# wzhe06/SparrowRecSys

Measured on AMD Instinct MI355X. Metric: ctr_samples_per_sec, higher is better.
Workload: dtype f32

## Files before the change

sparrowrecsys_amd/csrc/api_forward.h:

```cpp
static int launch_din_cols(sprk_handle h, const int32_t* ids, float* pooled, float* att, int32_t B, const DinColsMany* many, hipStream_t st) {
    DinColsRun c = h->din_cols_run;
    const long long ntasks = (long long)(many ? many->n : 1) * ((B + 15) / 16);
    const long long slots = (long long)h->num_cus * 16;
    c.ts = (c.T >= 16 && ntasks * 4 <= slots) ? 4 : ((c.T >= 8 && ntasks * 2 <= slots) ? 2 : 1);
    if (h->tune.din_cols_ts) c.ts = h->tune.din_cols_ts;
    if (many) c.ts = 1;
    c.ts_log2 = c.ts == 4 ? 2 : (c.ts == 2 ? 1 : 0);
    c.ql = (c.T + 3) / 4;
    const int EL = 4 * h->din_cols_kc;
    const size_t lds = ((size_t)2 * 64 * 36 + (size_t)DC_WAVES * 16 * c.idp + (size_t)DC_WAVES * 2 * 64 * EL) * sizeof(float);
    const long long grid = (ntasks * c.ts + DC_WAVES - 1) / DC_WAVES;
    if (many)
        hipLaunchKernelGGL(h->din_cols_kernels.many, dim3((unsigned)grid), dim3(DC_WAVES * 64), lds, st, c, nullptr, nullptr, nullptr, B, h->dev_err, *many);
    else
        hipLaunchKernelGGL(h->din_cols_kernels.one, dim3((unsigned)grid), dim3(DC_WAVES * 64), lds, st, c, ids, pooled, att, B, h->dev_err, DinColsOne{});
    HIP_TRY(hipGetLastError());
    return SPRK_OK;
}

static int launch_din_fused(sprk_handle h, const int32_t* ids, const float* dense, float* out, float* att, int32_t B, const DinFusedMany* many,
                            bool tail, hipStream_t st) {
    DinFusedRun c = h->din_fused_run;
    const long long ntasks = (long long)(many ? many->n : 1) * ((B + 15) / 16);
    const long long slots = (long long)h->num_cus * DF_WAVES;
// ... 136 lines not shown
        hipLaunchKernelGGL(h->mlp_rows_kernel, dim3(grid), dim3(MR_WAVES * 64), h->mlp_rows_lds, st, rr, ids, dense, out, B, h->dev_err, (const float*)h->mlp_rows_image);
        break;
    }
    case Route::DinTail: {
        const int tw = h->din_tail_waves;
        int grid = (ntasks + tw - 1) / tw;
        if (grid > h->num_cus) grid = h->num_cus;
        hipLaunchKernelGGL(h->din_tail_kernel, dim3(grid), dim3(tw * 64), kDinTailVariants[h->din_tail_variant].lds_bytes, st, h->din_tail_run, ids, dense, aux,
                           out, B, h->dev_err, h->din_tail_image, DinTailMany{});
        break;
    }
    default: {
        const int ntiles = (B + SPRK_TILE_M - 1) / SPRK_TILE_M;
        const int grid = ntiles < h->tile_grid_cap ? ntiles : h->tile_grid_cap;
        hipLaunchKernelGGL(k_tile_forward, dim3(grid), dim3(256), h->tile_lds_bytes, st, h->dev_plan, ids, dense, aux, out, B, h->dev_err);
    }
    }
    HIP_TRY(hipGetLastError());
    return SPRK_OK;
}

static int fork_helpers(sprk_handle h, int S, hipStream_t st) {
    HIP_TRY(hipEventRecord(h->many_fork, st));
    for (int s = 0; s < S; ++s) HIP_TRY(hipStreamWaitEvent(h->many_stream[s], h->many_fork, 0));
    return SPRK_OK;
}
static int join_helpers(sprk_handle h, int S, hipStream_t st) {
    for (int s = 0; s < S; ++s) {
        HIP_TRY(hipEventRecord(h->many_join[s], h->many_stream[s]));
        HIP_TRY(hipStreamWaitEvent(st, h->many_join[s], 0));
    }
    return SPRK_OK;
}

extern "C++" {
template <class Many, class Launch>
static int launch_groups(int32_t n_batches, int per, const int32_t* const* ids, const float* const* dense, float* const* out, Launch launch) {
    int g = 0;
    for (int32_t i0 = 0; i0 < n_batches; i0 += per, ++g) {
        Many m;
        memset(&m, 0, sizeof(m));
        m.n = n_batches - i0 < per ? n_batches - i0 : per;
        for (int j = 0; j < m.n; ++j) { m.ids[j] = ids[i0 + j]; m.dense[j] = dense ? dense[i0 + j] : nullptr; m.out[j] = out[i0 + j]; }
        SPRK_TRY(launch(m, g));
        HIP_TRY(hipGetLastError());
    }
    return SPRK_OK;
}
template <class Ok> static bool every_batch(int32_t n_batches, Ok ok) {
    for (int32_t i = 0; i < n_batches; ++i)
        if (!ok(i)) return false;
    return true;
}
}

static int launch_v2j_table(sprk_handle h, int32_t n_batches, const int32_t* const* ids, const float* const* dense, float* const* out, int32_t B,
                            hipStream_t st, bool* done) {
    *done = false;
    const int ntpb = (B + 15) / 16;
    long long grid = ((long long)n_batches * ntpb + V2_WAVES - 1) / V2_WAVES;
    if (grid > h->v2_grid_cap) grid = h->v2_grid_cap;
    if ((long long)n_batches * ntpb + 4 * grid * V2_WAVES >= (1LL << 31)) return SPRK_OK;
    hipStreamCaptureStatus cap = hipStreamCaptureStatusNone;
    if (hipStreamIsCapturing(st, &cap) != hipSuccess) { (void)hipGetLastError(); return SPRK_OK; }
    if (cap != hipStreamCaptureStatusNone) return SPRK_OK;
    const size_t n = (size_t)n_batches;
    int slot = h->v2j_table_last;
    bool same = slot >= 0 && h->v2j_table[slot].n == n && h->v2j_table[slot].stream == st;
    if (same) {
        const V2JBatch* last = h->v2j_table[slot].stage;
        for (size_t i = 0; i < n && same; ++i) same = last[i].ids == ids[i] && last[i].dense == dense[i] && last[i].out == out[i];
    }
    if (!same) {
        slot = h->v2j_table_last == 0 ? 1 : 0;
        sprk_engine::V2JTable& t = h->v2j_table[slot];
        if (!t.busy) HIP_TRY(hipEventCreateWithFlags(&t.busy, hipEventDisableTiming));
        if (t.used) HIP_TRY(hipEventSynchronize(t.busy));
        if (t.cap < n) {
            size_t want = t.cap ? 2 * t.cap : 4096;
            if (want < n) want = n;
            if (t.stage) (void)hipHostFree(t.stage);
            if (t.dev) (void)hipFree(t.dev);
            t.stage = nullptr; t.dev = nullptr; t.cap = 0; t.n = 0;
            HIP_TRY(hipHostMalloc((void**)&t.stage, want * sizeof(V2JBatch), hipHostMallocDefault));
            HIP_TRY(hipMalloc((void**)&t.dev, want * sizeof(V2JBatch)));
            t.cap = want;
        }
        t.n = 0;
        for (size_t i = 0; i < n; ++i) t.stage[i] = V2JBatch{ids[i], dense[i], out[i], nullptr};
        HIP_TRY(hipMemcpyAsync(t.dev, t.stage, n * sizeof(V2JBatch), hipMemcpyHostToDevice, st));
        t.n = n;
        t.stream = st;
        h->v2j_table_last = slot;
    }
    sprk_engine::V2JTable& t = h->v2j_table[slot];
    V2JRun jr = h->v2j_run;
    jr.flags = 0;
    const V2JManyTab m = {t.dev, n_batches, ntpb};
    hipLaunchKernelGGL(kV2JVariants[h->v2j_variant].fn_many_tab, dim3((int)grid), dim3(V2_WAVES * 64), h->v2j_lds_bytes, st, jr, m, B, h->dev_err, h->v2_image);
    HIP_TRY(hipGetLastError());
    HIP_TRY(hipEventRecord(t.busy, st));
    t.used = true;
    *done = true;
    return SPRK_OK;
}

static int forward_many_impl(sprk_handle h, int32_t n_batches, const int32_t* const* ids, const float* const* dense,
                             float* const* out, int32_t B, void* workspace, size_t workspace_bytes, void* stream,
                             int many_batches, int many_streams) {
    RoctxRange roctx_range_("sprk_forward_many");
    if (!h) return fail(SPRK_EINVAL, "handle is NULL");
    if (n_batches < 0) return fail(SPRK_EINVAL, "negative batch count");
    if (n_batches > 0 && !out) return fail(SPRK_EINVAL, "out is NULL");
    int S = (h->finalized && n_batches > 1) ? many_streams : 0;
    const size_t ws_need = (sprk_workspace_bytes(h, B) + 255) & ~(size_t)255;
    const bool ws_untouched = h->finalized && (h->route == Route::DinFused || h->route == Route::DienFused);
    if (S >= 2 && ws_need > 0 && !ws_untouched) {
        while (S >= 2 && (!workspace || workspace_bytes < (size_t)S * ws_need)) --S;
        if (S < 2) S = 0;
    }
    hipStream_t st = (hipStream_t)stream;
    const bool grouped = h->finalized && many_batches > 1 && n_batches > 1 && B > 0 && ids;
    const int ntpb = (B + 15) / 16;
    auto aligned = [&](int32_t i, const float* d) { return !(((uintptr_t)ids[i] | (uintptr_t)d) & 15); };
    auto present = [&](int32_t i) { return ids[i] && dense[i] && out[i]; };
    if (grouped && dense && h->route == Route::V2Joint && every_batch(n_batches, [&](int32_t i) { return present(i) && aligned(i, dense[i]); })) {
        const V2JVariant& jv = kV2JVariants[h->v2j_variant];
        V2JRun jr = h->v2j_run;
        jr.flags = 0;
        if (n_batches > many_batches) {
            bool done = false;
            SPRK_TRY(launch_v2j_table(h, n_batches, ids, dense, out, B, st, &done));
            if (done) return SPRK_OK;
        }
        return launch_groups<V2JMany>(n_batches, many_batches, ids, dense, out, [&](V2JMany& m, int) {
            m.ntpb = ntpb;
            long long grid = ((long long)m.n * ntpb + V2_WAVES - 1) / V2_WAVES;
            if (grid > h->v2_grid_cap) grid = h->v2_grid_cap;
            hipLaunchKernelGGL(jv.fn_many, dim3((int)grid), dim3(V2_WAVES * 64), h->v2j_lds_bytes, st, jr, m, B, h->dev_err, h->v2_image);
            return SPRK_OK;
        });
    }
    const float* const* rows_dense = h->plan.n_dense ? dense : nullptr;
    if (grouped && (dense || h->plan.n_dense == 0) && h->route == Route::Rows &&
        every_batch(n_batches, [&](int32_t i) { return ids[i] && out[i] && (!rows_dense || rows_dense[i]) && aligned(i, rows_dense ? rows_dense[i] : nullptr); })) {
        const RowsVariant& rv = kRowsVariants[h->rows_variant];
        RowsRun rr = h->rows_run;
        rr.flags = 0;
        return launch_groups<RowsMany>(n_batches, many_batches < RC_MB ? many_batches : RC_MB, ids, rows_dense, out, [&](RowsMany& m, int) {
            m.ntpb = ntpb;
            long long grid = ((long long)m.n * ntpb + RC_WAVES - 1) / RC_WAVES;
            if (grid > h->num_cus) grid = h->num_cus;
            hipLaunchKernelGGL(rv.fn_many, dim3((int)grid), dim3(RC_WAVES * 64), h->rows_lds_bytes, st, rr, m, B, h->dev_err, h->rows_image);
            return SPRK_OK;
        });
    }
    if (grouped && dense && h->route == Route::MlpRows && h->mlp_rows_many_kernel &&
        every_batch(n_batches, [&](int32_t i) { return present(i) && aligned(i, dense[i]); })) {
        MlpRowsRun rr = h->mlp_rows_run;
        rr.flags &= ~1;
        return launch_groups<MlpRowsMany>(n_batches, many_batches < MR_MB ? many_batches : MR_MB, ids, dense, out, [&](MlpRowsMany& m, int) {
            long long grid = ((long long)m.n * ntpb + MR_WAVES - 1) / MR_WAVES;
            if (grid > h->num_cus) grid = h->num_cus;
            hipLaunchKernelGGL(h->mlp_rows_many_kernel, dim3((int)grid), dim3(MR_WAVES * 64), h->mlp_rows_lds, st, rr, m, B, h->dev_err,
                               (const float*)h->mlp_rows_image);
            return SPRK_OK;
        });
    }
    if (grouped && dense && h->route == Route::Pairs && every_batch(n_batches, present)) {
        const size_t lds = kV1Variants[h->v1_variant].lds_bytes;
        return launch_groups<V1Many>(n_batches, many_batches < V1_MB ? many_batches : V1_MB, ids, dense, out, [&](V1Many& m, int) {
            m.ntpb = ntpb;
            long long grid = ((long long)m.n * ntpb + V1_WAVES - 1) / V1_WAVES;
            if (grid > h->num_cus) grid = h->num_cus;
            hipLaunchKernelGGL(h->v1_many_kernel, dim3((int)grid), dim3(V1_WAVES * 64), lds, st, h->v1_run, m, B, h->dev_err);
            return SPRK_OK;
        });
    }
    if (grouped && dense && h->route == Route::DinFused && h->tune.din_fused_mb && every_batch(n_batches, present)) {
        const int SG = S >= 2 ? S : 1;
        if (SG >= 2) SPRK_TRY(fork_helpers(h, SG, st));
        SPRK_TRY(launch_groups<DinFusedMany>(n_batches, many_batches < DF_MB ? many_batches : DF_MB, ids, dense, out, [&](DinFusedMany& m, int g) {
            return launch_din_fused(h, nullptr, nullptr, nullptr, nullptr, B, &m, true, SG >= 2 ? h->many_stream[g % SG] : st);
        }));
        if (SG >= 2) SPRK_TRY(join_helpers(h, SG, st));
        return SPRK_OK;
    }
    const bool cols = h->stage == Stage::DinCols || h->stage == Stage::DinFusedAttn;
    if (grouped && dense && workspace && ws_need > 0 && cols && (h->route == Route::DinTail || h->route == Route::DinFused)) {
        int per = many_batches < DIN_MB ? many_batches : DIN_MB;
        if ((size_t)per * ws_need > workspace_bytes) per = (int)(workspace_bytes / ws_need);
        if (per >= 2 && every_batch(n_batches, present)) {
            int SG = S >= 2 ? S : 1;
            while (SG > 1 && (size_t)SG * per * ws_need > workspace_bytes) --SG;
            if (SG >= 2) SPRK_TRY(fork_helpers(h, SG, st));
            const size_t tail_lds = kDinTailVariants[h->din_tail_variant].lds_bytes;
            const int tw = h->din_tail_waves;
            int g = 0;
            for (int32_t i0 = 0; i0 < n_batches; i0 += per, ++g) {
                const int n = n_batches - i0 < per ? n_batches - i0 : per;
                hipStream_t sg = SG >= 2 ? h->many_stream[g % SG] : st;
                char* wbase = (char*)workspace + (size_t)(g % SG) * per * ws_need;
                DinTailMany tm;
                memset(&tm, 0, sizeof(tm));
                tm.n = n; tm.ntpb = ntpb;
                for (int j = 0; j < n; ++j) {
                    float* pooled = (float*)(wbase + (size_t)j * ws_need);
                    tm.ids[j] = ids[i0 + j]; tm.dense[j] = dense[i0 + j]; tm.aux[j] = pooled; tm.out[j] = out[i0 + j];
                }
                if (n <= DC_MB) {
                    DinColsMany cm;
                    memset(&cm, 0, sizeof(cm));
                    cm.n = n;
                    for (int j = 0; j < n; ++j) { cm.ids[j] = tm.ids[j]; cm.pooled[j] = const_cast<float*>(tm.aux[j]); }
                    SPRK_TRY(launch_din_cols(h, nullptr, nullptr, nullptr, B, &cm, sg));
                } else {
                    for (int j = 0; j < n; ++j) SPRK_TRY(launch_din_cols(h, tm.ids[j], const_cast<float*>(tm.aux[j]), nullptr, B, nullptr, sg));
                }
                long long tg = ((long long)n * ntpb + tw - 1) / tw;
                if (tg > h->num_cus) tg = h->num_cus;
                hipLaunchKernelGGL(h->din_tail_many_kernel, dim3((int)tg), dim3(tw * 64), tail_lds, sg, h->din_tail_run, nullptr, nullptr, nullptr, nullptr, B,
                                   h->dev_err, h->din_tail_image, tm);
                HIP_TRY(hipGetLastError());
            }
// ... 93 lines not shown
    static const char* const kStageName[] = {"", "k_din_pool", "k_din_attn_cols", "k_din_fused", "k_dien_seq", "k_dien_seq_mfma"};
    const bool cols = h->stage == Stage::DinCols || h->stage == Stage::DinFusedAttn;
    size_t uploaded = 0;
    for (size_t b : h->slot_bytes) uploaded += b;
#ifndef SPRK_BUILD_DEFINES_STR
#define SPRK_BUILD_DEFINES_STR ""
#endif
    char split[96] = "";
    auto site = [&](bool on, const char* name) {
        if (!on) return;
        if (split[0]) strncat(split, ",", sizeof(split) - strlen(split) - 1);
        strncat(split, name, sizeof(split) - strlen(split) - 1);
    };
    switch (h->route) {
    case Route::V2Joint: site(kV2JVariants[h->v2j_variant].half, "v2"); break;
    case Route::Pairs:
        site(h->v1_run.w1frag != nullptr, "dyn_w1"); site(h->v1_run.w0frag != nullptr, "dyn_w0"); site(h->v1_run.e_scale != 0.f, "pairs_e");
        break;
    case Route::Rows: site(kRowsVariants[h->rows_variant].unf, "rows_unf"); break;
    case Route::MlpRows: site(h->mlp_rows_run.inv_w1_scale != 0.f, "dyn_w1"); break;
    case Route::DinTail: case Route::DinFused: case Route::DienFused:
        site(h->din_tail_run.inv_w1_scale != 0.f, "dyn_w1"); site(h->din_tail_run.inv_w0p_scale != 0.f, "dyn_w0p");
        site(h->din_tail_run.e_unscale != 0.f, "tail_unf");
        break;
    case Route::Tile: break;
    }
    site(cols, "din_attn");
    site(h->stage == Stage::DienSeqMfma, "dien_seq");
    const int n = snprintf(buf, buf_bytes, "kernel=%s;stage=%s;stage_waves_per_workgroup=%d;fused=%d;uploaded_bytes=%zu;derived_bytes=%zu;first_dense_fold=%d;split_f16=%s;build_defines=%s", kern,
                           kStageName[(int)h->stage], cols ? DC_WAVES : 0, h->route != Route::Tile ? 1 : 0, uploaded, h->derived_bytes, h->n_acc_folded, split, SPRK_BUILD_DEFINES_STR);
    if (n < 0 || (size_t)n >= buf_bytes) return fail(SPRK_EINVAL, "describe: buffer of %zu bytes is too small", buf_bytes);
    return SPRK_OK;
}

int sprk_check_ids(sprk_handle h, void* stream) {
    if (!h) return fail(SPRK_EINVAL, "handle is NULL");
    if (!h->finalized) return fail(SPRK_ESTATE, "check_ids before finalize");
    int flag = 0;
    HIP_TRY(hipMemcpyAsync(&flag, h->dev_err, sizeof(int), hipMemcpyDeviceToHost, (hipStream_t)stream));
    HIP_TRY(hipStreamSynchronize((hipStream_t)stream));
    if (flag) {
        HIP_TRY(hipMemsetAsync(h->dev_err, 0, sizeof(int), (hipStream_t)stream));
        HIP_TRY(hipStreamSynchronize((hipStream_t)stream));
        return fail(SPRK_ERANGE, "an id was outside its table (TF would raise InvalidArgumentError: assert_less_than_num_buckets) [flag 0x%x]", flag);
    }
    return SPRK_OK;
}

void sprk_destroy(sprk_handle h) {
    if (!h) return;
    for (size_t i = 0; i < h->slot_ptr.size(); ++i) free_slot(h, i);
    for (const sprk_engine::DevAlloc& a : h->allocs) release(a);
    if (h->v2j_tab) (void)hipFree(h->v2j_tab);
    for (sprk_engine::V2JTable& t : h->v2j_table) {
        if (t.used) (void)hipEventSynchronize(t.busy);
        if (t.stage) (void)hipHostFree(t.stage);
        if (t.dev) (void)hipFree(t.dev);
        if (t.busy) (void)hipEventDestroy(t.busy);
    }
    for (int i = 0; i < 4; ++i) { if (h->many_stream[i]) (void)hipStreamDestroy(h->many_stream[i]); if (h->many_join[i]) (void)hipEventDestroy(h->many_join[i]); }
    if (h->many_fork) (void)hipEventDestroy(h->many_fork);
    delete h;
}

int sprk_embedding_gather(const float* table, int32_t V, int32_t D, int32_t row_stride, const int32_t* ids,
                          int32_t B, float* out, void* stream) {
    if (!table || !ids || !out) return fail(SPRK_EINVAL, "NULL argument");
    if (V <= 0 || D <= 0 || (D & 3) || row_stride < D || (row_stride & 3)) return fail(SPRK_EINVAL, "bad gather geometry V=%d D=%d row_stride=%d", V, D, row_stride);
    if (B < 0) return fail(SPRK_EINVAL, "negative batch");
    if (B == 0) return SPRK_OK;
    const long long total = (long long)B * (D / 4);
    long long blocks = (total + 255) / 256;
    if (blocks > 8192) blocks = 8192;
    hipLaunchKernelGGL(k_embedding_gather, dim3((unsigned)blocks), dim3(256), 0, (hipStream_t)stream, table, V, D / 4, row_stride, ids, B, out);
    HIP_TRY(hipGetLastError());
    return SPRK_OK;
}
```

sparrowrecsys_amd/csrc/host_engine.h:

```cpp
enum class Route { Tile, V2Joint, Rows, Pairs, MlpRows, DinTail, DinFused, DienFused };
enum class Stage { None, DinPool, DinCols, DinFusedAttn, DienSeq, DienSeqMfma };

typedef void (*V2JKernel)(const V2JRun, const int*, const float*, float*, int, int*, const float*);
typedef void (*V2JManyKernel)(const V2JRun, const V2JMany, int, int*, const float*);
typedef void (*V2JManyTabKernel)(const V2JRun, const V2JManyTab, int, int*, const float*);
typedef void (*RowsKernel)(const RowsRun, const int*, const float*, float*, int, int*, const float*);
typedef void (*RowsManyKernel)(const RowsRun, const RowsMany, int, int*, const float*);
typedef void (*V1Kernel)(const V1Run, const int*, const float*, float*, int, int*);
typedef void (*V1ManyKernel)(const V1Run, const V1Many, int, int*);
typedef void (*MlpRowsKernel)(const MlpRowsRun, const int*, const float*, float*, int, int*, const float*);
typedef void (*MlpRowsManyKernel)(const MlpRowsRun, const MlpRowsMany, int, int*, const float*);
typedef void (*DinTailKernel)(const DinTailRun, const int*, const float*, const float*, float*, int, int*, const float*, const DinTailMany);
typedef void (*DinColsKernel)(const DinColsRun, const int*, float*, float*, int, int*, const DinColsOne);
typedef void (*DinColsManyKernel)(const DinColsRun, const int*, float*, float*, int, int*, const DinColsMany);
typedef void (*DinFusedKernel)(const DinFusedRun, const int*, const float*, float*, float*, int, int*, const DinFusedOne);
typedef void (*DinFusedManyKernel)(const DinFusedRun, const int*, const float*, float*, float*, int, int*, const DinFusedMany);
typedef void (*DienSeqKernel)(const DienRun, const int*, float*, int, int*);
typedef void (*DienFusedKernel)(const DienRun, const DinTailRun, const int*, const float*, float*, int, int*, const float*, float*);
struct DinColsKernels { DinColsKernel one; DinColsManyKernel many; };
struct DinFusedKernels { DinFusedKernel one; DinFusedManyKernel many; };
template <class Kernel> static int set_max_lds(Kernel k, size_t bytes) {
    HIP_TRY(hipFuncSetAttribute(reinterpret_cast<const void*>(k), hipFuncAttributeMaxDynamicSharedMemorySize, (int)bytes));
    return SPRK_OK;
}

struct sprk_engine {
    sprk_plan plan;
    std::vector<void*> slot_ptr;
    std::vector<size_t> slot_bytes;
    std::vector<char> slot_external;
    DevPlan* dev_plan = nullptr;
    int* dev_err = nullptr;
    bool finalized = false;
    Route route = Route::Tile;
    Stage stage = Stage::None;
    int device = 0;
    int num_cus = 256;
    int buf_stride[SPRK_MAX_BUFS] = {0, 0, 0};
    int buf_base[SPRK_MAX_BUFS] = {0, 0, 0};
    size_t tile_lds_bytes = 0;
    int ids_base = 0;
    std::vector<int> idc;
    int tile_grid_cap = 0;
    int many_streams = 0;
    hipStream_t many_stream[4] = {nullptr, nullptr, nullptr, nullptr};
    hipEvent_t many_fork = nullptr, many_join[4] = {nullptr, nullptr, nullptr, nullptr};
    int v1_variant = -1;
    V1Kernel v1_kernel = nullptr;
    V1Kernel v1_one_kernel = nullptr;
    V1ManyKernel v1_many_kernel = nullptr;
    V1Run v1_run;
    int mlp_rows_nbig = -1;
    MlpRowsRun mlp_rows_run;
    MlpRowsKernel mlp_rows_kernel = nullptr;
    MlpRowsManyKernel mlp_rows_many_kernel = nullptr;
    float* mlp_rows_image = nullptr;
    float* mlp_rows_small = nullptr;
    size_t mlp_rows_lds = 0;
    int din_tail_variant = -1;
    DinTailRun din_tail_run;
    DinTailKernel din_tail_kernel = nullptr, din_tail_many_kernel = nullptr;
    int din_tail_waves = 0;
    float* din_tail_image = nullptr;
    int din_ms = 0;
    size_t din_lds_bytes = 0;
    int din_grid_cap = 0;
    DienRun dien_run{};
    float* dien_frag = nullptr;
    size_t dien_frag_floats = 0;
    DienSeqKernel dien_seq_kernel = nullptr;
    SprkTuning tune;
    int din_cols_kc = 0;
    DinColsRun din_cols_run;
    DinColsKernels din_cols_kernels{};
    bool din_fused = false;
    bool din_fused_attn = false;
    DinFusedRun din_fused_run;
    DinFusedKernels din_fused_kernels[2]{};
    DinFusedKernel din_fused_att_kernel = nullptr;
    float* din_fused_image = nullptr;
    bool dien_fused = false;
    DienFusedKernel dien_fused_kernel = nullptr;
    size_t dien_fused_lds = 0;
    int v2_variant = -1;
    bool v2_rows_ok = false;
    V2Args v2;
    const float* v2_w1_grp[V2_MAX_FIELDS] = {};
    V2Run v2run;
    int v2_grid_cap = 0;
    float* v2_image = nullptr;
    float* v2_fo_all = nullptr;
    float* v2_folded = nullptr;
    size_t v2_fo_floats = 0;
    int v2j_variant = -1;
    V2JKernel v2j1_kernel = nullptr;
    float* v2j1_image = nullptr;
    size_t v2j1_lds_bytes = 0;
    int v2j1_waves = 8;
    int many_batches = 1;
    int rows_variant = -1;
    bool rows_from_v2 = false;
    int rows_g_emb = 0;
    RowsRun rows_run;
    float* rows_tab = nullptr;
    float* rows_scal = nullptr;
    float* rows_small = nullptr;
    float* rows_image = nullptr;
    size_t rows_lds_bytes = 0;
    int n_acc_folded = 0;
    size_t derived_bytes = 0;
    V2JRun v2j_run;
    float* v2j_tab = nullptr;
    size_t v2j_lds_bytes = 0;
    float* v2j_big = nullptr;
    struct V2JTable {
        V2JBatch* stage = nullptr;
        V2JBatch* dev = nullptr;
        size_t cap = 0;
        size_t n = 0;
        hipStream_t stream = nullptr;
        hipEvent_t busy = nullptr;
        bool used = false;
    };
    V2JTable v2j_table[2];
    int v2j_table_last = -1;
    struct DevAlloc { void* p; size_t vmm_size; hipMemGenericAllocationHandle_t handle; };
    std::vector<DevAlloc> allocs;
};

static void release(const sprk_engine::DevAlloc& a) {
    if (!a.vmm_size) { (void)hipFree(a.p); return; }
    (void)hipMemUnmap(a.p, a.vmm_size);
    (void)hipMemRelease(a.handle);
    (void)hipMemAddressFree(a.p, a.vmm_size);
}
template <class T> static int dev_alloc(sprk_engine* h, T** out, size_t bytes) {
    void* p = nullptr;
    HIP_TRY(hipMalloc(&p, bytes));
    h->allocs.push_back(sprk_engine::DevAlloc{p, 0, nullptr});
    *out = static_cast<T*>(p);
    return SPRK_OK;
}
static void dev_free(sprk_engine* h, void* p) {
    if (!p) return;
    for (size_t i = 0; i < h->allocs.size(); ++i)
        if (h->allocs[i].p == p) {
            release(h->allocs[i]);
            h->allocs.erase(h->allocs.begin() + (long)i);
            return;
        }
}
static void free_slot(sprk_engine* h, size_t slot) {
    if (h->slot_ptr[slot] && !h->slot_external[slot]) (void)hipFree(h->slot_ptr[slot]);
}

template <class T> static int table_alloc(sprk_engine* h, T** out, size_t bytes) {
    *out = nullptr;
    if (h->tune.vmm_tables && bytes >= ((size_t)256 << 20)) {
        hipMemAllocationProp prop = {};
        prop.type = hipMemAllocationTypePinned;
        prop.location.type = hipMemLocationTypeDevice;
        prop.location.id = h->device;
        size_t gran = 0;
        if (hipMemGetAllocationGranularity(&gran, &prop, hipMemAllocationGranularityRecommended) == hipSuccess) {
            if (gran < ((size_t)2 << 20)) gran = (size_t)2 << 20;
            const size_t total = (bytes + gran - 1) / gran * gran;
            void* va = nullptr;
            hipMemGenericAllocationHandle_t hnd;
            if (hipMemAddressReserve(&va, total, (size_t)1 << 30, nullptr, 0) == hipSuccess) {
                if (hipMemCreate(&hnd, total, &prop, 0) == hipSuccess) {
                    hipMemAccessDesc acc = {};
                    acc.location = prop.location;
                    acc.flags = hipMemAccessFlagsProtReadWrite;
                    if (hipMemMap(va, total, 0, hnd, 0) == hipSuccess) {
                        if (hipMemSetAccess(va, total, &acc, 1) == hipSuccess) {
                            h->allocs.push_back(sprk_engine::DevAlloc{va, total, hnd});
                            *out = static_cast<T*>(va);
                            return SPRK_OK;
// ... 14 lines not shown
```

sparrowrecsys_amd/csrc/host_setup_pairs.h:

```cpp
constexpr int V1_WAVES = 8;
constexpr int V1_ONE_MAX_TASKS = 16384;
struct V1Variant {
    int nf, nv;
    bool sep;
    V1Kernel fn_dyn, fn_f32, fn_one;
    V1ManyKernel fn_many_dyn, fn_many_f32;
    void (*pack)(const V1Run, float*);
    size_t lds_bytes;
};
#define V1_VARIANT(NF, NV, SEP, ONE)                                                                                                    \
    {NF, NV, SEP, &k_deepfm_pairs<NF, NV, 4, 4, V1_WAVES, true, SEP>, &k_deepfm_pairs<NF, NV, 4, 4, V1_WAVES, false, SEP>, ONE,         \
     &k_deepfm_pairs_many<NF, NV, 4, 4, V1_WAVES, true, SEP>, &k_deepfm_pairs_many<NF, NV, 4, 4, V1_WAVES, false, SEP>,                 \
     &k_v1_pack_image<4, 4, (NV + 3) / 4>, V1Lds<4, 4, (NV + 3) / 4>::bytes}
#define V1_ONE(NF, NV, SEP) &k_deepfm_pairs1<NF, NV, 4, 4, V1_WAVES, SEP>
#define V1_BOTH(NF, NV) V1_VARIANT(NF, NV, true, V1_ONE(NF, NV, true)), V1_VARIANT(NF, NV, false, V1_ONE(NF, NV, false))
const V1Variant kV1Variants[] = {
    V1_BOTH(6, 4),
    V1_BOTH(4, 3),
    V1_BOTH(4, 4),
    V1_VARIANT(4, 16, true, nullptr), V1_VARIANT(4, 16, false, nullptr),
};

int setup_deepfm_pairs(sprk_engine* h) {
    if (!h->tune.v1_chain) return SPRK_OK;
    const sprk_plan& p = h->plan;
    if (p.model_kind != SPRK_MODEL_DEEPFM || p.din.enabled || p.n_ops != 3 || p.n_taps != 3 || p.n_pairs < 1) return SPRK_OK;
    const sprk_op &od = p.ops[0], &o0 = p.ops[1], &o1 = p.ops[2];
    if (od.kind != SPRK_OP_PAIR_DOT || od.src_buf != 0 || od.dst_buf != 0) return SPRK_OK;
    if (o0.kind != SPRK_OP_DENSE || o0.act != SPRK_ACT_RELU || o0.src_buf != 0 || o0.dst_buf != 1 || o0.dst_off != 0 || o0.N != 64) return SPRK_OK;
    if (o1.kind != SPRK_OP_DENSE || o1.act != SPRK_ACT_RELU || o1.src_buf != 1 || o1.src_off != 0 || o1.K != o0.N || o1.dst_off != 0 || o1.N != 64) return SPRK_OK;
    V1Run r;
    memset(&r, 0, sizeof(r));
    int row_dst[V1_MAX_FIELDS], nf = 0, Dp = 0, num_dst = -1, scal_dst[V1_MAX_FIELDS], ns = 0, scal_col[V1_MAX_FIELDS], scal_vocab[V1_MAX_FIELDS];
    const float* scal_tab[V1_MAX_FIELDS];
    const int ds0 = o0.src_off, ds1 = o0.src_off + o0.K;
    int dsep_col[V1_MAX_DEEP], dsep_vocab[V1_MAX_DEEP], dsep_dst[V1_MAX_DEEP], n_dsep = 0;
    const float* dsep_tab[V1_MAX_DEEP];
    for (int i = 0; i < p.n_segs; ++i) {
        const sprk_seg& sg = p.segs[i];
        if (sg.kind == SPRK_SEG_ROWS) {
            if (nf == 0 && n_dsep == 0) Dp = sg.row_stride;
            if (sg.row_stride != Dp || sg.count * 4 != Dp || Dp > 64) return SPRK_OK;
            if (h->slot_bytes[sg.slot] < ((size_t)sg.vocab + 1) * Dp * sizeof(float)) return SPRK_OK;
            bool twin_outside = false;
            for (int j = 0; j < p.n_segs; ++j)
                if (j != i && p.segs[j].kind == SPRK_SEG_ROWS && p.segs[j].field == sg.field &&
                    !(p.segs[j].dst >= ds0 && p.segs[j].dst + p.segs[j].row_stride <= ds1)) twin_outside = true;
            if (twin_outside && sg.dst >= ds0 && sg.dst + Dp <= ds1) {
                if (n_dsep == V1_MAX_DEEP) return SPRK_OK;
                dsep_col[n_dsep] = sg.field; dsep_vocab[n_dsep] = sg.vocab; dsep_tab[n_dsep] = (const float*)h->slot_ptr[sg.slot];
                dsep_dst[n_dsep++] = sg.dst;
                continue;
            }
            if (nf == V1_MAX_FIELDS) return SPRK_OK;
            r.col[nf] = sg.field; r.vocab[nf] = sg.vocab; r.table[nf] = (const float*)h->slot_ptr[sg.slot];
            row_dst[nf++] = sg.dst;
        } else if (sg.kind == SPRK_SEG_SCALAR) {
            if (ns == V1_MAX_FIELDS) return SPRK_OK;
            if (h->slot_bytes[sg.slot] < ((size_t)sg.vocab + 1) * sizeof(float)) return SPRK_OK;
            scal_col[ns] = sg.field; scal_vocab[ns] = sg.vocab; scal_tab[ns] = (const float*)h->slot_ptr[sg.slot]; scal_dst[ns++] = sg.dst;
        } else if (sg.kind == SPRK_SEG_DENSE) {
            if (num_dst >= 0 || sg.field != 0 || sg.count > 8) return SPRK_OK;
            num_dst = sg.dst; r.n_num = sg.count;
        } else if (sg.kind != SPRK_SEG_ZERO) {
            return SPRK_OK;
// ... 124 lines not shown
                const long long rows = (long long)r.vocab[f] + 1;
                jobs.push_back({deep_tables[f], rows, Dp, Dp, absmax_grid(rows * Dp, 8192), 0});
            }
            float mx = 0.f, e_scale = 0.f;
            SPRK_TRY(static_scale(jobs, &e_scale, &mx));
            if (e_scale != 0.f && mx > 0.f) {
                r.e_scale = e_scale;
                r.e_inv = r.inv_w0_scale / r.e_scale;
            }
        }
    }
    r.tab = nullptr;
    if (PC == 1) {
        const int pack = !sep ? 0 : (Dp <= 12 ? 80 : (Dp == 16 ? 64 : 0));
        size_t rows = 0;
        for (int f = 0; f < nf; ++f) rows += (size_t)r.vocab[f] + 1;
        if (sep && !pack) for (int d = 0; d < r.n_deep; ++d) rows += (size_t)r.vocab[d] + 1;
        if (rows * 128 < ((size_t)1 << 32)) {
            float* tab = nullptr;
            SPRK_TRY(table_alloc(h, &tab, rows * 128));
            h->derived_bytes += rows * 128;
            float* w1c = nullptr;
            if (pack == 64) {
                size_t nw = 0;
                for (int d = 0; d < r.n_deep; ++d) { r.w1cbase[d] = (unsigned)nw; nw += (size_t)r.vocab[d] + 1; }
                SPRK_TRY(dev_alloc(h, &w1c, nw * sizeof(float) + 16));
                for (int d = 0; d < r.n_deep; ++d)
                    HIP_TRY(hipMemcpy(w1c + r.w1cbase[d], r.w1[d], ((size_t)r.vocab[d] + 1) * sizeof(float), hipMemcpyDeviceToDevice));
            }
            size_t base = 0;
            for (int f = 0; f < nf + ((sep && !pack) ? r.n_deep : 0); ++f) {
                const bool deep_row = f >= nf;
                const bool packed_here = pack && f < r.n_deep;
                const long long n = (long long)r.vocab[deep_row ? f - nf : f] + 1;
                long long nb = (n * 32 + 255) / 256;
                if (nb > 65536) nb = 65536;
                hipLaunchKernelGGL(k_v1_build_rows, dim3((unsigned)nb), dim3(256), 0, 0, r.table[f], Dp,
                                   (deep_row || (packed_here && pack == 64)) ? (const float*)nullptr : r.w1[f], n, tab + base * 32,
                                   packed_here ? r.table[nf + f] : (const float*)nullptr, pack / 4);
                r.rowbase[f] = (unsigned)base;
                base += (size_t)n;
            }
            HIP_TRY(hipGetLastError());
            HIP_TRY(hipDeviceSynchronize());
            r.tab = tab;
            r.pack = pack;
            r.w1c = w1c;
        }
    }
    const V1Variant& vv = kV1Variants[variant];
    const bool dyn = r.inv_w1_scale != 0.f;
    h->v1_kernel = dyn ? vv.fn_dyn : vv.fn_f32;
    h->v1_many_kernel = dyn ? vv.fn_many_dyn : vv.fn_many_f32;
    h->v1_one_kernel = (r.tab && r.w1frag && PC == 1 && h->tune.v1_one) ? vv.fn_one : nullptr;
    SPRK_TRY(set_max_lds(h->v1_kernel, vv.lds_bytes));
    SPRK_TRY(set_max_lds(h->v1_many_kernel, vv.lds_bytes));
    if (h->v1_one_kernel) SPRK_TRY(set_max_lds(h->v1_one_kernel, vv.lds_bytes));
    h->v1_run = r;
    h->v1_variant = variant;
    return SPRK_OK;
}
```

sparrowrecsys_amd/csrc/host_setup_rows.h:

```cpp
constexpr int RC_WAVES = 8;
struct RowsLayout { int image_floats, ss, rb, sn, s1, off_wn, off_bn, off_m, off_c0, off_w1, off_b1, off_hfm, off_hd, off_fn, off_cp, off_af; };
template <class LD> constexpr RowsLayout rows_layout() {
    return {LD::total_pad, LD::SS, LD::RB, LD::SN, LD::S1, LD::off_wn, LD::off_bn, LD::off_m, LD::off_c0, LD::off_w1, LD::off_b1, LD::off_hfm,
            LD::off_hd, LD::off_fn, LD::off_cp, LD::off_af};
}
struct RowsVariant {
    int kpc, h0c, h1c, g_big, njf;
    bool hasnum;
    bool unf;
    RowsKernel fn;
    RowsManyKernel fn_many;
    RowsKernel fn_one;
    RowsLayout ld;
};
#define ROWS_VARIANT_X(KPC, H0C, H1C, G_BIG, NJF, HASNUM, UNF)                                                                   \
    {KPC, H0C, H1C, G_BIG, NJF, HASNUM, UNF, &k_rows_chain<KPC, H0C, H1C, G_BIG, NJF, HASNUM, RC_WAVES, UNF>,                    \
     &k_rows_chain_many<KPC, H0C, H1C, G_BIG, NJF, HASNUM, RC_WAVES, UNF>, &k_rows_chain1<KPC, H0C, H1C, G_BIG, NJF, HASNUM, RC_WAVES, UNF>, \
     rows_layout<RowsLds<KPC, H0C, H1C, HASNUM, UNF>>()}
#define ROWS_VARIANT(KPC, H0C, H1C, G_BIG, NJF, HASNUM) ROWS_VARIANT_X(KPC, H0C, H1C, G_BIG, NJF, HASNUM, false)
const RowsVariant kRowsVariants[] = {
    ROWS_VARIANT_X(4, 2, 1, 2, 2, true, true),
    ROWS_VARIANT_X(4, 2, 1, 2, 1, true, true), ROWS_VARIANT_X(4, 2, 1, 1, 1, true, true), ROWS_VARIANT_X(2, 2, 1, 2, 2, true, true),
    ROWS_VARIANT(4, 2, 1, 2, 2, true),
    ROWS_VARIANT(4, 2, 1, 2, 1, true), ROWS_VARIANT(4, 2, 1, 1, 1, true), ROWS_VARIANT(4, 2, 1, 3, 3, true), ROWS_VARIANT(4, 2, 1, 3, 1, true),
    ROWS_VARIANT(2, 2, 1, 2, 2, true),
    ROWS_VARIANT(2, 2, 1, 3, 3, true),
    ROWS_VARIANT(1, 2, 1, 3, 3, true),
    ROWS_VARIANT(0, 1, 1, 2, 0, false),
};
int find_rows_variant(int kpc, int h0c, int h1c, int g_big, int njf, bool hasnum, bool unf = false) {
    for (size_t v = 0; v < sizeof(kRowsVariants) / sizeof(kRowsVariants[0]); ++v) {
        const RowsVariant& r = kRowsVariants[v];
        if (r.kpc == kpc && r.h0c == h0c && r.h1c == h1c && r.g_big == g_big && r.njf == njf && r.hasnum == hasnum && r.unf == unf) return (int)v;
    }
    return -1;
}
int pull(std::vector<float>& dst, const float* src, size_t n) {
    dst.resize(n);
    HIP_TRY(hipMemcpy(dst.data(), src, n * sizeof(float), hipMemcpyDeviceToHost));
    return SPRK_OK;
}
int rows_finish(sprk_engine* h, const RowsVariant& rv, const std::vector<float>& image, size_t small_floats) {
    SPRK_TRY(dev_alloc(h, &h->rows_image, (size_t)rv.ld.image_floats * sizeof(float)));
    HIP_TRY(hipMemcpy(h->rows_image, image.data(), (size_t)rv.ld.image_floats * sizeof(float), hipMemcpyHostToDevice));
    h->rows_lds_bytes = ((size_t)rv.ld.image_floats + RC_WAVES * 256 + small_floats) * sizeof(float);
    if (h->rows_lds_bytes > 160 * 1024) return fail(SPRK_EINVAL, "rows chain needs %zu bytes of LDS", h->rows_lds_bytes);
    SPRK_TRY(set_max_lds(rv.fn, h->rows_lds_bytes));
    SPRK_TRY(set_max_lds(rv.fn_many, h->rows_lds_bytes));
    SPRK_TRY(set_max_lds(rv.fn_one, h->rows_lds_bytes));
    HIP_TRY(hipDeviceSynchronize());
    return SPRK_OK;
}

int setup_rows_v2(sprk_engine* h, bool allow_unf = true) {
    const V2Args& a = h->v2;
    const sprk_plan& p = h->plan;
    const int G = h->rows_g_emb;
    const sprk_op &d0 = p.ops[G + 2], &d1 = p.ops[G + 3];
    const int KP = p.ops[0].N, H0 = d0.N, H1 = d1.N, Dp = a.ldp_emb;
    int big[V2_MAX_FIELDS], nbig = 0, sm[V2_MAX_FIELDS], nsm = 0;
    for (int g = 0; g < G; ++g) {
        if ((long long)a.emb_vocab[g] + 1 <= 32 && nsm < RC_MAX_SMALL) sm[nsm++] = g;
        else big[nbig++] = g;
    }
    if (nbig < 1 || nbig > RC_MAX_BIG) return SPRK_OK;
    int variant = -1;
    float p_scale = 1.f;
    if (allow_unf && h->tune.rows_unf && h->tune.dyn_f16 && nbig <= 2 && Dp <= 16 && KP + H0 > 16) {
        const int vu = find_rows_variant(KP / 16, H0 / 16, H1 / 16, nbig, nsm, true, true);
        if (vu >= 0) {
            std::vector<AbsmaxJob> jobs;
            for (int b = 0; b < nbig; ++b) jobs.push_back({a.table[big[b]], (long long)a.emb_vocab[big[b]] + 1, Dp, Dp, 1024, 0});
            float e_scale = 0.f;
            SPRK_TRY(static_scale(jobs, &e_scale));
            if (e_scale != 0.f) {
                p_scale = e_scale;
                variant = vu;
            }
        }
    }
    if (variant < 0) variant = find_rows_variant(KP / 16, H0 / 16, H1 / 16, nbig, nsm, true);
    if (variant < 0) return SPRK_OK;
    const RowsVariant& rv = kRowsVariants[variant];
    const bool unf = rv.unf;
    const float* w1g[V2_MAX_FIELDS];
    for (int g = 0; g < G; ++g) {
        w1g[g] = nullptr;
        for (int i = 0; i < a.n_fo; ++i)
            if (a.fo_col[i] == a.emb_col[g] && a.fo_vocab[i] == a.emb_vocab[g]) w1g[g] = a.w1[i];
        if (!w1g[g]) return SPRK_OK;
    }
    RowsRun& r = h->rows_run;
    memset(&r, 0, sizeof(r));
    r.F = a.F; r.ND = a.ND; r.n_num = a.n_num;
    size_t big_rows = 0;
    for (int b = 0; b < nbig; ++b) {
        r.big_col[b] = a.emb_col[big[b]]; r.big_vocab[b] = a.emb_vocab[big[b]];
        r.big_rowbase[b] = (unsigned)big_rows; r.big_scal[b] = (unsigned)big_rows;
        big_rows += (size_t)a.emb_vocab[big[b]] + 1;
    }
    if (big_rows >= ((size_t)1 << 31)) return SPRK_OK;
// ... 181 lines not shown
```

sparrowrecsys_amd/csrc/k_chain_v1.h:

```cpp

#define V1_MAX_FIELDS 8
#define V1_MAX_DEEP 2
#define V1_MAX_ROWS (V1_MAX_FIELDS + V1_MAX_DEEP)

struct V1Run {
    int F, ND, n_num;
    int nf;
    int col[V1_MAX_FIELDS];
    int vocab[V1_MAX_FIELDS];
    int row_floats;
    const float* table[V1_MAX_ROWS];
    const float* w1[V1_MAX_FIELDS];
    int n_deep;
    int sep;
    int pack;
    const float* w1c;
    unsigned w1cbase[V1_MAX_DEEP];
    float pw[V1_MAX_FIELDS * V1_MAX_FIELDS];
    const float* w0;
    const float* b0;
    const float* W1;
    int ld1;
    const float* b1;
    const float* hdeep;
    float head_bias;
    const float* w1frag;
    float inv_w1_scale;
    const float* w0frag;
    float inv_w0_scale;
    const float* image;
    float e_scale, e_inv;
    const float* tab;
    unsigned rowbase[V1_MAX_ROWS];
};

static __global__ __launch_bounds__(256) void k_v1_build_rows(const float* __restrict__ table, int Dp, const float* __restrict__ w1,
                                                       long long rows, float* __restrict__ out, const float* __restrict__ deep, int deep_off) {
    const long long total = rows * 32;
    for (long long i = (long long)blockIdx.x * 256 + threadIdx.x; i < total; i += (long long)gridDim.x * 256) {
        const long long v = i >> 5;
        const int c = (int)(i & 31);
        float x = c < Dp ? table[v * Dp + c] : ((c == 16 && w1) ? w1[v] : 0.f);
        if (deep && c >= deep_off && c - deep_off < Dp) x = deep[v * Dp + (c - deep_off)];
        out[i] = x;
    }
}

static __global__ __launch_bounds__(256) void k_v1_pack_w0(const float* __restrict__ W0, int ldw0, int n_deep, int off0, int off1,
                                                    int Dp, int n_off, int n_num, int H0, int PC, float* __restrict__ w0) {
    const int KW = 16 * (V1_MAX_DEEP * PC + 1);
    for (int i = threadIdx.x; i < H0 * KW; i += 256) {
        const int n = i / KW, k = i - n * KW, c = k >> 4, j = k & 15;
        float v = 0.f;
        if (c < V1_MAX_DEEP * PC) {
            const int f = c / PC, col = 16 * (c - f * PC) + j;
            if (f < n_deep && col < Dp) v = W0[(size_t)n * ldw0 + (f == 0 ? off0 : off1) + col];
        } else if (j < n_num) {
            v = W0[(size_t)n * ldw0 + n_off + j];
        }
        w0[i] = v;
    }
}

#define V1_MB 16
struct V1Many {
    const int* ids[V1_MB];
    const float* dense[V1_MB];
    float* out[V1_MB];
    int n, ntpb;
};

template <int H0C, int H1C, int PC = 1>
struct V1Lds {
    static constexpr int H0 = H0C * 16, H1 = H1C * 16;
    static constexpr int S1 = H0 + 4;
    static constexpr int KE = 32 * PC;
    static constexpr int SE = KE + 4;
    static constexpr int off_w1 = 0;
    static constexpr int off_w0e = off_w1 + H1 * S1;
    static constexpr int off_w0n = off_w0e + H0 * SE;
    static constexpr int off_b0 = off_w0n + H0 * 8;
    static constexpr int off_b1 = off_b0 + H0;
    static constexpr int off_hd = off_b1 + H1;
    static constexpr int total = off_hd + H1;
    static constexpr int total_pad = (total + 255) & ~255;
    static constexpr size_t bytes = sizeof(float) * total_pad;
    static_assert(H1C * (H0C / 2) * 512 <= H1 * S1 && H0C * PC * 512 <= H0 * SE && H0C % 2 == 0, "fragments fit their regions");
};

template <int H0C, int H1C, int PC>
__global__ __launch_bounds__(256) void k_v1_pack_image(const V1Run A, float* __restrict__ img) {
    using LD = V1Lds<H0C, H1C, PC>;
    const int tid = threadIdx.x, KW = 16 * (V1_MAX_DEEP * PC + 1);
    for (int i = tid; i < LD::total_pad; i += 256) img[i] = 0.f;
    __syncthreads();
    if (A.w1frag) {
        for (int i = tid; i < H1C * (H0C / 2) * 512; i += 256) img[LD::off_w1 + i] = A.w1frag[i];
    } else {
        for (int i = tid; i < LD::H1 * LD::S1; i += 256) {
            const int n = i / LD::S1, k = i - n * LD::S1;
            img[LD::off_w1 + i] = k < LD::H0 ? A.W1[(size_t)n * A.ld1 + k] : 0.f;
        }
    }
    if (A.w0frag) {
        for (int i = tid; i < H0C * PC * 512; i += 256) img[LD::off_w0e + i] = A.w0frag[i];
    } else {
        for (int i = tid; i < LD::H0 * LD::SE; i += 256) {
            const int n = i / LD::SE, k = i - n * LD::SE;
            img[LD::off_w0e + i] = k < LD::KE ? A.w0[(size_t)n * KW + k] : 0.f;
        }
    }
    for (int i = tid; i < LD::H0 * 8; i += 256) img[LD::off_w0n + i] = A.w0[(size_t)(i >> 3) * KW + 16 * V1_MAX_DEEP * PC + (i & 7)];
    for (int i = tid; i < LD::H0; i += 256) img[LD::off_b0 + i] = A.b0[i];
    for (int i = tid; i < LD::H1; i += 256) { img[LD::off_b1 + i] = A.b1[i]; img[LD::off_hd + i] = A.hdeep[i]; }
}

template <int NR, int PC>
struct V1Set {
    f32x4 x[NR][PC];
    float xa, xb;
    float w1a, w1b;
};

template <int NF, int NV, int H0C, int H1C, int WAVES, bool DYN, bool MB, bool SEP, bool ONE = false>
__device__ __forceinline__ void v1_body(const V1Run& A, const int* __restrict__ ids0, const float* __restrict__ dense0,
                                        float* __restrict__ out0, int B, int* __restrict__ err, const V1Many* __restrict__ Mp) {
    constexpr int PC = (NV + 3) / 4;
    constexpr int NR = NF + (SEP ? V1_MAX_DEEP : 0);
    constexpr int DB = SEP ? NF : 0;
    using LD = V1Lds<H0C, H1C, PC>;
    using Set = V1Set<NR, PC>;
    static_assert(!(ONE && MB) && !(ONE && PC > 1), "one-task shape: one batch, narrow rows");
    static_assert(NF >= 2 && NF <= V1_MAX_FIELDS && NV >= 1 && (NV <= 4 || NV % 4 == 0) && NV <= 16, "shape");
    const int tid = threadIdx.x;
    const int lane = tid & 63;
    const int wave = __builtin_amdgcn_readfirstlane(tid >> 6);
    const int r = lane & 15, q = lane >> 4;
    const f32x4 zero = f32x4{0.f, 0.f, 0.f, 0.f};
    const int m_ntpb = MB ? Mp->ntpb : 0;
    const int ntasks = MB ? Mp->n * m_ntpb : (B + 15) >> 4;
    const int task_stride = gridDim.x * WAVES;
    bool bad = false;
    auto batch_of = [&](int t, int& tl) {
        if constexpr (MB) {
            const int b = __builtin_amdgcn_readfirstlane(t / m_ntpb);
            tl = t - b * m_ntpb;
            return b;
        } else {
            tl = t;
            return 0;
        }
    };
    auto ld_ids = [&](int tg, int (&idv)[NF]) {
        int t;
        const int bi = batch_of(tg, t);
        const int* ids = MB ? Mp->ids[bi] : ids0;
        const int m = min(t * 16 + r, B - 1);
        const int* row = ids + (size_t)m * A.F;
#pragma unroll
        for (int f = 0; f < NF; ++f) idv[f] = row[A.col[f]];
    };
    auto issue_gather = [&](int tg, const int (&idv)[NF], Set& S) {
        int t;
        const int bi = batch_of(tg, t);
        const float* dense = MB ? Mp->dense[bi] : dense0;
        const int m = min(t * 16 + r, B - 1);
        {
            const float* nrow = dense + (size_t)m * A.ND;
            const int last = A.n_num - 1;
            S.xa = nrow[min(q, last)];
            S.xb = nrow[min(q + 4, last)];
        }
        unsigned sid[NF];
#pragma unroll
        for (int f = 0; f < NF; ++f) {
            bad |= (unsigned)(idv[f] + 1) > (unsigned)A.vocab[f];
            sid[f] = min((unsigned)idv[f], (unsigned)A.vocab[f]);
        }
        if ((ONE && NV == 4) || (PC == 1 && A.tab)) {
            const char* tb = reinterpret_cast<const char*>(A.tab);
            unsigned ro[NF];
#pragma unroll
            for (int f = 0; f < NF; ++f) ro[f] = (sid[f] + A.rowbase[f]) * 128u;
#pragma unroll
            for (int f = 0; f < NF; ++f) S.x[f][0] = q < NV ? *reinterpret_cast<const f32x4*>(tb + (ro[f] + 16u * q)) : zero;
            if constexpr (SEP) {
#pragma unroll
                for (int d = 0; d < V1_MAX_DEEP; ++d) {
                    S.x[NF + d][0] = zero;
                    if (d < A.n_deep) {
                        const unsigned rd = A.pack ? ro[d] + (unsigned)A.pack : (sid[d] + A.rowbase[NF + d]) * 128u;
                        if (q < NV) S.x[NF + d][0] = *reinterpret_cast<const f32x4*>(tb + (rd + 16u * q));
                    }
                }
            }
            unsigned oa = ro[0], ob = ro[NF > 4 ? 4 : 0];
            if (NF > 1) oa = q == 1 ? ro[NF > 1 ? 1 : 0] : oa;
            if (NF > 2) oa = q == 2 ? ro[NF > 2 ? 2 : 0] : oa;
            if (NF > 3) oa = q == 3 ? ro[NF > 3 ? 3 : 0] : oa;
            if (NF > 5) ob = q == 1 ? ro[NF > 5 ? 5 : 0] : ob;
            if (NF > 6) ob = q == 2 ? ro[NF > 6 ? 6 : 0] : ob;
            if (NF > 7) ob = q == 3 ? ro[NF > 7 ? 7 : 0] : ob;
            const float* pa = reinterpret_cast<const float*>(tb + (oa + 64u));
            if (A.w1c) {
                const unsigned ci = (q == 1 ? sid[1] + A.w1cbase[1] : sid[0] + A.w1cbase[0]);
                pa = q < A.n_deep ? A.w1c + ci : pa;
            }
            S.w1a = (q < NF) ? *pa : 0.f;
            S.w1b = (NF > 4 && q + 4 < NF) ? *reinterpret_cast<const float*>(tb + (ob + 64u)) : 0.f;
            return;
        }
#pragma unroll
        for (int f = 0; f < NF; ++f)
#pragma unroll
            for (int pc = 0; pc < PC; ++pc)
                S.x[f][pc] = 4 * pc + q < NV ? ld4(A.table[f] + (size_t)sid[f] * A.row_floats + 16 * pc + 4 * q) : zero;
        if constexpr (SEP) {
#pragma unroll
// ... 107 lines not shown
#pragma unroll
            for (int nb = 0; nb < H0C; ++nb)
#pragma unroll
                for (int j = 0; j < 4; ++j) mx = fmaxf(mx, h0[nb][j]);
            mx = rows4_max(mx);
            float scale, inv;
            dyn_scale(mx, A.inv_w1_scale, scale, inv);
            f32x4 acc[H1C];
#pragma unroll
            for (int n1 = 0; n1 < H1C; ++n1) acc[n1] = zero;
            int wfo = LD::off_w1 + lane * 4;
            asm volatile("" : "+v"(wfo));
#pragma unroll
            for (int b = 0; b < H0C / 2; ++b) {
                f16x8 bh, bl;
                dyn_split8(h0[2 * b], h0[2 * b + 1], scale, bh, bl);
#pragma unroll
                for (int n1 = 0; n1 < H1C; ++n1) {
                    const f16x8 ah = __builtin_bit_cast(f16x8, ld4(smem + wfo + ((n1 * (H0C / 2) + b) * 2 + 0) * 256));
                    const f16x8 al = __builtin_bit_cast(f16x8, ld4(smem + wfo + ((n1 * (H0C / 2) + b) * 2 + 1) * 256));
                    acc[n1] = mfma_f16(ah, bh, acc[n1]);
                    acc[n1] = mfma_f16(ah, bl, acc[n1]);
                    acc[n1] = mfma_f16(al, bh, acc[n1]);
                }
            }
#pragma unroll
            for (int n1 = 0; n1 < H1C; ++n1) h1[n1] = acc[n1] * inv + ld4(smem + LD::off_b1 + n1 * 16 + 4 * q);
        } else {
#pragma unroll
            for (int n1 = 0; n1 < H1C; ++n1) h1[n1] = ld4(smem + LD::off_b1 + n1 * 16 + 4 * q);
            int w1o = LD::off_w1 + r * LD::S1 + 4 * q;
            asm volatile("" : "+v"(w1o));
#pragma unroll
            for (int c = 0; c < H0C; ++c) {
                f32x4 a[H1C];
#pragma unroll
                for (int n1 = 0; n1 < H1C; ++n1) a[n1] = ld4(smem + w1o + n1 * 16 * LD::S1 + 16 * c);
#pragma unroll
                for (int st = 0; st < 4; ++st)
#pragma unroll
                    for (int n1 = 0; n1 < H1C; ++n1)
                        h1[n1] = __builtin_amdgcn_mfma_f32_16x16x4f32(a[n1][st], h0[c][st], h1[n1], 0, 0, 0);
            }
        }
#pragma unroll
        for (int n1 = 0; n1 < H1C; ++n1) {
            const f32x4 hd = ld4(smem + LD::off_hd + n1 * 16 + 4 * q), hr = relu4_fast(h1[n1]);
#pragma unroll
            for (int j = 0; j < 4; ++j) z = fmaf(hd[j], hr[j], z);
        }
        z = rows4_sum(z);
        return sigmoidf_acc(z + A.head_bias);
    };
    auto store = [&](int tg, float score) {
        int tl;
        const int bo = batch_of(tg, tl);
        float* out = MB ? Mp->out[bo] : out0;
        const int mm = tl * 16 + r;
        if (q == 0 && mm < B) out[mm] = score;
    };

    int tA = blockIdx.x * WAVES + wave, tB = tA + task_stride;
    int idA[NF], idB[NF];
#pragma unroll
    for (int f = 0; f < NF; ++f) { idA[f] = -1; idB[f] = -1; }
    if (tA < ntasks) ld_ids(tA, idA);
    if (!ONE && tB < ntasks) ld_ids(tB, idB);
#pragma unroll 1
    for (int c = wave; c < LD::total_pad / 256; c += WAVES) lds_dma16(A.image + c * 256 + lane * 4, smem + c * 256);
    Set SA, SB;
    if constexpr (ONE) {
        __builtin_amdgcn_s_waitcnt(0x0F70);
        __builtin_amdgcn_s_barrier();
        if (tA < ntasks) issue_gather(tA, idA, SA);
#pragma unroll
        for (int nb = 0; nb < H0C; ++nb) {
            rna[nb] = smem[LD::off_w0n + (nb * 16 + r) * 8 + q];
            rnb[nb] = smem[LD::off_w0n + (nb * 16 + r) * 8 + q + 4];
        }
        if (tA < ntasks) store(tA, compute(SA));
    } else {
    __builtin_amdgcn_s_waitcnt(0x0F70);
    __builtin_amdgcn_s_barrier();
#pragma unroll
    for (int nb = 0; nb < H0C; ++nb) {
        rna[nb] = smem[LD::off_w0n + (nb * 16 + r) * 8 + q];
        rnb[nb] = smem[LD::off_w0n + (nb * 16 + r) * 8 + q + 4];
    }
    if (tA >= ntasks) {
    } else if (PC == 1 && ntasks <= 2 * task_stride) {
        issue_gather(tA, idA, SA);
        if (tB < ntasks) issue_gather(tB, idB, SB);
        store(tA, compute(SA));
        if (tB < ntasks) store(tB, compute(SB));
    } else {
        issue_gather(tA, idA, SA);
        for (int tk = tA; tk < ntasks; tk += task_stride) {
            const Set cur = SA;
            if (tk + task_stride < ntasks) {
                issue_gather(tk + task_stride, idB, SA);
                if (tk + 2 * task_stride < ntasks) ld_ids(tk + 2 * task_stride, idB);
            }
            store(tk, compute(cur));
        }
    }
    }
    if (__ballot(bad) != 0 && lane == 0) atomicOr(err, 1);
}

template <int NF, int NV, int H0C, int H1C, int WAVES, bool DYN, bool SEP>
__global__ __launch_bounds__(WAVES * 64, 2) void k_deepfm_pairs(const V1Run A, const int* __restrict__ ids, const float* __restrict__ dense,
                                                                float* __restrict__ out, int B, int* __restrict__ err) {
    v1_body<NF, NV, H0C, H1C, WAVES, DYN, false, SEP>(A, ids, dense, out, B, err, nullptr);
}
template <int NF, int NV, int H0C, int H1C, int WAVES, bool DYN, bool SEP>
__global__ __launch_bounds__(WAVES * 64, 2) void k_deepfm_pairs_many(const V1Run A, const V1Many M, int B, int* __restrict__ err) {
    v1_body<NF, NV, H0C, H1C, WAVES, DYN, true, SEP>(A, nullptr, nullptr, nullptr, B, err, &M);
}
template <int NF, int NV, int H0C, int H1C, int WAVES, bool SEP>
__global__ __launch_bounds__(WAVES * 64, 4) void k_deepfm_pairs1(const V1Run A, const int* __restrict__ ids, const float* __restrict__ dense,
                                                                 float* __restrict__ out, int B, int* __restrict__ err) {
    v1_body<NF, NV, H0C, H1C, WAVES, true, false, SEP, true>(A, ids, dense, out, B, err, nullptr);
}
```

sparrowrecsys_amd/csrc/k_chain_v2j.h:

```cpp

#define V2J_MAX_BIG 4
#define V2J_MAX_JF 3
#define V2J_SS 52

struct V2JRun {
    int F, ND, n_num;
    int big_col[V2J_MAX_BIG];
    int big_vocab[V2J_MAX_BIG];
    unsigned big_rowbase[V2J_MAX_BIG];
    int big_grp[V2J_MAX_BIG];
    int j_col[V2J_MAX_JF];
    int j_vocab[V2J_MAX_JF];
    int s_off[V2J_MAX_JF];
    int small_floats;
    int wf_off;
    const float* tab0;
    const float* small;
    float h0w, fo_bias, head_bias;
    int flags;
    float w_scale, unscale_h, unscale_s;
};

#define V2J_MB 64
struct V2JMany {
    const int* ids[V2J_MB];
    const float* dense[V2J_MB];
    float* out[V2J_MB];
    int n;
    int ntpb;
};
struct V2JBatch {
    const int* ids;
    const float* dense;
    float* out;
    void* pad_;
};
struct V2JManyTab {
    const V2JBatch* batch;
    int n;
    int ntpb;
};
struct V2JOne {};
__device__ __forceinline__ const int* v2j_ids(const V2JMany& m, int b) { return m.ids[b]; }
__device__ __forceinline__ const float* v2j_dense(const V2JMany& m, int b) { return m.dense[b]; }
__device__ __forceinline__ float* v2j_out(const V2JMany& m, int b) { return m.out[b]; }
typedef const __attribute__((address_space(4))) V2JBatch* V2JBatchCP;
__device__ __forceinline__ const int* v2j_ids(const V2JManyTab& m, int b) { return ((V2JBatchCP)(uintptr_t)m.batch + b)->ids; }
__device__ __forceinline__ const float* v2j_dense(const V2JManyTab& m, int b) { return ((V2JBatchCP)(uintptr_t)m.batch + b)->dense; }
__device__ __forceinline__ float* v2j_out(const V2JManyTab& m, int b) { return ((V2JBatchCP)(uintptr_t)m.batch + b)->out; }

__device__ __forceinline__ void split_half4(f32x4 w, float scale, f16x4& hi, f16x4& lo) {
#pragma unroll
    for (int j = 0; j < 4; ++j) {
        const float x = w[j] * scale;
        const _Float16 h = (_Float16)x;
        hi[j] = h;
        lo[j] = (_Float16)(x - (float)h);
    }
}

static __global__ __launch_bounds__(256) void k_v2_absmax(const float* __restrict__ rows, long long nrows, int row_floats,
                                                   int ncols, unsigned* __restrict__ out) {
    float m = 0.f;
    const long long total = nrows * ncols;
    for (long long i = (long long)blockIdx.x * 256 + threadIdx.x; i < total; i += (long long)gridDim.x * 256) {
        const long long v = i / ncols;
        const int c = (int)(i - v * ncols);
        const float a = fabsf(rows[v * row_floats + c]);
        m = (a > m || a != a) ? a : m;
    }
    for (int d = 32; d >= 1; d >>= 1) { const float o = __shfl_xor(m, d); m = (o > m || o != o) ? o : m; }
    if ((threadIdx.x & 63) == 0) atomicMax(out, __float_as_uint(m));
}
static __global__ __launch_bounds__(256) void k_v2_count_small(const float* __restrict__ rows, long long nrows, int row_floats, int ncols,
                                                        float thresh, unsigned long long* __restrict__ out) {
    unsigned small = 0, nz = 0;
    const long long total = nrows * ncols;
    for (long long i = (long long)blockIdx.x * 256 + threadIdx.x; i < total; i += (long long)gridDim.x * 256) {
        const long long v = i / ncols;
        const int c = (int)(i - v * ncols);
        const float a = fabsf(rows[v * row_floats + c]);
        nz += a > 0.f;
        small += (a > 0.f && a < thresh);
    }
    for (int d = 32; d >= 1; d >>= 1) { small += __shfl_xor(small, d); nz += __shfl_xor(nz, d); }
    if ((threadIdx.x & 63) == 0) { atomicAdd(out, (unsigned long long)small); atomicAdd(out + 1, (unsigned long long)nz); }
}
static __global__ __launch_bounds__(256) void k_v2_split_rows(const float* __restrict__ src, float* __restrict__ dst,
                                                       long long nrows, float scale) {
    const long long total = nrows * 8;
    for (long long i = (long long)blockIdx.x * 256 + threadIdx.x; i < total; i += (long long)gridDim.x * 256) {
        const long long v = i >> 3;
        const int pc = (int)(i & 7);
        const f32x4 in = ld4(src + v * 32 + 4 * pc);
        if (pc < 4) {
            f16x4 hi, lo;
            split_half4(in, scale, hi, lo);
            f16x8 o = {hi[0], hi[1], hi[2], hi[3], lo[0], lo[1], lo[2], lo[3]};
            *reinterpret_cast<f16x8*>(dst + v * 32 + 4 * pc) = o;
        } else {
            st4(dst + v * 32 + 4 * pc, in);
        }
// ... 52 lines not shown
    return f32x4{__builtin_fmaf(s.x, s.x, -(p.x * p.x)), __builtin_fmaf(s.y, s.y, -(p.y * p.y)), __builtin_fmaf(s.z, s.z, -(p.z * p.z)),
                 __builtin_fmaf(s.w, s.w, -(p.w * p.w))};
}

template <int G_BIG, int NJF>
struct V2JSet {
    f32x4 x[G_BIG];
    int so[NJF];
    f32x4 xn;
    float w1a;
    float* dst;
};

template <int G_BIG, int NJF, int KPC, int H0C, int H1C, int WAVES, bool HALF, class Many>
__device__ __forceinline__ void v2j_body(const V2JRun& A, const int* __restrict__ ids, const float* __restrict__ dense,
                                         float* __restrict__ out, int B, int* __restrict__ err,
                                         const float* __restrict__ image, const Many* __restrict__ Mp) {
    constexpr bool MB = !std::is_same<Many, V2JOne>::value;
    constexpr int G_EMB = G_BIG + NJF;
    using LD = V2Lds<G_EMB, 4, KPC, H0C, H1C, true>;
    using Set = V2JSet<G_BIG, NJF>;
    constexpr int KP = LD::KP, H0 = H0C * 16;
    constexpr unsigned RB = (KP + 16) * 4;
    static_assert(KP + H0 + 1 <= V2J_SS, "small-field row layout");
    constexpr int NKR = HALF ? 1 : (G_BIG + 1) * KPC;
    static_assert(KPC == 1, "row layout: one 16-float chunk of projections per field");
    static_assert(G_BIG >= 1 && G_BIG <= 3 && NJF >= 1 && NJF <= V2J_MAX_JF, "field split");
    const int tid = threadIdx.x;
    const int lane = tid & 63;
    const int wave = __builtin_amdgcn_readfirstlane(tid >> 6);
    const int r = lane & 15, q = lane >> 4;
    const f32x4 zero = f32x4{0.f, 0.f, 0.f, 0.f};
    int m_ntpb = 0, ntasks = (B + 15) >> 4;
    if constexpr (MB) { m_ntpb = Mp->ntpb; ntasks = Mp->n * m_ntpb; }
    const int task_stride = gridDim.x * WAVES;
    const int wave_global = blockIdx.x * WAVES + wave;
    auto batch_of = [&](int tk) -> int {
        if constexpr (MB) return __builtin_amdgcn_readfirstlane(tk / m_ntpb);
        else return 0;
    };
    auto in_batch = [&](int tk, int b) -> int { return MB ? tk - b * m_ntpb : tk; };
    float* stage = smem + LD::total_pad + wave * LD::stage_floats;
    const float* small_s = smem + LD::total_pad + WAVES * LD::stage_floats;
    const float* wq = smem + 4 * q;
    bool bad = false;
    const bool aligned = !(A.flags & 1);
    auto clampt = [&](int tk) { return tk < ntasks ? tk : ntasks - 1; };

    auto ld_raw = [&](int tkg, f32x4& raw) -> int {
        const int b = batch_of(tkg);
        const int tk = in_batch(tkg, b);
        const int* ids_b = ids;
        const float* dense_b = dense;
        if constexpr (MB) { ids_b = v2j_ids(*Mp, b); dense_b = v2j_dense(*Mp, b); }
        if (aligned && tk * 16 + 16 <= B) {
            const bool isid = lane < 32;
            const int j = isid ? lane : lane - 32;
            const int n4 = 4 * (isid ? A.F : A.ND);
            const float* src = isid ? reinterpret_cast<const float*>(ids_b) + (size_t)tk * 16 * A.F
                                    : dense_b + (size_t)tk * 16 * A.ND;
            raw = ld4(src + 4 * (j < n4 ? j : 0));
        }
        return b;
    };
    auto gather = [&](int tkg, int b, const f32x4& raw, Set& S) {
        const int tk = in_batch(tkg, b);
        if (aligned && tk * 16 + 16 <= B) {
            const bool isid = lane < 32;
            const int j = isid ? lane : lane - 32;
            const int n4 = 4 * (isid ? A.F : A.ND);
            if (j < n4) st4(stage + (isid ? 0 : 128) + 4 * j, raw);
        } else {
            const int* ids_b = ids;
            const float* dense_b = dense;
            if constexpr (MB) { ids_b = v2j_ids(*Mp, b); dense_b = v2j_dense(*Mp, b); }
            stage_task_slow(stage, ids_b, dense_b, A.F, A.ND, tk, B, lane);
        }
        const int* sid_row = reinterpret_cast<const int*>(stage) + r * A.F;
        unsigned sid[G_BIG];
#pragma unroll
        for (int b = 0; b < G_BIG; ++b) {
            const int id = sid_row[A.big_col[b]];
            bad |= (unsigned)(id + 1) > (unsigned)A.big_vocab[b];
            sid[b] = min((unsigned)id, (unsigned)A.big_vocab[b]) + A.big_rowbase[b];
        }
#pragma unroll
        for (int f = 0; f < NJF; ++f) {
            const int id = sid_row[A.j_col[f]];
            bad |= (unsigned)(id + 1) > (unsigned)A.j_vocab[f];
            S.so[f] = A.s_off[f] + (int)min((unsigned)id, (unsigned)A.j_vocab[f]) * V2J_SS;
        }
        {
            const float* nrow = stage + 128 + r * A.ND;
            const int c0 = 4 * q, last = A.n_num - 1;
            if constexpr (HALF) {
                S.xn.x = nrow[min(q, last)];
                S.xn.y = nrow[min(q + 4, last)];
            } else {
                S.xn.x = nrow[min(c0 + 0, last)];
                S.xn.y = nrow[min(c0 + 1, last)];
                S.xn.z = nrow[min(c0 + 2, last)];
                S.xn.w = nrow[min(c0 + 3, last)];
            }
        }
        const char* tb = reinterpret_cast<const char*>(A.tab0);
#pragma unroll
        for (int b = 0; b < G_BIG; ++b) S.x[b] = *reinterpret_cast<const f32x4*>(tb + (sid[b] * RB + 16u * q));
        {
            unsigned s0 = sid[0] * RB, s1 = sid[G_BIG > 1 ? 1 : 0] * RB, s2 = sid[G_BIG > 2 ? 2 : 0] * RB;
            asm("" : "+v"(s0), "+v"(s1), "+v"(s2));
            unsigned so = s0;
            if (G_BIG > 1) so = q == 1 ? s1 : so;
            if (G_BIG > 2) so = q == 2 ? s2 : so;
            S.w1a = *reinterpret_cast<const float*>(tb + (so + 4u * KP));
        }
        {
            float* out_b;
            if constexpr (MB) {
                out_b = v2j_out(*Mp, b);
                asm("" : "+s"(out_b));
            } else {
                out_b = out;
            }
            const int m = tk * 16 + r;
            S.dst = (q == 0 && m < B) ? out_b + m : nullptr;
        }
    };

    f32x4 rW0[H0C][NKR], rW1[H1C][H0C];
    f32x4 rwn[KPC], rbpn[KPC], rb1[H1C], rhfm[KPC], rhd[H1C];
    f32x4 rfn = zero;
    float rwn8[2] = {0.f, 0.f}, rfn8[2] = {0.f, 0.f}, rwf[H0C][2];
    f16x8 hWa[HALF ? G_BIG : 1][H0C], hWb[HALF ? G_BIG : 1][H0C];
    f16x8 hSel = {0, 0, 0, 0, 0, 0, 0, 0};
    auto load_weights = [&]() {
        const float* w0r = wq + LD::off_w0 + r * LD::S0;
#pragma unroll
        for (int n0 = 0; n0 < H0C; ++n0) {
            if constexpr (HALF) {
                rwf[n0][0] = small_s[A.wf_off + (n0 * 16 + r) * 8 + q];
                rwf[n0][1] = small_s[A.wf_off + (n0 * 16 + r) * 8 + q + 4];
            } else {
                rW0[n0][0] = ld4(w0r + n0 * 16 * LD::S0 + 16 * G_EMB);
            }
#pragma unroll
            for (int b = 0; b < G_BIG; ++b) {
                const f32x4 w = ld4(w0r + n0 * 16 * LD::S0 + 16 * A.big_grp[b]);
                if constexpr (HALF) {
                    f16x4 hi, lo;
                    split_half4(w, A.w_scale, hi, lo);
                    hWa[b][n0] = f16x8{hi[0], hi[1], hi[2], hi[3], hi[0], hi[1], hi[2], hi[3]};
                    hWb[b][n0] = f16x8{lo[0], lo[1], lo[2], lo[3], lo[0], lo[1], lo[2], lo[3]};
                } else {
                    rW0[n0][(HALF ? 0 : 1 + b)] = w;
                }
            }
        }
        if constexpr (HALF) {
#pragma unroll
            for (int e = 0; e < 8; ++e) hSel[e] = (4 * q + (e & 3) == r) ? (_Float16)1.0f : (_Float16)0.0f;
        }
#pragma unroll
        for (int n1 = 0; n1 < H1C; ++n1) {
#pragma unroll
            for (int j = 0; j < H0C; ++j) rW1[n1][j] = ld4(wq + LD::off_w1 + (n1 * 16 + r) * LD::S1 + 16 * j);
            rb1[n1] = ld4(wq + LD::off_b1 + n1 * 16);
            rhd[n1] = ld4(wq + LD::off_hd + n1 * 16);
        }
#pragma unroll
        for (int nb = 0; nb < KPC; ++nb) {
            rwn[nb] = ld4(wq + LD::off_wn + (nb * 16 + r) * LD::SN);
            rbpn[nb] = ld4(wq + LD::off_bp + G_EMB * KP + nb * 16);
// ... 124 lines not shown
#pragma unroll 1
    for (int c = wave; c < A.small_floats / 256; c += WAVES) lds_dma16(A.small + c * 256 + lane * 4, smem + LD::total_pad + WAVES * LD::stage_floats + c * 256);
    const bool two = tA < ntasks && ntasks <= 2 * task_stride;
    constexpr int NG = G_BIG + 1;
    static_assert(NG < 16, "s_waitcnt immediate below encodes vmcnt < 16");
    if (two) {
        gather(tA, nA, rawA, SA);
        __builtin_amdgcn_s_waitcnt(0x0F70 | NG);
    } else {
        __builtin_amdgcn_s_waitcnt(0x0F70);
        if (tA < ntasks) {
            gather(tA, nA, rawA, SA);
            nA = ld_raw(clampt(tA + 2 * task_stride), rawA);
            gather(clampt(tB), nB, rawB, SB);
            nB = ld_raw(clampt(tB + 2 * task_stride), rawB);
        }
    }
    __builtin_amdgcn_s_barrier();
    load_weights();
    if (tA >= ntasks) {
    } else if (two) {
        gather(clampt(tB), nB, rawB, SB);
        store(SA, compute(SA));
        if (tB < ntasks) store(SB, compute(SB));
    } else {
        for (;;) {
            store(SA, compute(SA));
            tA += 2 * task_stride;
            gather(clampt(tA), nA, rawA, SA);
            nA = ld_raw(clampt(tA + 2 * task_stride), rawA);
            if (tB >= ntasks) break;
            store(SB, compute(SB));
            tB += 2 * task_stride;
            gather(clampt(tB), nB, rawB, SB);
            nB = ld_raw(clampt(tB + 2 * task_stride), rawB);
            if (tA >= ntasks) break;
        }
    }
    if (__ballot(bad) != 0 && lane == 0) atomicOr(err, 1);
}

template <int G_BIG, int NJF, int KPC, int H0C, int H1C, int WAVES, bool HALF>
__global__ __launch_bounds__(WAVES * 64, 2) void k_deepfm_v2_joint(const V2JRun A, const int* __restrict__ ids,
                                                                   const float* __restrict__ dense, float* __restrict__ out, int B,
                                                                   int* __restrict__ err, const float* __restrict__ image) {
    v2j_body<G_BIG, NJF, KPC, H0C, H1C, WAVES, HALF, V2JOne>(A, ids, dense, out, B, err, image, nullptr);
}
template <int G_BIG, int NJF, int KPC, int H0C, int H1C, int WAVES, bool HALF>
__global__ __launch_bounds__(WAVES * 64, 2) void k_deepfm_v2_joint_many(const V2JRun A, const V2JMany M, int B, int* __restrict__ err,
                                                                        const float* __restrict__ image) {
    v2j_body<G_BIG, NJF, KPC, H0C, H1C, WAVES, HALF, V2JMany>(A, nullptr, nullptr, nullptr, B, err, image, &M);
}
template <int G_BIG, int NJF, int KPC, int H0C, int H1C, int WAVES, bool HALF>
__global__ __launch_bounds__(WAVES * 64, 2) void k_deepfm_v2_joint_many_tab(const V2JRun A, const V2JManyTab M, int B, int* __restrict__ err,
                                                                            const float* __restrict__ image) {
    v2j_body<G_BIG, NJF, KPC, H0C, H1C, WAVES, HALF, V2JManyTab>(A, nullptr, nullptr, nullptr, B, err, image, &M);
}
```

sparrowrecsys_amd/csrc/k_rows_chain.h:

```cpp

#define RC_MAX_BIG 3
#define RC_MAX_SMALL 3
#define RC_MB 64

struct RowsRun {
    int F, ND, n_num;
    int big_col[RC_MAX_BIG];
    int big_vocab[RC_MAX_BIG];
    unsigned big_rowbase[RC_MAX_BIG];
    unsigned big_scal[RC_MAX_BIG];
    int s_col[RC_MAX_SMALL];
    int s_vocab[RC_MAX_SMALL];
    int s_off[RC_MAX_SMALL];
    int small_floats;
    const float* rows;
    const float* scal;
    const float* small;
    float bias;
    int flags;
    float unscale;
};
struct RowsMany {
    const int* ids[RC_MB];
    const float* dense[RC_MB];
    float* out[RC_MB];
    int n, ntpb;
};

template <int KPC, int H0C, int H1C, bool HASNUM, bool UNF = false>
struct RowsLds {
    static constexpr int KP = KPC * 16, H0 = H0C * 16, H1 = H1C * 16;
    static constexpr int SS = KP + H0 + 4;
    static constexpr int RB = UNF ? 64 : (((KP + H0) * 4 + 63) & ~63);
    static constexpr int SN = 12;
    static constexpr int S1 = H0 + 4;
    static constexpr int off_wn = 0;
    static constexpr int off_bn = off_wn + (HASNUM ? KP * SN : 0);
    static constexpr int off_m = off_bn + (HASNUM ? KP : 0);
    static constexpr int off_c0 = off_m + (HASNUM ? H0 * SN : 0);
    static constexpr int off_w1 = off_c0 + H0;
    static constexpr int off_b1 = off_w1 + H1 * S1;
    static constexpr int off_hfm = off_b1 + H1;
    static constexpr int off_hd = off_hfm + KP;
    static constexpr int off_fn = off_hd + H1;
    static constexpr int off_cp = off_fn + 8;
    static constexpr int off_af = (off_cp + (UNF ? KP : 0) + 3) & ~3;
    static constexpr int total = off_af + (UNF ? (KPC + H0C) * 2 * 256 : 0);
    static constexpr int total_pad = (total + 255) & ~255;
    static constexpr int stage_floats = 256;
    static_assert((SS / 4) % 2 == 1, "small-row stride must be an odd number of 16-byte slots");
};

static __global__ __launch_bounds__(256) void k_rows_build(const float* __restrict__ table, int row_floats, long long rows,
                                                    const float* __restrict__ Wp, int ldp, const float* __restrict__ bp, int KP,
                                                    const float* __restrict__ W0t, int ld0, int col0, int H0, int nsrc,
                                                    const float* __restrict__ qbias,
                                                    const float* __restrict__ w1, const float* __restrict__ hfm, int n_hfm, float h0w,
                                                    float* __restrict__ out, int out_stride, float* __restrict__ scal_out,
                                                    int scal_in_row) {
    __shared__ float sP[4][64];
    const int wv = threadIdx.x >> 6, n = threadIdx.x & 63;
    for (long long v = (long long)blockIdx.x * 4 + wv; v < rows; v += (long long)gridDim.x * 4) {
        const float* x = table + v * row_floats;
        float p = 0.f;
        if (KP > 0) {
            if (n < KP) {
                const float* w = Wp + (size_t)n * ldp;
                p = bp ? bp[n] : 0.f;
                for (int c = 0; c < row_floats; c += 16)
                    for (int s = 0; s < 4; ++s)
                        for (int q = 0; q < 4; ++q) {
                            const int k = c + 4 * q + s;
                            if (k < row_floats) p = fmaf(w[k], x[k], p);
                        }
            }
        } else if (n < nsrc) {
            p = x[n];
        }
        sP[wv][n] = p;
        float sqw = (KP > 0 && n < n_hfm && n < KP) ? hfm[n] * p * p : 0.f;
        for (int d = 32; d >= 1; d >>= 1) sqw += __shfl_xor(sqw, d);
        float* o = out ? out + v * out_stride : nullptr;
        if (o && n < KP) o[n] = p;
        for (int m = n; o && m < H0; m += 64) {
            const float* w = W0t + (size_t)m * ld0 + col0;
            float acc = qbias ? qbias[m] : 0.f;
            for (int k = 0; k < nsrc; ++k) acc = fmaf(w[k], sP[wv][k], acc);
            o[KP + m] = acc;
        }
        const float s = w1 ? h0w * w1[v] - sqw : 0.f;
        if (n == 0) {
            if (scal_out) scal_out[v] = s;
            if (o && scal_in_row) o[KP + H0] = s;
        }
    }
}

static __global__ __launch_bounds__(256) void k_rows_unf_split(const float* __restrict__ table, int row_floats, long long rows, float scale,
                                                        _Float16* __restrict__ out, int W = 16) {
    for (long long i = (long long)blockIdx.x * 256 + threadIdx.x; i < rows * W; i += (long long)gridDim.x * 256) {
        const long long v = i / W;
        const int k = (int)(i - v * W);
        const float x = k < row_floats ? table[v * row_floats + k] * scale : 0.f;
        const _Float16 hi = (_Float16)x;
        out[v * 2 * W + k] = hi;
        out[v * 2 * W + W + k] = (_Float16)(x - (float)hi);
    }
}
template <int G_BIG, int KPC, int H0C>
struct RowsSetUnf {
    f16x8 ehi, elo;
    int so[RC_MAX_SMALL];
    float xa, xb;
    float sc;
};

template <int G_BIG, int KPC, int H0C>
struct RowsSet {
    f32x4 xp[G_BIG > 0 ? G_BIG : 1][KPC > 0 ? KPC : 1];
    f32x4 xq[G_BIG > 0 ? G_BIG : 1][H0C];
    int so[RC_MAX_SMALL];
    float xa, xb;
    float sc;
};

__device__ __forceinline__ float dot4_fma(f32x4 a, f32x4 b, float acc) {
    acc = fmaf(a.x, b.x, acc);
    acc = fmaf(a.y, b.y, acc);
    acc = fmaf(a.z, b.z, acc);
    return fmaf(a.w, b.w, acc);
}

template <int KPC, int H0C, int H1C, int G_BIG, int NJF, bool HASNUM, int WAVES, bool MB, bool ONE = false, bool UNF = false>
__device__ __forceinline__ void rows_chain_body(const RowsRun& A, const int* __restrict__ ids, const float* __restrict__ dense,
                                                float* __restrict__ out, int B, int* __restrict__ err,
                                                const float* __restrict__ image, const RowsMany* __restrict__ Mp) {
    using LD = RowsLds<KPC, H0C, H1C, HASNUM, UNF>;
    using Set = typename std::conditional<UNF, RowsSetUnf<G_BIG, KPC, H0C>, RowsSet<G_BIG, KPC, H0C>>::type;
    static_assert(!UNF || (G_BIG <= 2 && KPC > 0), "UNF: two big fields are one K = 32 block");
    constexpr int KP = LD::KP, H0 = LD::H0;
    constexpr unsigned RB = LD::RB;
    constexpr bool HASFM = KPC > 0;
    static_assert(G_BIG >= 1 && G_BIG <= RC_MAX_BIG && NJF >= 0 && NJF <= RC_MAX_SMALL, "field split");
    const int tid = threadIdx.x;
    const int lane = tid & 63;
    const int wave = __builtin_amdgcn_readfirstlane(tid >> 6);
    const int r = lane & 15, q = lane >> 4;
    const f32x4 zero = f32x4{0.f, 0.f, 0.f, 0.f};
    const int m_n = MB ? Mp->n : 1, m_ntpb = MB ? Mp->ntpb : 0;
    const int ntasks = MB ? m_n * m_ntpb : (B + 15) >> 4;
    const int task_stride = gridDim.x * WAVES;
    const int wave_global = blockIdx.x * WAVES + wave;
    auto batch_of = [&](int tk, int& tl) {
        if constexpr (MB) {
            const int b = __builtin_amdgcn_readfirstlane(tk / m_ntpb);
            tl = tk - b * m_ntpb;
            return b;
        } else {
            tl = tk;
            return 0;
        }
    };
    float* stage = smem + LD::total_pad + wave * LD::stage_floats;
    const float* small_s = smem + LD::total_pad + WAVES * LD::stage_floats;
    const float* wq = smem + 4 * q;
    bool bad = false;
    const bool aligned = !(A.flags & 1);
    auto clampt = [&](int tk) { return tk < ntasks ? tk : ntasks - 1; };

    auto ld_raw = [&](int tkg, f32x4& raw) {
        int tk;
        const int bi = batch_of(tkg, tk);
        const int* ids_b = MB ? Mp->ids[bi] : ids;
        const float* dense_b = MB ? Mp->dense[bi] : dense;
        if (aligned && tk * 16 + 16 <= B) {
            const bool isid = lane < 32 || !HASNUM;
            const int j = lane < 32 ? lane : lane - 32;
            const int n4 = 4 * (isid ? A.F : A.ND);
            const float* src = isid ? reinterpret_cast<const float*>(ids_b) + (size_t)tk * 16 * A.F
                                    : dense_b + (size_t)tk * 16 * A.ND;
            raw = ld4(src + 4 * (j < n4 ? j : 0));
        }
    };
    auto gather = [&](int tkg, const f32x4& raw, Set& S) {
        int tk;
        const int bi = batch_of(tkg, tk);
        const int* ids_b = MB ? Mp->ids[bi] : ids;
        const float* dense_b = MB ? Mp->dense[bi] : dense;
        if (aligned && tk * 16 + 16 <= B) {
            const bool isid = lane < 32;
            const int j = isid ? lane : lane - 32;
            const int n4 = 4 * (isid ? A.F : (HASNUM ? A.ND : 0));
            if (j < n4) st4(stage + (isid ? 0 : 128) + 4 * j, raw);
        } else {
            stage_task_slow(stage, ids_b, dense_b, A.F, HASNUM ? A.ND : 0, tk, B, lane);
        }
        const int* sid_row = reinterpret_cast<const int*>(stage) + r * A.F;
        unsigned sid[G_BIG], rid[G_BIG];
#pragma unroll
        for (int b = 0; b < G_BIG; ++b) {
            const int id = sid_row[A.big_col[b]];
            bad |= (unsigned)(id + 1) > (unsigned)A.big_vocab[b];
            rid[b] = min((unsigned)id, (unsigned)A.big_vocab[b]);
            sid[b] = rid[b] + A.big_rowbase[b];
        }
#pragma unroll
        for (int f = 0; f < NJF; ++f) {
            const int id = sid_row[A.s_col[f]];
            bad |= (unsigned)(id + 1) > (unsigned)A.s_vocab[f];
            S.so[f] = A.s_off[f] + (int)min((unsigned)id, (unsigned)A.s_vocab[f]) * LD::SS;
        }
        if constexpr (HASNUM) {
            const float* nrow = stage + 128 + r * A.ND;
            const int last = A.n_num - 1;
            S.xa = nrow[min(q, last)];
            S.xb = nrow[min(q + 4, last)];
        }
        const char* tb = reinterpret_cast<const char*>(A.rows);
        if constexpr (UNF) {
            unsigned sq = sid[0];
            if (G_BIG > 1) sq = (q >> 1) ? sid[G_BIG > 1 ? 1 : 0] : sq;
            else sq = (q >> 1) ? (unsigned)A.big_vocab[0] + A.big_rowbase[0] : sq;
            const size_t ro = (size_t)sq * RB + 16u * (q & 1);
            S.ehi = *reinterpret_cast<const f16x8*>(tb + ro);
            S.elo = *reinterpret_cast<const f16x8*>(tb + ro + 32u);
        } else {
#pragma unroll
        for (int b = 0; b < G_BIG; ++b) {
            const size_t ro = (size_t)sid[b] * RB + 16u * q;
#pragma unroll
            for (int nb = 0; nb < KPC; ++nb) S.xp[b][nb] = *reinterpret_cast<const f32x4*>(tb + ro + 64u * nb);
#pragma unroll
            for (int n0 = 0; n0 < H0C; ++n0) S.xq[b][n0] = *reinterpret_cast<const f32x4*>(tb + ro + 4u * KP + 64u * n0);
        }
        }
        if constexpr (HASFM) {
            unsigned s0 = rid[0] + A.big_scal[0], s1 = rid[G_BIG > 1 ? 1 : 0] + A.big_scal[G_BIG > 1 ? 1 : 0],
                     s2 = rid[G_BIG > 2 ? 2 : 0] + A.big_scal[G_BIG > 2 ? 2 : 0];
            asm("" : "+v"(s0), "+v"(s1), "+v"(s2));
            unsigned so = s0;
            if (G_BIG > 1) so = q == 1 ? s1 : so;
            if (G_BIG > 2) so = q == 2 ? s2 : so;
            S.sc = A.scal[so];
        }
    };

    float rwna[HASFM && HASNUM ? KPC : 1], rwnb[HASFM && HASNUM ? KPC : 1];
    float rma[H0C], rmb[H0C];
    f32x4 rW1[H1C][H0C];
    float rfa = 0.f, rfb = 0.f;
    auto load_weights = [&]() {
        if constexpr (HASNUM) {
#pragma unroll
            for (int nb = 0; nb < KPC; ++nb) {
                rwna[nb] = smem[LD::off_wn + (nb * 16 + r) * LD::SN + q];
                rwnb[nb] = smem[LD::off_wn + (nb * 16 + r) * LD::SN + q + 4];
            }
#pragma unroll
            for (int n0 = 0; n0 < H0C; ++n0) {
                rma[n0] = smem[LD::off_m + (n0 * 16 + r) * LD::SN + q];
                rmb[n0] = smem[LD::off_m + (n0 * 16 + r) * LD::SN + q + 4];
            }
            rfa = smem[LD::off_fn + q];
            rfb = smem[LD::off_fn + q + 4];
        }
#pragma unroll
        for (int n1 = 0; n1 < H1C; ++n1)
#pragma unroll
            for (int j = 0; j < H0C; ++j) rW1[n1][j] = ld4(wq + LD::off_w1 + (n1 * 16 + r) * LD::S1 + 16 * j);
    };

    auto compute = [&](const Set& S) -> float {
#pragma clang fp contract(off)
        float zz = 0.f;
        f32x4 pn[HASFM ? KPC : 1], hp[H0C];
#pragma unroll
        for (int n0 = 0; n0 < H0C; ++n0) hp[n0] = ld4(wq + LD::off_c0 + n0 * 16);
        if constexpr (HASNUM) {
#pragma unroll
            for (int nb = 0; nb < KPC; ++nb) {
                pn[nb] = __builtin_amdgcn_mfma_f32_16x16x4f32(rwna[nb], S.xa, ld4(wq + LD::off_bn + nb * 16), 0, 0, 0);
            }
#pragma unroll
            for (int n0 = 0; n0 < H0C; ++n0) hp[n0] = __builtin_amdgcn_mfma_f32_16x16x4f32(rma[n0], S.xa, hp[n0], 0, 0, 0);
#pragma unroll
            for (int nb = 0; nb < KPC; ++nb) pn[nb] = __builtin_amdgcn_mfma_f32_16x16x4f32(rwnb[nb], S.xb, pn[nb], 0, 0, 0);
#pragma unroll
            for (int n0 = 0; n0 < H0C; ++n0) hp[n0] = __builtin_amdgcn_mfma_f32_16x16x4f32(rmb[n0], S.xb, hp[n0], 0, 0, 0);
            zz = fmaf(rfb, S.xb, rfa * S.xa);
        } else if constexpr (HASFM) {
#pragma unroll
            for (int nb = 0; nb < KPC; ++nb) pn[nb] = zero;
        }
        if constexpr (HASFM) zz += (q < G_BIG) ? S.sc : 0.f;
        f32x4 s[HASFM ? KPC : 1];
        f32x4 hq[H0C];
// ... 12 lines not shown
            }
        } else {
#pragma unroll
        for (int nb = 0; nb < KPC; ++nb) {
            s[nb] = S.xp[0][nb];
#pragma unroll
            for (int b = 1; b < G_BIG; ++b) s[nb] += S.xp[b][nb];
        }
#pragma unroll
        for (int n0 = 0; n0 < H0C; ++n0) {
            hq[n0] = S.xq[0][n0];
#pragma unroll
            for (int b = 1; b < G_BIG; ++b) hq[n0] += S.xq[b][n0];
        }
        }
        float ssc = 0.f;
#pragma unroll
        for (int f = 0; f < NJF; ++f) {
#pragma unroll
            for (int nb = 0; nb < KPC; ++nb) s[nb] += ld4(small_s + S.so[f] + 16 * nb + 4 * q);
#pragma unroll
            for (int n0 = 0; n0 < H0C; ++n0) hq[n0] += ld4(small_s + S.so[f] + KP + 16 * n0 + 4 * q);
            ssc += small_s[S.so[f] + KP + H0];
        }
        if (NJF > 0) zz += (q == 3) ? ssc : 0.f;
        float z = zz;
        if constexpr (HASFM) {
#pragma unroll
            for (int nb = 0; nb < KPC; ++nb) {
                const f32x4 t = s[nb] + pn[nb], u = pn[nb] * pn[nb];
                const f32x4 d = f32x4{fmaf(t.x, t.x, -u.x), fmaf(t.y, t.y, -u.y), fmaf(t.z, t.z, -u.z), fmaf(t.w, t.w, -u.w)};
                z = dot4_fma(ld4(wq + LD::off_hfm + nb * 16), d, z);
            }
        }
        f32x4 h0[H0C];
#pragma unroll
        for (int n0 = 0; n0 < H0C; ++n0) h0[n0] = relu4_fast(hp[n0] + hq[n0]);
#pragma unroll
        for (int n1 = 0; n1 < H1C; ++n1) {
            f32x4 e = ld4(wq + LD::off_b1 + n1 * 16), o = zero;
#pragma unroll
            for (int j = 0; j < H0C; ++j) {
                e = __builtin_amdgcn_mfma_f32_16x16x4f32(rW1[n1][j].x, h0[j].x, e, 0, 0, 0);
                o = __builtin_amdgcn_mfma_f32_16x16x4f32(rW1[n1][j].y, h0[j].y, o, 0, 0, 0);
                e = __builtin_amdgcn_mfma_f32_16x16x4f32(rW1[n1][j].z, h0[j].z, e, 0, 0, 0);
                o = __builtin_amdgcn_mfma_f32_16x16x4f32(rW1[n1][j].w, h0[j].w, o, 0, 0, 0);
            }
            z = dot4_fma(ld4(wq + LD::off_hd + n1 * 16), relu4_fast(e + o), z);
        }
        z += __shfl_xor(z, 16);
        z += __shfl_xor(z, 32);
        return sigmoidf_fast(z + A.bias);
    };
    auto store = [&](int tkg, float score) {
        int tk;
        const int bi = batch_of(tkg, tk);
        float* out_b = MB ? Mp->out[bi] : out;
        const int m = tk * 16 + r;
        if (q == 0 && m < B) out_b[m] = score;
    };

    Set SA, SB;
    f32x4 rawA = zero, rawB = zero;
    int tA = wave_global, tB = wave_global + task_stride;
    if (ntasks > 0) {
        if (!ONE || tA < ntasks) ld_raw(clampt(tA), rawA);
        if (!ONE) ld_raw(clampt(tB), rawB);
    }
#pragma unroll 1
    for (int c = wave; c < LD::total_pad / 256; c += WAVES) lds_dma16(image + c * 256 + lane * 4, smem + c * 256);
    if constexpr (NJF > 0) {
#pragma unroll 1
        for (int c = wave; c < A.small_floats / 256; c += WAVES) lds_dma16(A.small + c * 256 + lane * 4, smem + LD::total_pad + WAVES * LD::stage_floats + c * 256);
    }
    constexpr int NG = (UNF ? 2 : G_BIG * (KPC + H0C)) + (HASFM ? 1 : 0);
    constexpr int WAIT_NG = 0x0F70 | (NG & 15) | ((NG >> 4) << 14);
    static_assert(NG < 64, "vmcnt field");
    if constexpr (ONE) {
        if (tA < ntasks) {
            gather(tA, rawA, SA);
            __builtin_amdgcn_s_waitcnt(WAIT_NG);
        } else {
            __builtin_amdgcn_s_waitcnt(0x0F70);
        }
        __builtin_amdgcn_s_barrier();
        load_weights();
        if (tA < ntasks) store(tA, compute(SA));
    } else {
    constexpr bool FAST2 = NG < 16;
    const bool two = FAST2 && tA < ntasks && ntasks <= 2 * task_stride;
    if (two) {
        gather(tA, rawA, SA);
        __builtin_amdgcn_s_waitcnt(0x0F70 | (FAST2 ? NG : 0));
    } else {
        __builtin_amdgcn_s_waitcnt(0x0F70);
    }
    __builtin_amdgcn_s_barrier();
    load_weights();
    if (tA >= ntasks) {
    } else if (two) {
        gather(clampt(tB), rawB, SB);
        store(tA, compute(SA));
        if (tB < ntasks) store(tB, compute(SB));
    } else {
        gather(tA, rawA, SA);
        ld_raw(clampt(tA + 2 * task_stride), rawA);
        gather(clampt(tB), rawB, SB);
        ld_raw(clampt(tB + 2 * task_stride), rawB);
        for (;;) {
            store(tA, compute(SA));
            tA += 2 * task_stride;
            gather(clampt(tA), rawA, SA);
            ld_raw(clampt(tA + 2 * task_stride), rawA);
            if (tB >= ntasks) break;
            store(tB, compute(SB));
            tB += 2 * task_stride;
            gather(clampt(tB), rawB, SB);
            ld_raw(clampt(tB + 2 * task_stride), rawB);
            if (tA >= ntasks) break;
        }
    }
    }
    if (__ballot(bad) != 0 && lane == 0) atomicOr(err, 1);
}

template <int KPC, int H0C, int H1C, int G_BIG, int NJF, bool HASNUM, int WAVES, bool UNF = false>
__global__ __launch_bounds__(WAVES * 64, 2) void k_rows_chain(const RowsRun A, const int* __restrict__ ids,
                                                              const float* __restrict__ dense, float* __restrict__ out, int B,
                                                              int* __restrict__ err, const float* __restrict__ image) {
    rows_chain_body<KPC, H0C, H1C, G_BIG, NJF, HASNUM, WAVES, false, false, UNF>(A, ids, dense, out, B, err, image, nullptr);
}
template <int KPC, int H0C, int H1C, int G_BIG, int NJF, bool HASNUM, int WAVES, bool UNF = false>
__global__ __launch_bounds__(WAVES * 64, UNF ? 4 : 3) void k_rows_chain1(const RowsRun A, const int* __restrict__ ids,
                                                               const float* __restrict__ dense, float* __restrict__ out, int B,
                                                               int* __restrict__ err, const float* __restrict__ image) {
    rows_chain_body<KPC, H0C, H1C, G_BIG, NJF, HASNUM, WAVES, false, true, UNF>(A, ids, dense, out, B, err, image, nullptr);
}
template <int KPC, int H0C, int H1C, int G_BIG, int NJF, bool HASNUM, int WAVES, bool UNF = false>
__global__ __launch_bounds__(WAVES * 64, 2) void k_rows_chain_many(const RowsRun A, const RowsMany M, int B,
                                                                   int* __restrict__ err, const float* __restrict__ image) {
    rows_chain_body<KPC, H0C, H1C, G_BIG, NJF, HASNUM, WAVES, true, false, UNF>(A, nullptr, nullptr, nullptr, B, err, image, &M);
}
```

sparrowrecsys_amd/csrc/tu_instances.h:

```cpp
#ifndef SPRK_SINGLE_TU
#ifndef SPRK_TU_FAMILY
#define SPRK_TU_FAMILY 0
#endif
#if SPRK_TU_FAMILY == 1
#define SPRK_INST_1 template
#else
#define SPRK_INST_1 extern template
#endif
#if SPRK_TU_FAMILY == 2
#define SPRK_INST_2 template
#else
#define SPRK_INST_2 extern template
#endif
#if SPRK_TU_FAMILY == 3
#define SPRK_INST_3 template
#else
#define SPRK_INST_3 extern template
#endif
#if SPRK_TU_FAMILY == 4
#define SPRK_INST_4 template
#else
#define SPRK_INST_4 extern template
#endif
#if SPRK_TU_FAMILY == 5
#define SPRK_INST_5 template
#else
#define SPRK_INST_5 extern template
#endif
#if SPRK_TU_FAMILY == 6
#define SPRK_INST_6 template
#else
#define SPRK_INST_6 extern template
#endif
SPRK_INST_1 __global__ void sprk_dev::k_deepfm_v2_joint<1, 1, 1, 2, 1, 8, false>(sprk_dev::V2JRun, int const*, float const*, float*, int, int*, float const*);
SPRK_INST_1 __global__ void sprk_dev::k_deepfm_v2_joint<1, 1, 1, 2, 1, 8, true>(sprk_dev::V2JRun, int const*, float const*, float*, int, int*, float const*);
SPRK_INST_1 __global__ void sprk_dev::k_deepfm_v2_joint<1, 2, 1, 2, 1, 8, false>(sprk_dev::V2JRun, int const*, float const*, float*, int, int*, float const*);
SPRK_INST_1 __global__ void sprk_dev::k_deepfm_v2_joint<1, 2, 1, 2, 1, 8, true>(sprk_dev::V2JRun, int const*, float const*, float*, int, int*, float const*);
SPRK_INST_1 __global__ void sprk_dev::k_deepfm_v2_joint<1, 3, 1, 2, 1, 8, false>(sprk_dev::V2JRun, int const*, float const*, float*, int, int*, float const*);
SPRK_INST_1 __global__ void sprk_dev::k_deepfm_v2_joint<1, 3, 1, 2, 1, 8, true>(sprk_dev::V2JRun, int const*, float const*, float*, int, int*, float const*);
SPRK_INST_1 __global__ void sprk_dev::k_deepfm_v2_joint<2, 1, 1, 2, 1, 8, false>(sprk_dev::V2JRun, int const*, float const*, float*, int, int*, float const*);
SPRK_INST_1 __global__ void sprk_dev::k_deepfm_v2_joint<2, 1, 1, 2, 1, 8, true>(sprk_dev::V2JRun, int const*, float const*, float*, int, int*, float const*);
SPRK_INST_1 __global__ void sprk_dev::k_deepfm_v2_joint<2, 2, 1, 2, 1, 8, false>(sprk_dev::V2JRun, int const*, float const*, float*, int, int*, float const*);
SPRK_INST_1 __global__ void sprk_dev::k_deepfm_v2_joint<2, 2, 1, 2, 1, 8, true>(sprk_dev::V2JRun, int const*, float const*, float*, int, int*, float const*);
SPRK_INST_1 __global__ void sprk_dev::k_deepfm_v2_joint<2, 3, 1, 2, 1, 8, false>(sprk_dev::V2JRun, int const*, float const*, float*, int, int*, float const*);
SPRK_INST_1 __global__ void sprk_dev::k_deepfm_v2_joint<2, 3, 1, 2, 1, 8, true>(sprk_dev::V2JRun, int const*, float const*, float*, int, int*, float const*);
SPRK_INST_1 __global__ void sprk_dev::k_deepfm_v2_joint<3, 1, 1, 2, 1, 8, false>(sprk_dev::V2JRun, int const*, float const*, float*, int, int*, float const*);
SPRK_INST_1 __global__ void sprk_dev::k_deepfm_v2_joint<3, 1, 1, 2, 1, 8, true>(sprk_dev::V2JRun, int const*, float const*, float*, int, int*, float const*);
SPRK_INST_1 __global__ void sprk_dev::k_deepfm_v2_joint<3, 2, 1, 2, 1, 8, false>(sprk_dev::V2JRun, int const*, float const*, float*, int, int*, float const*);
SPRK_INST_1 __global__ void sprk_dev::k_deepfm_v2_joint<3, 2, 1, 2, 1, 8, true>(sprk_dev::V2JRun, int const*, float const*, float*, int, int*, float const*);
SPRK_INST_1 __global__ void sprk_dev::k_deepfm_v2_joint<3, 3, 1, 2, 1, 8, false>(sprk_dev::V2JRun, int const*, float const*, float*, int, int*, float const*);
SPRK_INST_1 __global__ void sprk_dev::k_deepfm_v2_joint<3, 3, 1, 2, 1, 8, true>(sprk_dev::V2JRun, int const*, float const*, float*, int, int*, float const*);
SPRK_INST_1 __global__ void sprk_dev::k_deepfm_v2_joint_many<1, 1, 1, 2, 1, 8, false>(sprk_dev::V2JRun, sprk_dev::V2JMany, int, int*, float const*);
SPRK_INST_1 __global__ void sprk_dev::k_deepfm_v2_joint_many<1, 1, 1, 2, 1, 8, true>(sprk_dev::V2JRun, sprk_dev::V2JMany, int, int*, float const*);
SPRK_INST_1 __global__ void sprk_dev::k_deepfm_v2_joint_many<1, 2, 1, 2, 1, 8, false>(sprk_dev::V2JRun, sprk_dev::V2JMany, int, int*, float const*);
SPRK_INST_1 __global__ void sprk_dev::k_deepfm_v2_joint_many<1, 2, 1, 2, 1, 8, true>(sprk_dev::V2JRun, sprk_dev::V2JMany, int, int*, float const*);
SPRK_INST_1 __global__ void sprk_dev::k_deepfm_v2_joint_many<1, 3, 1, 2, 1, 8, false>(sprk_dev::V2JRun, sprk_dev::V2JMany, int, int*, float const*);
SPRK_INST_1 __global__ void sprk_dev::k_deepfm_v2_joint_many<1, 3, 1, 2, 1, 8, true>(sprk_dev::V2JRun, sprk_dev::V2JMany, int, int*, float const*);
SPRK_INST_1 __global__ void sprk_dev::k_deepfm_v2_joint_many<2, 1, 1, 2, 1, 8, false>(sprk_dev::V2JRun, sprk_dev::V2JMany, int, int*, float const*);
SPRK_INST_1 __global__ void sprk_dev::k_deepfm_v2_joint_many<2, 1, 1, 2, 1, 8, true>(sprk_dev::V2JRun, sprk_dev::V2JMany, int, int*, float const*);
SPRK_INST_1 __global__ void sprk_dev::k_deepfm_v2_joint_many<2, 2, 1, 2, 1, 8, false>(sprk_dev::V2JRun, sprk_dev::V2JMany, int, int*, float const*);
SPRK_INST_1 __global__ void sprk_dev::k_deepfm_v2_joint_many<2, 2, 1, 2, 1, 8, true>(sprk_dev::V2JRun, sprk_dev::V2JMany, int, int*, float const*);
SPRK_INST_1 __global__ void sprk_dev::k_deepfm_v2_joint_many<2, 3, 1, 2, 1, 8, false>(sprk_dev::V2JRun, sprk_dev::V2JMany, int, int*, float const*);
SPRK_INST_1 __global__ void sprk_dev::k_deepfm_v2_joint_many<2, 3, 1, 2, 1, 8, true>(sprk_dev::V2JRun, sprk_dev::V2JMany, int, int*, float const*);
SPRK_INST_1 __global__ void sprk_dev::k_deepfm_v2_joint_many<3, 1, 1, 2, 1, 8, false>(sprk_dev::V2JRun, sprk_dev::V2JMany, int, int*, float const*);
SPRK_INST_1 __global__ void sprk_dev::k_deepfm_v2_joint_many<3, 1, 1, 2, 1, 8, true>(sprk_dev::V2JRun, sprk_dev::V2JMany, int, int*, float const*);
SPRK_INST_1 __global__ void sprk_dev::k_deepfm_v2_joint_many<3, 2, 1, 2, 1, 8, false>(sprk_dev::V2JRun, sprk_dev::V2JMany, int, int*, float const*);
SPRK_INST_1 __global__ void sprk_dev::k_deepfm_v2_joint_many<3, 2, 1, 2, 1, 8, true>(sprk_dev::V2JRun, sprk_dev::V2JMany, int, int*, float const*);
SPRK_INST_1 __global__ void sprk_dev::k_deepfm_v2_joint_many<3, 3, 1, 2, 1, 8, false>(sprk_dev::V2JRun, sprk_dev::V2JMany, int, int*, float const*);
SPRK_INST_1 __global__ void sprk_dev::k_deepfm_v2_joint_many<3, 3, 1, 2, 1, 8, true>(sprk_dev::V2JRun, sprk_dev::V2JMany, int, int*, float const*);
SPRK_INST_1 __global__ void sprk_dev::k_deepfm_v2_joint_many_tab<1, 1, 1, 2, 1, 8, false>(sprk_dev::V2JRun, sprk_dev::V2JManyTab, int, int*, float const*);
SPRK_INST_1 __global__ void sprk_dev::k_deepfm_v2_joint_many_tab<1, 1, 1, 2, 1, 8, true>(sprk_dev::V2JRun, sprk_dev::V2JManyTab, int, int*, float const*);
SPRK_INST_1 __global__ void sprk_dev::k_deepfm_v2_joint_many_tab<1, 2, 1, 2, 1, 8, false>(sprk_dev::V2JRun, sprk_dev::V2JManyTab, int, int*, float const*);
SPRK_INST_1 __global__ void sprk_dev::k_deepfm_v2_joint_many_tab<1, 2, 1, 2, 1, 8, true>(sprk_dev::V2JRun, sprk_dev::V2JManyTab, int, int*, float const*);
SPRK_INST_1 __global__ void sprk_dev::k_deepfm_v2_joint_many_tab<1, 3, 1, 2, 1, 8, false>(sprk_dev::V2JRun, sprk_dev::V2JManyTab, int, int*, float const*);
SPRK_INST_1 __global__ void sprk_dev::k_deepfm_v2_joint_many_tab<1, 3, 1, 2, 1, 8, true>(sprk_dev::V2JRun, sprk_dev::V2JManyTab, int, int*, float const*);
SPRK_INST_1 __global__ void sprk_dev::k_deepfm_v2_joint_many_tab<2, 1, 1, 2, 1, 8, false>(sprk_dev::V2JRun, sprk_dev::V2JManyTab, int, int*, float const*);
SPRK_INST_1 __global__ void sprk_dev::k_deepfm_v2_joint_many_tab<2, 1, 1, 2, 1, 8, true>(sprk_dev::V2JRun, sprk_dev::V2JManyTab, int, int*, float const*);
SPRK_INST_1 __global__ void sprk_dev::k_deepfm_v2_joint_many_tab<2, 2, 1, 2, 1, 8, false>(sprk_dev::V2JRun, sprk_dev::V2JManyTab, int, int*, float const*);
SPRK_INST_1 __global__ void sprk_dev::k_deepfm_v2_joint_many_tab<2, 2, 1, 2, 1, 8, true>(sprk_dev::V2JRun, sprk_dev::V2JManyTab, int, int*, float const*);
SPRK_INST_1 __global__ void sprk_dev::k_deepfm_v2_joint_many_tab<2, 3, 1, 2, 1, 8, false>(sprk_dev::V2JRun, sprk_dev::V2JManyTab, int, int*, float const*);
SPRK_INST_1 __global__ void sprk_dev::k_deepfm_v2_joint_many_tab<2, 3, 1, 2, 1, 8, true>(sprk_dev::V2JRun, sprk_dev::V2JManyTab, int, int*, float const*);
SPRK_INST_1 __global__ void sprk_dev::k_deepfm_v2_joint_many_tab<3, 1, 1, 2, 1, 8, false>(sprk_dev::V2JRun, sprk_dev::V2JManyTab, int, int*, float const*);
SPRK_INST_1 __global__ void sprk_dev::k_deepfm_v2_joint_many_tab<3, 1, 1, 2, 1, 8, true>(sprk_dev::V2JRun, sprk_dev::V2JManyTab, int, int*, float const*);
SPRK_INST_1 __global__ void sprk_dev::k_deepfm_v2_joint_many_tab<3, 2, 1, 2, 1, 8, false>(sprk_dev::V2JRun, sprk_dev::V2JManyTab, int, int*, float const*);
SPRK_INST_1 __global__ void sprk_dev::k_deepfm_v2_joint_many_tab<3, 2, 1, 2, 1, 8, true>(sprk_dev::V2JRun, sprk_dev::V2JManyTab, int, int*, float const*);
SPRK_INST_1 __global__ void sprk_dev::k_deepfm_v2_joint_many_tab<3, 3, 1, 2, 1, 8, false>(sprk_dev::V2JRun, sprk_dev::V2JManyTab, int, int*, float const*);
SPRK_INST_1 __global__ void sprk_dev::k_deepfm_v2_joint_many_tab<3, 3, 1, 2, 1, 8, true>(sprk_dev::V2JRun, sprk_dev::V2JManyTab, int, int*, float const*);
SPRK_INST_2 __global__ void sprk_dev::k_deepfm_v2_joint1<1, 1, false>(sprk_dev::V2JRun, int const*, float const*, float*, int, int*, float const*);
SPRK_INST_2 __global__ void sprk_dev::k_deepfm_v2_joint1<1, 1, true>(sprk_dev::V2JRun, int const*, float const*, float*, int, int*, float const*);
SPRK_INST_2 __global__ void sprk_dev::k_deepfm_v2_joint1<1, 2, false>(sprk_dev::V2JRun, int const*, float const*, float*, int, int*, float const*);
SPRK_INST_2 __global__ void sprk_dev::k_deepfm_v2_joint1<1, 2, true>(sprk_dev::V2JRun, int const*, float const*, float*, int, int*, float const*);
SPRK_INST_2 __global__ void sprk_dev::k_deepfm_v2_joint1<1, 3, false>(sprk_dev::V2JRun, int const*, float const*, float*, int, int*, float const*);
SPRK_INST_2 __global__ void sprk_dev::k_deepfm_v2_joint1<1, 3, true>(sprk_dev::V2JRun, int const*, float const*, float*, int, int*, float const*);
SPRK_INST_2 __global__ void sprk_dev::k_deepfm_v2_joint1<2, 1, false>(sprk_dev::V2JRun, int const*, float const*, float*, int, int*, float const*);
SPRK_INST_2 __global__ void sprk_dev::k_deepfm_v2_joint1<2, 1, true>(sprk_dev::V2JRun, int const*, float const*, float*, int, int*, float const*);
SPRK_INST_2 __global__ void sprk_dev::k_deepfm_v2_joint1<2, 2, false>(sprk_dev::V2JRun, int const*, float const*, float*, int, int*, float const*);
SPRK_INST_2 __global__ void sprk_dev::k_deepfm_v2_joint1<2, 2, true>(sprk_dev::V2JRun, int const*, float const*, float*, int, int*, float const*);
SPRK_INST_2 __global__ void sprk_dev::k_deepfm_v2_joint1<2, 3, false>(sprk_dev::V2JRun, int const*, float const*, float*, int, int*, float const*);
SPRK_INST_2 __global__ void sprk_dev::k_deepfm_v2_joint1<2, 3, true>(sprk_dev::V2JRun, int const*, float const*, float*, int, int*, float const*);
SPRK_INST_2 __global__ void sprk_dev::k_deepfm_v2_joint1<3, 1, false>(sprk_dev::V2JRun, int const*, float const*, float*, int, int*, float const*);
SPRK_INST_2 __global__ void sprk_dev::k_deepfm_v2_joint1<3, 1, true>(sprk_dev::V2JRun, int const*, float const*, float*, int, int*, float const*);
SPRK_INST_2 __global__ void sprk_dev::k_deepfm_v2_joint1<3, 2, false>(sprk_dev::V2JRun, int const*, float const*, float*, int, int*, float const*);
SPRK_INST_2 __global__ void sprk_dev::k_deepfm_v2_joint1<3, 2, true>(sprk_dev::V2JRun, int const*, float const*, float*, int, int*, float const*);
SPRK_INST_2 __global__ void sprk_dev::k_deepfm_v2_joint1<3, 3, false>(sprk_dev::V2JRun, int const*, float const*, float*, int, int*, float const*);
SPRK_INST_2 __global__ void sprk_dev::k_deepfm_v2_joint1<3, 3, true>(sprk_dev::V2JRun, int const*, float const*, float*, int, int*, float const*);
SPRK_INST_2 __global__ void sprk_dev::k_rows_chain<0, 1, 1, 2, 0, false, 8, false>(sprk_dev::RowsRun, int const*, float const*, float*, int, int*, float const*);
SPRK_INST_2 __global__ void sprk_dev::k_rows_chain<1, 2, 1, 3, 3, true, 8, false>(sprk_dev::RowsRun, int const*, float const*, float*, int, int*, float const*);
SPRK_INST_2 __global__ void sprk_dev::k_rows_chain<2, 2, 1, 2, 2, true, 8, false>(sprk_dev::RowsRun, int const*, float const*, float*, int, int*, float const*);
SPRK_INST_2 __global__ void sprk_dev::k_rows_chain<2, 2, 1, 2, 2, true, 8, true>(sprk_dev::RowsRun, int const*, float const*, float*, int, int*, float const*);
SPRK_INST_2 __global__ void sprk_dev::k_rows_chain<2, 2, 1, 3, 3, true, 8, false>(sprk_dev::RowsRun, int const*, float const*, float*, int, int*, float const*);
SPRK_INST_2 __global__ void sprk_dev::k_rows_chain<4, 2, 1, 1, 1, true, 8, false>(sprk_dev::RowsRun, int const*, float const*, float*, int, int*, float const*);
SPRK_INST_2 __global__ void sprk_dev::k_rows_chain<4, 2, 1, 1, 1, true, 8, true>(sprk_dev::RowsRun, int const*, float const*, float*, int, int*, float const*);
SPRK_INST_2 __global__ void sprk_dev::k_rows_chain<4, 2, 1, 2, 1, true, 8, false>(sprk_dev::RowsRun, int const*, float const*, float*, int, int*, float const*);
SPRK_INST_2 __global__ void sprk_dev::k_rows_chain<4, 2, 1, 2, 1, true, 8, true>(sprk_dev::RowsRun, int const*, float const*, float*, int, int*, float const*);
SPRK_INST_2 __global__ void sprk_dev::k_rows_chain<4, 2, 1, 2, 2, true, 8, false>(sprk_dev::RowsRun, int const*, float const*, float*, int, int*, float const*);
SPRK_INST_2 __global__ void sprk_dev::k_rows_chain<4, 2, 1, 2, 2, true, 8, true>(sprk_dev::RowsRun, int const*, float const*, float*, int, int*, float const*);
SPRK_INST_2 __global__ void sprk_dev::k_rows_chain<4, 2, 1, 3, 1, true, 8, false>(sprk_dev::RowsRun, int const*, float const*, float*, int, int*, float const*);
SPRK_INST_2 __global__ void sprk_dev::k_rows_chain<4, 2, 1, 3, 3, true, 8, false>(sprk_dev::RowsRun, int const*, float const*, float*, int, int*, float const*);
SPRK_INST_2 __global__ void sprk_dev::k_rows_chain1<0, 1, 1, 2, 0, false, 8, false>(sprk_dev::RowsRun, int const*, float const*, float*, int, int*, float const*);
SPRK_INST_2 __global__ void sprk_dev::k_rows_chain1<1, 2, 1, 3, 3, true, 8, false>(sprk_dev::RowsRun, int const*, float const*, float*, int, int*, float const*);
SPRK_INST_2 __global__ void sprk_dev::k_rows_chain1<2, 2, 1, 2, 2, true, 8, false>(sprk_dev::RowsRun, int const*, float const*, float*, int, int*, float const*);
SPRK_INST_2 __global__ void sprk_dev::k_rows_chain1<2, 2, 1, 2, 2, true, 8, true>(sprk_dev::RowsRun, int const*, float const*, float*, int, int*, float const*);
SPRK_INST_2 __global__ void sprk_dev::k_rows_chain1<2, 2, 1, 3, 3, true, 8, false>(sprk_dev::RowsRun, int const*, float const*, float*, int, int*, float const*);
SPRK_INST_2 __global__ void sprk_dev::k_rows_chain1<4, 2, 1, 1, 1, true, 8, false>(sprk_dev::RowsRun, int const*, float const*, float*, int, int*, float const*);
SPRK_INST_2 __global__ void sprk_dev::k_rows_chain1<4, 2, 1, 1, 1, true, 8, true>(sprk_dev::RowsRun, int const*, float const*, float*, int, int*, float const*);
SPRK_INST_2 __global__ void sprk_dev::k_rows_chain1<4, 2, 1, 2, 1, true, 8, false>(sprk_dev::RowsRun, int const*, float const*, float*, int, int*, float const*);
SPRK_INST_2 __global__ void sprk_dev::k_rows_chain1<4, 2, 1, 2, 1, true, 8, true>(sprk_dev::RowsRun, int const*, float const*, float*, int, int*, float const*);
SPRK_INST_2 __global__ void sprk_dev::k_rows_chain1<4, 2, 1, 2, 2, true, 8, false>(sprk_dev::RowsRun, int const*, float const*, float*, int, int*, float const*);
SPRK_INST_2 __global__ void sprk_dev::k_rows_chain1<4, 2, 1, 2, 2, true, 8, true>(sprk_dev::RowsRun, int const*, float const*, float*, int, int*, float const*);
SPRK_INST_2 __global__ void sprk_dev::k_rows_chain1<4, 2, 1, 3, 1, true, 8, false>(sprk_dev::RowsRun, int const*, float const*, float*, int, int*, float const*);
SPRK_INST_2 __global__ void sprk_dev::k_rows_chain1<4, 2, 1, 3, 3, true, 8, false>(sprk_dev::RowsRun, int const*, float const*, float*, int, int*, float const*);
SPRK_INST_2 __global__ void sprk_dev::k_rows_chain_many<0, 1, 1, 2, 0, false, 8, false>(sprk_dev::RowsRun, sprk_dev::RowsMany, int, int*, float const*);
SPRK_INST_2 __global__ void sprk_dev::k_rows_chain_many<1, 2, 1, 3, 3, true, 8, false>(sprk_dev::RowsRun, sprk_dev::RowsMany, int, int*, float const*);
SPRK_INST_2 __global__ void sprk_dev::k_rows_chain_many<2, 2, 1, 2, 2, true, 8, false>(sprk_dev::RowsRun, sprk_dev::RowsMany, int, int*, float const*);
SPRK_INST_2 __global__ void sprk_dev::k_rows_chain_many<2, 2, 1, 2, 2, true, 8, true>(sprk_dev::RowsRun, sprk_dev::RowsMany, int, int*, float const*);
SPRK_INST_2 __global__ void sprk_dev::k_rows_chain_many<2, 2, 1, 3, 3, true, 8, false>(sprk_dev::RowsRun, sprk_dev::RowsMany, int, int*, float const*);
SPRK_INST_2 __global__ void sprk_dev::k_rows_chain_many<4, 2, 1, 1, 1, true, 8, false>(sprk_dev::RowsRun, sprk_dev::RowsMany, int, int*, float const*);
SPRK_INST_2 __global__ void sprk_dev::k_rows_chain_many<4, 2, 1, 1, 1, true, 8, true>(sprk_dev::RowsRun, sprk_dev::RowsMany, int, int*, float const*);
SPRK_INST_2 __global__ void sprk_dev::k_rows_chain_many<4, 2, 1, 2, 1, true, 8, false>(sprk_dev::RowsRun, sprk_dev::RowsMany, int, int*, float const*);
SPRK_INST_2 __global__ void sprk_dev::k_rows_chain_many<4, 2, 1, 2, 1, true, 8, true>(sprk_dev::RowsRun, sprk_dev::RowsMany, int, int*, float const*);
SPRK_INST_2 __global__ void sprk_dev::k_rows_chain_many<4, 2, 1, 2, 2, true, 8, false>(sprk_dev::RowsRun, sprk_dev::RowsMany, int, int*, float const*);
SPRK_INST_2 __global__ void sprk_dev::k_rows_chain_many<4, 2, 1, 2, 2, true, 8, true>(sprk_dev::RowsRun, sprk_dev::RowsMany, int, int*, float const*);
SPRK_INST_2 __global__ void sprk_dev::k_rows_chain_many<4, 2, 1, 3, 1, true, 8, false>(sprk_dev::RowsRun, sprk_dev::RowsMany, int, int*, float const*);
SPRK_INST_2 __global__ void sprk_dev::k_rows_chain_many<4, 2, 1, 3, 3, true, 8, false>(sprk_dev::RowsRun, sprk_dev::RowsMany, int, int*, float const*);
SPRK_INST_2 __global__ void sprk_dev::k_v2_pack_image<2, 4, 1, 2, 1, true>(sprk_dev::V2Args, float*);
SPRK_INST_2 __global__ void sprk_dev::k_v2_pack_image<3, 4, 1, 2, 1, true>(sprk_dev::V2Args, float*);
SPRK_INST_2 __global__ void sprk_dev::k_v2_pack_image<4, 4, 1, 2, 1, true>(sprk_dev::V2Args, float*);
SPRK_INST_2 __global__ void sprk_dev::k_v2_pack_image<5, 4, 1, 2, 1, true>(sprk_dev::V2Args, float*);
SPRK_INST_2 __global__ void sprk_dev::k_v2_pack_image<6, 4, 1, 2, 1, true>(sprk_dev::V2Args, float*);
SPRK_INST_3 __global__ void sprk_dev::k_deepfm_pairs<4, 16, 4, 4, 8, false, false>(sprk_dev::V1Run, int const*, float const*, float*, int, int*);
SPRK_INST_3 __global__ void sprk_dev::k_deepfm_pairs<4, 16, 4, 4, 8, false, true>(sprk_dev::V1Run, int const*, float const*, float*, int, int*);
SPRK_INST_3 __global__ void sprk_dev::k_deepfm_pairs<4, 16, 4, 4, 8, true, false>(sprk_dev::V1Run, int const*, float const*, float*, int, int*);
SPRK_INST_3 __global__ void sprk_dev::k_deepfm_pairs<4, 16, 4, 4, 8, true, true>(sprk_dev::V1Run, int const*, float const*, float*, int, int*);
SPRK_INST_3 __global__ void sprk_dev::k_deepfm_pairs<4, 3, 4, 4, 8, false, false>(sprk_dev::V1Run, int const*, float const*, float*, int, int*);
SPRK_INST_3 __global__ void sprk_dev::k_deepfm_pairs<4, 3, 4, 4, 8, false, true>(sprk_dev::V1Run, int const*, float const*, float*, int, int*);
SPRK_INST_3 __global__ void sprk_dev::k_deepfm_pairs<4, 3, 4, 4, 8, true, false>(sprk_dev::V1Run, int const*, float const*, float*, int, int*);
SPRK_INST_3 __global__ void sprk_dev::k_deepfm_pairs<4, 3, 4, 4, 8, true, true>(sprk_dev::V1Run, int const*, float const*, float*, int, int*);
SPRK_INST_3 __global__ void sprk_dev::k_deepfm_pairs<4, 4, 4, 4, 8, false, false>(sprk_dev::V1Run, int const*, float const*, float*, int, int*);
SPRK_INST_3 __global__ void sprk_dev::k_deepfm_pairs<4, 4, 4, 4, 8, false, true>(sprk_dev::V1Run, int const*, float const*, float*, int, int*);
SPRK_INST_3 __global__ void sprk_dev::k_deepfm_pairs<4, 4, 4, 4, 8, true, false>(sprk_dev::V1Run, int const*, float const*, float*, int, int*);
SPRK_INST_3 __global__ void sprk_dev::k_deepfm_pairs<4, 4, 4, 4, 8, true, true>(sprk_dev::V1Run, int const*, float const*, float*, int, int*);
SPRK_INST_3 __global__ void sprk_dev::k_deepfm_pairs<6, 4, 4, 4, 8, false, false>(sprk_dev::V1Run, int const*, float const*, float*, int, int*);
SPRK_INST_3 __global__ void sprk_dev::k_deepfm_pairs<6, 4, 4, 4, 8, false, true>(sprk_dev::V1Run, int const*, float const*, float*, int, int*);
SPRK_INST_3 __global__ void sprk_dev::k_deepfm_pairs<6, 4, 4, 4, 8, true, false>(sprk_dev::V1Run, int const*, float const*, float*, int, int*);
SPRK_INST_3 __global__ void sprk_dev::k_deepfm_pairs<6, 4, 4, 4, 8, true, true>(sprk_dev::V1Run, int const*, float const*, float*, int, int*);
SPRK_INST_3 __global__ void sprk_dev::k_deepfm_pairs1<4, 3, 4, 4, 8, false>(sprk_dev::V1Run, int const*, float const*, float*, int, int*);
SPRK_INST_3 __global__ void sprk_dev::k_deepfm_pairs1<4, 3, 4, 4, 8, true>(sprk_dev::V1Run, int const*, float const*, float*, int, int*);
SPRK_INST_3 __global__ void sprk_dev::k_deepfm_pairs1<4, 4, 4, 4, 8, false>(sprk_dev::V1Run, int const*, float const*, float*, int, int*);
SPRK_INST_3 __global__ void sprk_dev::k_deepfm_pairs1<4, 4, 4, 4, 8, true>(sprk_dev::V1Run, int const*, float const*, float*, int, int*);
SPRK_INST_3 __global__ void sprk_dev::k_deepfm_pairs1<6, 4, 4, 4, 8, false>(sprk_dev::V1Run, int const*, float const*, float*, int, int*);
SPRK_INST_3 __global__ void sprk_dev::k_deepfm_pairs1<6, 4, 4, 4, 8, true>(sprk_dev::V1Run, int const*, float const*, float*, int, int*);
SPRK_INST_3 __global__ void sprk_dev::k_deepfm_pairs_many<4, 16, 4, 4, 8, false, false>(sprk_dev::V1Run, sprk_dev::V1Many, int, int*);
SPRK_INST_3 __global__ void sprk_dev::k_deepfm_pairs_many<4, 16, 4, 4, 8, false, true>(sprk_dev::V1Run, sprk_dev::V1Many, int, int*);
SPRK_INST_3 __global__ void sprk_dev::k_deepfm_pairs_many<4, 16, 4, 4, 8, true, false>(sprk_dev::V1Run, sprk_dev::V1Many, int, int*);
SPRK_INST_3 __global__ void sprk_dev::k_deepfm_pairs_many<4, 16, 4, 4, 8, true, true>(sprk_dev::V1Run, sprk_dev::V1Many, int, int*);
SPRK_INST_3 __global__ void sprk_dev::k_deepfm_pairs_many<4, 3, 4, 4, 8, false, false>(sprk_dev::V1Run, sprk_dev::V1Many, int, int*);
SPRK_INST_3 __global__ void sprk_dev::k_deepfm_pairs_many<4, 3, 4, 4, 8, false, true>(sprk_dev::V1Run, sprk_dev::V1Many, int, int*);
SPRK_INST_3 __global__ void sprk_dev::k_deepfm_pairs_many<4, 3, 4, 4, 8, true, false>(sprk_dev::V1Run, sprk_dev::V1Many, int, int*);
SPRK_INST_3 __global__ void sprk_dev::k_deepfm_pairs_many<4, 3, 4, 4, 8, true, true>(sprk_dev::V1Run, sprk_dev::V1Many, int, int*);
SPRK_INST_3 __global__ void sprk_dev::k_deepfm_pairs_many<4, 4, 4, 4, 8, false, false>(sprk_dev::V1Run, sprk_dev::V1Many, int, int*);
SPRK_INST_3 __global__ void sprk_dev::k_deepfm_pairs_many<4, 4, 4, 4, 8, false, true>(sprk_dev::V1Run, sprk_dev::V1Many, int, int*);
SPRK_INST_3 __global__ void sprk_dev::k_deepfm_pairs_many<4, 4, 4, 4, 8, true, false>(sprk_dev::V1Run, sprk_dev::V1Many, int, int*);
SPRK_INST_3 __global__ void sprk_dev::k_deepfm_pairs_many<4, 4, 4, 4, 8, true, true>(sprk_dev::V1Run, sprk_dev::V1Many, int, int*);
SPRK_INST_3 __global__ void sprk_dev::k_deepfm_pairs_many<6, 4, 4, 4, 8, false, false>(sprk_dev::V1Run, sprk_dev::V1Many, int, int*);
SPRK_INST_3 __global__ void sprk_dev::k_deepfm_pairs_many<6, 4, 4, 4, 8, false, true>(sprk_dev::V1Run, sprk_dev::V1Many, int, int*);
SPRK_INST_3 __global__ void sprk_dev::k_deepfm_pairs_many<6, 4, 4, 4, 8, true, false>(sprk_dev::V1Run, sprk_dev::V1Many, int, int*);
SPRK_INST_3 __global__ void sprk_dev::k_deepfm_pairs_many<6, 4, 4, 4, 8, true, true>(sprk_dev::V1Run, sprk_dev::V1Many, int, int*);
SPRK_INST_3 __global__ void sprk_dev::k_v1_pack_image<4, 4, 1>(sprk_dev::V1Run, float*);
SPRK_INST_3 __global__ void sprk_dev::k_v1_pack_image<4, 4, 4>(sprk_dev::V1Run, float*);
SPRK_INST_4 __global__ void sprk_dev::k_dien_fused<10, 32, 8, 4>(sprk_dev::DienRun, sprk_dev::DinTailRun, int const*, float const*, float*, int, int*, float const*, float*);
SPRK_INST_4 __global__ void sprk_dev::k_dien_fused<16, 32, 8, 4>(sprk_dev::DienRun, sprk_dev::DinTailRun, int const*, float const*, float*, int, int*, float const*, float*);
SPRK_INST_4 __global__ void sprk_dev::k_dien_mfma_pack<10, 32>(float const*, unsigned int const*, float*, int);
SPRK_INST_4 __global__ void sprk_dev::k_dien_mfma_pack<16, 32>(float const*, unsigned int const*, float*, int);
SPRK_INST_4 __global__ void sprk_dev::k_dien_seq<10, 32>(sprk_dev::DienRun, int const*, float*, int, int*);
SPRK_INST_4 __global__ void sprk_dev::k_dien_seq<16, 32>(sprk_dev::DienRun, int const*, float*, int, int*);
SPRK_INST_4 __global__ void sprk_dev::k_dien_seq_mfma<10, 32>(sprk_dev::DienRun, int const*, float*, int, int*);
SPRK_INST_4 __global__ void sprk_dev::k_dien_seq_mfma<16, 32>(sprk_dev::DienRun, int const*, float*, int, int*);
SPRK_INST_4 __global__ void sprk_dev::k_din_attn_cols<1, false>(sprk_dev::DinColsRun, int const*, float*, float*, int, int*, sprk_dev::DinColsArg<false>::type);
SPRK_INST_4 __global__ void sprk_dev::k_din_attn_cols<1, true>(sprk_dev::DinColsRun, int const*, float*, float*, int, int*, sprk_dev::DinColsArg<true>::type);
SPRK_INST_4 __global__ void sprk_dev::k_din_attn_cols<2, false>(sprk_dev::DinColsRun, int const*, float*, float*, int, int*, sprk_dev::DinColsArg<false>::type);
SPRK_INST_4 __global__ void sprk_dev::k_din_attn_cols<2, true>(sprk_dev::DinColsRun, int const*, float*, float*, int, int*, sprk_dev::DinColsArg<true>::type);
SPRK_INST_4 __global__ void sprk_dev::k_din_tail<4, 2, 1, 16, true, false, true>(sprk_dev::DinTailRun, int const*, float const*, float const*, float*, int, int*, float const*, sprk_dev::DinTailMany);
SPRK_INST_4 __global__ void sprk_dev::k_din_tail<4, 2, 1, 16, true, true, true>(sprk_dev::DinTailRun, int const*, float const*, float const*, float*, int, int*, float const*, sprk_dev::DinTailMany);
SPRK_INST_4 __global__ void sprk_dev::k_din_tail<4, 2, 1, 8, false, false, false>(sprk_dev::DinTailRun, int const*, float const*, float const*, float*, int, int*, float const*, sprk_dev::DinTailMany);
SPRK_INST_4 __global__ void sprk_dev::k_din_tail<4, 2, 1, 8, false, true, false>(sprk_dev::DinTailRun, int const*, float const*, float const*, float*, int, int*, float const*, sprk_dev::DinTailMany);
SPRK_INST_4 __global__ void sprk_dev::k_din_tail<4, 2, 1, 8, true, false, false>(sprk_dev::DinTailRun, int const*, float const*, float const*, float*, int, int*, float const*, sprk_dev::DinTailMany);
SPRK_INST_4 __global__ void sprk_dev::k_din_tail<4, 2, 1, 8, true, true, false>(sprk_dev::DinTailRun, int const*, float const*, float const*, float*, int, int*, float const*, sprk_dev::DinTailMany);
SPRK_INST_4 __global__ void sprk_dev::k_din_tail<4, 2, 2, 8, false, false, false>(sprk_dev::DinTailRun, int const*, float const*, float const*, float*, int, int*, float const*, sprk_dev::DinTailMany);
SPRK_INST_4 __global__ void sprk_dev::k_din_tail<4, 2, 2, 8, false, true, false>(sprk_dev::DinTailRun, int const*, float const*, float const*, float*, int, int*, float const*, sprk_dev::DinTailMany);
SPRK_INST_4 __global__ void sprk_dev::k_din_tail<4, 2, 2, 8, true, false, false>(sprk_dev::DinTailRun, int const*, float const*, float const*, float*, int, int*, float const*, sprk_dev::DinTailMany);
SPRK_INST_4 __global__ void sprk_dev::k_din_tail<4, 2, 2, 8, true, false, true>(sprk_dev::DinTailRun, int const*, float const*, float const*, float*, int, int*, float const*, sprk_dev::DinTailMany);
SPRK_INST_4 __global__ void sprk_dev::k_din_tail<4, 2, 2, 8, true, true, false>(sprk_dev::DinTailRun, int const*, float const*, float const*, float*, int, int*, float const*, sprk_dev::DinTailMany);
SPRK_INST_4 __global__ void sprk_dev::k_din_tail<4, 2, 2, 8, true, true, true>(sprk_dev::DinTailRun, int const*, float const*, float const*, float*, int, int*, float const*, sprk_dev::DinTailMany);
SPRK_INST_4 __global__ void sprk_dev::k_din_tail<8, 4, 1, 16, true, false, true>(sprk_dev::DinTailRun, int const*, float const*, float const*, float*, int, int*, float const*, sprk_dev::DinTailMany);
SPRK_INST_4 __global__ void sprk_dev::k_din_tail<8, 4, 1, 16, true, true, true>(sprk_dev::DinTailRun, int const*, float const*, float const*, float*, int, int*, float const*, sprk_dev::DinTailMany);
SPRK_INST_4 __global__ void sprk_dev::k_din_tail<8, 4, 1, 8, false, false, false>(sprk_dev::DinTailRun, int const*, float const*, float const*, float*, int, int*, float const*, sprk_dev::DinTailMany);
SPRK_INST_4 __global__ void sprk_dev::k_din_tail<8, 4, 1, 8, false, true, false>(sprk_dev::DinTailRun, int const*, float const*, float const*, float*, int, int*, float const*, sprk_dev::DinTailMany);
SPRK_INST_4 __global__ void sprk_dev::k_din_tail<8, 4, 1, 8, true, false, false>(sprk_dev::DinTailRun, int const*, float const*, float const*, float*, int, int*, float const*, sprk_dev::DinTailMany);
SPRK_INST_4 __global__ void sprk_dev::k_din_tail<8, 4, 1, 8, true, true, false>(sprk_dev::DinTailRun, int const*, float const*, float const*, float*, int, int*, float const*, sprk_dev::DinTailMany);
SPRK_INST_4 __global__ void sprk_dev::k_din_tail<8, 4, 2, 8, false, false, false>(sprk_dev::DinTailRun, int const*, float const*, float const*, float*, int, int*, float const*, sprk_dev::DinTailMany);
SPRK_INST_4 __global__ void sprk_dev::k_din_tail<8, 4, 2, 8, false, true, false>(sprk_dev::DinTailRun, int const*, float const*, float const*, float*, int, int*, float const*, sprk_dev::DinTailMany);
SPRK_INST_4 __global__ void sprk_dev::k_din_tail<8, 4, 2, 8, true, false, false>(sprk_dev::DinTailRun, int const*, float const*, float const*, float*, int, int*, float const*, sprk_dev::DinTailMany);
SPRK_INST_4 __global__ void sprk_dev::k_din_tail<8, 4, 2, 8, true, false, true>(sprk_dev::DinTailRun, int const*, float const*, float const*, float*, int, int*, float const*, sprk_dev::DinTailMany);
SPRK_INST_4 __global__ void sprk_dev::k_din_tail<8, 4, 2, 8, true, true, false>(sprk_dev::DinTailRun, int const*, float const*, float const*, float*, int, int*, float const*, sprk_dev::DinTailMany);
SPRK_INST_4 __global__ void sprk_dev::k_din_tail<8, 4, 2, 8, true, true, true>(sprk_dev::DinTailRun, int const*, float const*, float const*, float*, int, int*, float const*, sprk_dev::DinTailMany);
SPRK_INST_4 __global__ void sprk_dev::k_din_tail_pack<4, 2, 1>(float const*, int, int, int, int, int, float const*, float const*, float const*, int, float const*, float const*, float const*, int, float const*, float*, float const*, float const*);
SPRK_INST_4 __global__ void sprk_dev::k_din_tail_pack<4, 2, 2>(float const*, int, int, int, int, int, float const*, float const*, float const*, int, float const*, float const*, float const*, int, float const*, float*, float const*, float const*);
SPRK_INST_4 __global__ void sprk_dev::k_din_tail_pack<8, 4, 1>(float const*, int, int, int, int, int, float const*, float const*, float const*, int, float const*, float const*, float const*, int, float const*, float*, float const*, float const*);
SPRK_INST_4 __global__ void sprk_dev::k_din_tail_pack<8, 4, 2>(float const*, int, int, int, int, int, float const*, float const*, float const*, int, float const*, float const*, float const*, int, float const*, float*, float const*, float const*);
SPRK_INST_5 __global__ void sprk_dev::k_din_fused<1, false, false, false>(sprk_dev::DinFusedRun, int const*, float const*, float*, float*, int, int*, sprk_dev::DinFusedArg<false>::type);
SPRK_INST_5 __global__ void sprk_dev::k_din_fused<1, false, false, true>(sprk_dev::DinFusedRun, int const*, float const*, float*, float*, int, int*, sprk_dev::DinFusedArg<false>::type);
SPRK_INST_5 __global__ void sprk_dev::k_din_fused<1, false, true, false>(sprk_dev::DinFusedRun, int const*, float const*, float*, float*, int, int*, sprk_dev::DinFusedArg<false>::type);
SPRK_INST_5 __global__ void sprk_dev::k_din_fused<1, true, false, false>(sprk_dev::DinFusedRun, int const*, float const*, float*, float*, int, int*, sprk_dev::DinFusedArg<true>::type);
SPRK_INST_5 __global__ void sprk_dev::k_din_fused<1, true, true, false>(sprk_dev::DinFusedRun, int const*, float const*, float*, float*, int, int*, sprk_dev::DinFusedArg<true>::type);
SPRK_INST_5 __global__ void sprk_dev::k_din_fused<2, false, false, false>(sprk_dev::DinFusedRun, int const*, float const*, float*, float*, int, int*, sprk_dev::DinFusedArg<false>::type);
SPRK_INST_5 __global__ void sprk_dev::k_din_fused<2, false, false, true>(sprk_dev::DinFusedRun, int const*, float const*, float*, float*, int, int*, sprk_dev::DinFusedArg<false>::type);
SPRK_INST_5 __global__ void sprk_dev::k_din_fused<2, false, true, false>(sprk_dev::DinFusedRun, int const*, float const*, float*, float*, int, int*, sprk_dev::DinFusedArg<false>::type);
SPRK_INST_5 __global__ void sprk_dev::k_din_fused<2, true, false, false>(sprk_dev::DinFusedRun, int const*, float const*, float*, float*, int, int*, sprk_dev::DinFusedArg<true>::type);
SPRK_INST_5 __global__ void sprk_dev::k_din_fused<2, true, true, false>(sprk_dev::DinFusedRun, int const*, float const*, float*, float*, int, int*, sprk_dev::DinFusedArg<true>::type);
SPRK_INST_6 __global__ void sprk_dev::k_mlp_rows<8, 8, 1, -1, 8, false, 0>(sprk_dev::MlpRowsRun, int const*, float const*, float*, int, int*, float const*);
// ... 27 lines not shown
```

Measured before the change: 17.17 billion.

## Extend device batch-table single-launch path to rows and pairs routes

Generalizes the V2Joint batch-pointer table path into a shared helper and adds table-driven many-batch kernels for the rows-chain and DeepFM pairs routes. When there are more batches than fit in one kernel argument struct, a single launch now reads per-batch pointers from a device table instead of issuing many grouped launches. This is meant to cut launch count and host overhead, at the cost of a host-to-device table copy when pointers change and an extra indirection per task in the kernels.

```diff
diff --git a/sparrowrecsys_amd/csrc/api_forward.h b/sparrowrecsys_amd/csrc/api_forward.h
--- a/sparrowrecsys_amd/csrc/api_forward.h
+++ b/sparrowrecsys_amd/csrc/api_forward.h
@@ -212,28 +212,27 @@
         if (!ok(i)) return false;
     return true;
 }
-}
-
-static int launch_v2j_table(sprk_handle h, int32_t n_batches, const int32_t* const* ids, const float* const* dense, float* const* out, int32_t B,
-                            hipStream_t st, bool* done) {
+template <class GridOf, class Launch>
+static int launch_batch_table(sprk_handle h, int32_t n_batches, const int32_t* const* ids, const float* const* dense, float* const* out, int32_t B,
+                              hipStream_t st, int waves, int look, GridOf grid_of, Launch launch, bool* done) {
     *done = false;
     const int ntpb = (B + 15) / 16;
-    long long grid = ((long long)n_batches * ntpb + V2_WAVES - 1) / V2_WAVES;
-    if (grid > h->v2_grid_cap) grid = h->v2_grid_cap;
-    if ((long long)n_batches * ntpb + 4 * grid * V2_WAVES >= (1LL << 31)) return SPRK_OK;
+    const long long grid = grid_of((long long)n_batches * ntpb);
+    if ((long long)n_batches * ntpb + look * grid * waves >= (1LL << 31)) return SPRK_OK;
     hipStreamCaptureStatus cap = hipStreamCaptureStatusNone;
     if (hipStreamIsCapturing(st, &cap) != hipSuccess) { (void)hipGetLastError(); return SPRK_OK; }
     if (cap != hipStreamCaptureStatusNone) return SPRK_OK;
     const size_t n = (size_t)n_batches;
-    int slot = h->v2j_table_last;
-    bool same = slot >= 0 && h->v2j_table[slot].n == n && h->v2j_table[slot].stream == st;
+    auto dense_of = [&](size_t i) -> const float* { return dense ? dense[i] : nullptr; };
+    int slot = h->batch_table_last;
+    bool same = slot >= 0 && h->batch_table[slot].n == n && h->batch_table[slot].stream == st;
     if (same) {
-        const V2JBatch* last = h->v2j_table[slot].stage;
-        for (size_t i = 0; i < n && same; ++i) same = last[i].ids == ids[i] && last[i].dense == dense[i] && last[i].out == out[i];
+        const ManyBatch* last = h->batch_table[slot].stage;
+        for (size_t i = 0; i < n && same; ++i) same = last[i].ids == ids[i] && last[i].dense == dense_of(i) && last[i].out == out[i];
     }
     if (!same) {
-        slot = h->v2j_table_last == 0 ? 1 : 0;
-        sprk_engine::V2JTable& t = h->v2j_table[slot];
+        slot = h->batch_table_last == 0 ? 1 : 0;
+        sprk_engine::BatchTable& t = h->batch_table[slot];
         if (!t.busy) HIP_TRY(hipEventCreateWithFlags(&t.busy, hipEventDisableTiming));
         if (t.used) HIP_TRY(hipEventSynchronize(t.busy));
         if (t.cap < n) {
@@ -242,27 +241,25 @@
             if (t.stage) (void)hipHostFree(t.stage);
             if (t.dev) (void)hipFree(t.dev);
             t.stage = nullptr; t.dev = nullptr; t.cap = 0; t.n = 0;
-            HIP_TRY(hipHostMalloc((void**)&t.stage, want * sizeof(V2JBatch), hipHostMallocDefault));
-            HIP_TRY(hipMalloc((void**)&t.dev, want * sizeof(V2JBatch)));
+            HIP_TRY(hipHostMalloc((void**)&t.stage, want * sizeof(ManyBatch), hipHostMallocDefault));
+            HIP_TRY(hipMalloc((void**)&t.dev, want * sizeof(ManyBatch)));
             t.cap = want;
         }
         t.n = 0;
-        for (size_t i = 0; i < n; ++i) t.stage[i] = V2JBatch{ids[i], dense[i], out[i], nullptr};
-        HIP_TRY(hipMemcpyAsync(t.dev, t.stage, n * sizeof(V2JBatch), hipMemcpyHostToDevice, st));
+        for (size_t i = 0; i < n; ++i) t.stage[i] = ManyBatch{ids[i], dense_of(i), out[i], nullptr};
+        HIP_TRY(hipMemcpyAsync(t.dev, t.stage, n * sizeof(ManyBatch), hipMemcpyHostToDevice, st));
         t.n = n;
         t.stream = st;
-        h->v2j_table_last = slot;
-    }
-    sprk_engine::V2JTable& t = h->v2j_table[slot];
-    V2JRun jr = h->v2j_run;
-    jr.flags = 0;
-    const V2JManyTab m = {t.dev, n_batches, ntpb};
-    hipLaunchKernelGGL(kV2JVariants[h->v2j_variant].fn_many_tab, dim3((int)grid), dim3(V2_WAVES * 64), h->v2j_lds_bytes, st, jr, m, B, h->dev_err, h->v2_image);
+        h->batch_table_last = slot;
+    }
+    sprk_engine::BatchTable& t = h->batch_table[slot];
+    launch(ManyTab{t.dev, n_batches, ntpb}, (int)grid);
     HIP_TRY(hipGetLastError());
     HIP_TRY(hipEventRecord(t.busy, st));
     t.used = true;
     *done = true;
     return SPRK_OK;
+}
 }
 
 static int forward_many_impl(sprk_handle h, int32_t n_batches, const int32_t* const* ids, const float* const* dense,
@@ -290,7 +287,12 @@
         jr.flags = 0;
         if (n_batches > many_batches) {
             bool done = false;
-            SPRK_TRY(launch_v2j_table(h, n_batches, ids, dense, out, B, st, &done));
+            SPRK_TRY(launch_batch_table(h, n_batches, ids, dense, out, B, st, V2_WAVES, 4,
+                                        [&](long long tasks) { const long long g = (tasks + V2_WAVES - 1) / V2_WAVES; return g > h->v2_grid_cap ? (long long)h->v2_grid_cap : g; },
+                                        [&](const ManyTab& m, int grid) {
+                                            hipLaunchKernelGGL(jv.fn_many_tab, dim3(grid), dim3(V2_WAVES * 64), h->v2j_lds_bytes, st, jr, m, B, h->dev_err, h->v2_image);
+                                        },
+                                        &done));
             if (done) return SPRK_OK;
         }
         return launch_groups<V2JMany>(n_batches, many_batches, ids, dense, out, [&](V2JMany& m, int) {
@@ -307,7 +309,18 @@
         const RowsVariant& rv = kRowsVariants[h->rows_variant];
         RowsRun rr = h->rows_run;
         rr.flags = 0;
-        return launch_groups<RowsMany>(n_batches, many_batches < RC_MB ? many_batches : RC_MB, ids, rows_dense, out, [&](RowsMany& m, int) {
+        const int per = many_batches < RC_MB ? many_batches : RC_MB;
+        auto cus = [&](long long tasks) { const long long g = (tasks + RC_WAVES - 1) / RC_WAVES; return g > h->num_cus ? (long long)h->num_cus : g; };
+        if (n_batches > per) {
+            bool done = false;
+            SPRK_TRY(launch_batch_table(h, n_batches, ids, rows_dense, out, B, st, RC_WAVES, 4, cus,
+                                        [&](const ManyTab& m, int grid) {
+                                            hipLaunchKernelGGL(rv.fn_many_tab, dim3(grid), dim3(RC_WAVES * 64), h->rows_lds_bytes, st, rr, m, B, h->dev_err, h->rows_image);
+                                        },
+                                        &done));
+            if (done) return SPRK_OK;
+        }
+        return launch_groups<RowsMany>(n_batches, per, ids, rows_dense, out, [&](RowsMany& m, int) {
             m.ntpb = ntpb;
             long long grid = ((long long)m.n * ntpb + RC_WAVES - 1) / RC_WAVES;
             if (grid > h->num_cus) grid = h->num_cus;
@@ -329,7 +342,18 @@
     }
     if (grouped && dense && h->route == Route::Pairs && every_batch(n_batches, present)) {
         const size_t lds = kV1Variants[h->v1_variant].lds_bytes;
-        return launch_groups<V1Many>(n_batches, many_batches < V1_MB ? many_batches : V1_MB, ids, dense, out, [&](V1Many& m, int) {
+        const int per = many_batches < V1_MB ? many_batches : V1_MB;
+        if (n_batches > per) {
+            bool done = false;
+            SPRK_TRY(launch_batch_table(h, n_batches, ids, dense, out, B, st, V1_WAVES, 2,
+                                        [&](long long tasks) { const long long g = (tasks + V1_WAVES - 1) / V1_WAVES; return g > h->num_cus ? (long long)h->num_cus : g; },
+                                        [&](const ManyTab& m, int grid) {
+                                            hipLaunchKernelGGL(h->v1_many_tab_kernel, dim3(grid), dim3(V1_WAVES * 64), lds, st, h->v1_run, m, B, h->dev_err);
+                                        },
+                                        &done));
+            if (done) return SPRK_OK;
+        }
+        return launch_groups<V1Many>(n_batches, per, ids, dense, out, [&](V1Many& m, int) {
             m.ntpb = ntpb;
             long long grid = ((long long)m.n * ntpb + V1_WAVES - 1) / V1_WAVES;
             if (grid > h->num_cus) grid = h->num_cus;
@@ -529,7 +553,7 @@
     for (size_t i = 0; i < h->slot_ptr.size(); ++i) free_slot(h, i);
     for (const sprk_engine::DevAlloc& a : h->allocs) release(a);
     if (h->v2j_tab) (void)hipFree(h->v2j_tab);
-    for (sprk_engine::V2JTable& t : h->v2j_table) {
+    for (sprk_engine::BatchTable& t : h->batch_table) {
         if (t.used) (void)hipEventSynchronize(t.busy);
         if (t.stage) (void)hipHostFree(t.stage);
         if (t.dev) (void)hipFree(t.dev);
diff --git a/sparrowrecsys_amd/csrc/host_engine.h b/sparrowrecsys_amd/csrc/host_engine.h
--- a/sparrowrecsys_amd/csrc/host_engine.h
+++ b/sparrowrecsys_amd/csrc/host_engine.h
@@ -3,11 +3,13 @@
 
 typedef void (*V2JKernel)(const V2JRun, const int*, const float*, float*, int, int*, const float*);
 typedef void (*V2JManyKernel)(const V2JRun, const V2JMany, int, int*, const float*);
-typedef void (*V2JManyTabKernel)(const V2JRun, const V2JManyTab, int, int*, const float*);
+typedef void (*V2JManyTabKernel)(const V2JRun, const ManyTab, int, int*, const float*);
 typedef void (*RowsKernel)(const RowsRun, const int*, const float*, float*, int, int*, const float*);
 typedef void (*RowsManyKernel)(const RowsRun, const RowsMany, int, int*, const float*);
+typedef void (*RowsManyTabKernel)(const RowsRun, const ManyTab, int, int*, const float*);
 typedef void (*V1Kernel)(const V1Run, const int*, const float*, float*, int, int*);
 typedef void (*V1ManyKernel)(const V1Run, const V1Many, int, int*);
+typedef void (*V1ManyTabKernel)(const V1Run, const ManyTab, int, int*);
 typedef void (*MlpRowsKernel)(const MlpRowsRun, const int*, const float*, float*, int, int*, const float*);
 typedef void (*MlpRowsManyKernel)(const MlpRowsRun, const MlpRowsMany, int, int*, const float*);
 typedef void (*DinTailKernel)(const DinTailRun, const int*, const float*, const float*, float*, int, int*, const float*, const DinTailMany);
@@ -49,6 +51,7 @@
     V1Kernel v1_kernel = nullptr;
     V1Kernel v1_one_kernel = nullptr;
     V1ManyKernel v1_many_kernel = nullptr;
+    V1ManyTabKernel v1_many_tab_kernel = nullptr;
     V1Run v1_run;
     int mlp_rows_nbig = -1;
     MlpRowsRun mlp_rows_run;
@@ -113,17 +116,17 @@
     float* v2j_tab = nullptr;
     size_t v2j_lds_bytes = 0;
     float* v2j_big = nullptr;
-    struct V2JTable {
-        V2JBatch* stage = nullptr;
-        V2JBatch* dev = nullptr;
+    struct BatchTable {
+        ManyBatch* stage = nullptr;
+        ManyBatch* dev = nullptr;
         size_t cap = 0;
         size_t n = 0;
         hipStream_t stream = nullptr;
         hipEvent_t busy = nullptr;
         bool used = false;
     };
-    V2JTable v2j_table[2];
-    int v2j_table_last = -1;
+    BatchTable batch_table[2];
+    int batch_table_last = -1;
     struct DevAlloc { void* p; size_t vmm_size; hipMemGenericAllocationHandle_t handle; };
     std::vector<DevAlloc> allocs;
 };
diff --git a/sparrowrecsys_amd/csrc/host_setup_pairs.h b/sparrowrecsys_amd/csrc/host_setup_pairs.h
--- a/sparrowrecsys_amd/csrc/host_setup_pairs.h
+++ b/sparrowrecsys_amd/csrc/host_setup_pairs.h
@@ -5,12 +5,14 @@
     bool sep;
     V1Kernel fn_dyn, fn_f32, fn_one;
     V1ManyKernel fn_many_dyn, fn_many_f32;
+    V1ManyTabKernel fn_many_tab_dyn, fn_many_tab_f32;
     void (*pack)(const V1Run, float*);
     size_t lds_bytes;
 };
 #define V1_VARIANT(NF, NV, SEP, ONE)                                                                                                    \
     {NF, NV, SEP, &k_deepfm_pairs<NF, NV, 4, 4, V1_WAVES, true, SEP>, &k_deepfm_pairs<NF, NV, 4, 4, V1_WAVES, false, SEP>, ONE,         \
      &k_deepfm_pairs_many<NF, NV, 4, 4, V1_WAVES, true, SEP>, &k_deepfm_pairs_many<NF, NV, 4, 4, V1_WAVES, false, SEP>,                 \
+     &k_deepfm_pairs_many_tab<NF, NV, 4, 4, V1_WAVES, true, SEP>, &k_deepfm_pairs_many_tab<NF, NV, 4, 4, V1_WAVES, false, SEP>,         \
      &k_v1_pack_image<4, 4, (NV + 3) / 4>, V1Lds<4, 4, (NV + 3) / 4>::bytes}
 #define V1_ONE(NF, NV, SEP) &k_deepfm_pairs1<NF, NV, 4, 4, V1_WAVES, SEP>
 #define V1_BOTH(NF, NV) V1_VARIANT(NF, NV, true, V1_ONE(NF, NV, true)), V1_VARIANT(NF, NV, false, V1_ONE(NF, NV, false))
@@ -241,9 +243,11 @@
     const bool dyn = r.inv_w1_scale != 0.f;
     h->v1_kernel = dyn ? vv.fn_dyn : vv.fn_f32;
     h->v1_many_kernel = dyn ? vv.fn_many_dyn : vv.fn_many_f32;
+    h->v1_many_tab_kernel = dyn ? vv.fn_many_tab_dyn : vv.fn_many_tab_f32;
     h->v1_one_kernel = (r.tab && r.w1frag && PC == 1 && h->tune.v1_one) ? vv.fn_one : nullptr;
     SPRK_TRY(set_max_lds(h->v1_kernel, vv.lds_bytes));
     SPRK_TRY(set_max_lds(h->v1_many_kernel, vv.lds_bytes));
+    SPRK_TRY(set_max_lds(h->v1_many_tab_kernel, vv.lds_bytes));
     if (h->v1_one_kernel) SPRK_TRY(set_max_lds(h->v1_one_kernel, vv.lds_bytes));
     h->v1_run = r;
     h->v1_variant = variant;
diff --git a/sparrowrecsys_amd/csrc/host_setup_rows.h b/sparrowrecsys_amd/csrc/host_setup_rows.h
--- a/sparrowrecsys_amd/csrc/host_setup_rows.h
+++ b/sparrowrecsys_amd/csrc/host_setup_rows.h
@@ -10,12 +10,14 @@
     bool unf;
     RowsKernel fn;
     RowsManyKernel fn_many;
+    RowsManyTabKernel fn_many_tab;
     RowsKernel fn_one;
     RowsLayout ld;
 };
 #define ROWS_VARIANT_X(KPC, H0C, H1C, G_BIG, NJF, HASNUM, UNF)                                                                   \
     {KPC, H0C, H1C, G_BIG, NJF, HASNUM, UNF, &k_rows_chain<KPC, H0C, H1C, G_BIG, NJF, HASNUM, RC_WAVES, UNF>,                    \
-     &k_rows_chain_many<KPC, H0C, H1C, G_BIG, NJF, HASNUM, RC_WAVES, UNF>, &k_rows_chain1<KPC, H0C, H1C, G_BIG, NJF, HASNUM, RC_WAVES, UNF>, \
+     &k_rows_chain_many<KPC, H0C, H1C, G_BIG, NJF, HASNUM, RC_WAVES, UNF>,                                                      \
+     &k_rows_chain_many_tab<KPC, H0C, H1C, G_BIG, NJF, HASNUM, RC_WAVES, UNF>, &k_rows_chain1<KPC, H0C, H1C, G_BIG, NJF, HASNUM, RC_WAVES, UNF>, \
      rows_layout<RowsLds<KPC, H0C, H1C, HASNUM, UNF>>()}
 #define ROWS_VARIANT(KPC, H0C, H1C, G_BIG, NJF, HASNUM) ROWS_VARIANT_X(KPC, H0C, H1C, G_BIG, NJF, HASNUM, false)
 const RowsVariant kRowsVariants[] = {
@@ -47,6 +49,7 @@
     if (h->rows_lds_bytes > 160 * 1024) return fail(SPRK_EINVAL, "rows chain needs %zu bytes of LDS", h->rows_lds_bytes);
     SPRK_TRY(set_max_lds(rv.fn, h->rows_lds_bytes));
     SPRK_TRY(set_max_lds(rv.fn_many, h->rows_lds_bytes));
+    SPRK_TRY(set_max_lds(rv.fn_many_tab, h->rows_lds_bytes));
     SPRK_TRY(set_max_lds(rv.fn_one, h->rows_lds_bytes));
     HIP_TRY(hipDeviceSynchronize());
     return SPRK_OK;
diff --git a/sparrowrecsys_amd/csrc/k_chain_v1.h b/sparrowrecsys_amd/csrc/k_chain_v1.h
--- a/sparrowrecsys_amd/csrc/k_chain_v1.h
+++ b/sparrowrecsys_amd/csrc/k_chain_v1.h
@@ -69,6 +69,10 @@
     float* out[V1_MB];
     int n, ntpb;
 };
+struct V1One {};
+__device__ __forceinline__ const int* many_ids(const V1Many& m, int b) { return m.ids[b]; }
+__device__ __forceinline__ const float* many_dense(const V1Many& m, int b) { return m.dense[b]; }
+__device__ __forceinline__ float* many_out(const V1Many& m, int b) { return m.out[b]; }
 
 template <int H0C, int H1C, int PC = 1>
 struct V1Lds {
@@ -120,11 +124,13 @@
     f32x4 x[NR][PC];
     float xa, xb;
     float w1a, w1b;
+    float* dst;
 };
 
-template <int NF, int NV, int H0C, int H1C, int WAVES, bool DYN, bool MB, bool SEP, bool ONE = false>
+template <int NF, int NV, int H0C, int H1C, int WAVES, bool DYN, class Many, bool SEP, bool ONE = false>
 __device__ __forceinline__ void v1_body(const V1Run& A, const int* __restrict__ ids0, const float* __restrict__ dense0,
-                                        float* __restrict__ out0, int B, int* __restrict__ err, const V1Many* __restrict__ Mp) {
+                                        float* __restrict__ out0, int B, int* __restrict__ err, const Many* __restrict__ Mp) {
+    constexpr bool MB = !std::is_same<Many, V1One>::value;
     constexpr int PC = (NV + 3) / 4;
     constexpr int NR = NF + (SEP ? V1_MAX_DEEP : 0);
     constexpr int DB = SEP ? NF : 0;
@@ -137,33 +143,37 @@
     const int wave = __builtin_amdgcn_readfirstlane(tid >> 6);
     const int r = lane & 15, q = lane >> 4;
     const f32x4 zero = f32x4{0.f, 0.f, 0.f, 0.f};
-    const int m_ntpb = MB ? Mp->ntpb : 0;
-    const int ntasks = MB ? Mp->n * m_ntpb : (B + 15) >> 4;
+    int m_ntpb = 0, ntasks = (B + 15) >> 4;
+    if constexpr (MB) { m_ntpb = Mp->ntpb; ntasks = Mp->n * m_ntpb; }
     const int task_stride = gridDim.x * WAVES;
     bool bad = false;
-    auto batch_of = [&](int t, int& tl) {
-        if constexpr (MB) {
-            const int b = __builtin_amdgcn_readfirstlane(t / m_ntpb);
-            tl = t - b * m_ntpb;
-            return b;
-        } else {
-            tl = t;
-            return 0;
-        }
+    auto batch_of = [&](int t) -> int {
+        if constexpr (MB) return __builtin_amdgcn_readfirstlane(t / m_ntpb);
+        else return 0;
     };
-    auto ld_ids = [&](int tg, int (&idv)[NF]) {
-        int t;
-        const int bi = batch_of(tg, t);
-        const int* ids = MB ? Mp->ids[bi] : ids0;
+    auto in_batch = [&](int t, int b) -> int { return MB ? t - b * m_ntpb : t; };
+    auto ld_ids = [&](int tg, int (&idv)[NF]) -> int {
+        const int bi = batch_of(tg);
+        const int t = in_batch(tg, bi);
+        const int* ids = ids0;
+        if constexpr (MB) ids = many_ids(*Mp, bi);
         const int m = min(t * 16 + r, B - 1);
         const int* row = ids + (size_t)m * A.F;
 #pragma unroll
         for (int f = 0; f < NF; ++f) idv[f] = row[A.col[f]];
+        return bi;
     };
-    auto issue_gather = [&](int tg, const int (&idv)[NF], Set& S) {
-        int t;
-        const int bi = batch_of(tg, t);
-        const float* dense = MB ? Mp->dense[bi] : dense0;
+    auto issue_gather = [&](int tg, int bi, const int (&idv)[NF], Set& S) {
+        const int t = in_batch(tg, bi);
+        const float* dense = dense0;
+        if constexpr (MB) {
+            dense = many_dense(*Mp, bi);
+            float* out_b = many_out(*Mp, bi);
+            const int mo = t * 16 + r;
+            S.dst = (q == 0 && mo < B) ? out_b + mo : nullptr;
+        } else {
+            S.dst = nullptr;
+        }
         const int m = min(t * 16 + r, B - 1);
         {
             const float* nrow = dense + (size_t)m * A.ND;
@@ -377,33 +387,35 @@
         z = rows4_sum(z);
         return sigmoidf_acc(z + A.head_bias);
     };
-    auto store = [&](int tg, float score) {
-        int tl;
-        const int bo = batch_of(tg, tl);
-        float* out = MB ? Mp->out[bo] : out0;
-        const int mm = tl * 16 + r;
-        if (q == 0 && mm < B) out[mm] = score;
+    auto store = [&](int tg, const Set& S, float score) {
+        if constexpr (MB) {
+            if (S.dst) *(__attribute__((address_space(1))) float*)(uintptr_t)S.dst = score;
+        } else {
+            const int mm = tg * 16 + r;
+            if (q == 0 && mm < B) out0[mm] = score;
+        }
     };
 
     int tA = blockIdx.x * WAVES + wave, tB = tA + task_stride;
     int idA[NF], idB[NF];
 #pragma unroll
     for (int f = 0; f < NF; ++f) { idA[f] = -1; idB[f] = -1; }
-    if (tA < ntasks) ld_ids(tA, idA);
-    if (!ONE && tB < ntasks) ld_ids(tB, idB);
+    int nA = 0, nB = 0;
+    if (tA < ntasks) nA = ld_ids(tA, idA);
+    if (!ONE && tB < ntasks) nB = ld_ids(tB, idB);
 #pragma unroll 1
     for (int c = wave; c < LD::total_pad / 256; c += WAVES) lds_dma16(A.image + c * 256 + lane * 4, smem + c * 256);
     Set SA, SB;
     if constexpr (ONE) {
         __builtin_amdgcn_s_waitcnt(0x0F70);
         __builtin_amdgcn_s_barrier();
-        if (tA < ntasks) issue_gather(tA, idA, SA);
+        if (tA < ntasks) issue_gather(tA, nA, idA, SA);
 #pragma unroll
         for (int nb = 0; nb < H0C; ++nb) {
             rna[nb] = smem[LD::off_w0n + (nb * 16 + r) * 8 + q];
             rnb[nb] = smem[LD::off_w0n + (nb * 16 + r) * 8 + q + 4];
         }
-        if (tA < ntasks) store(tA, compute(SA));
+        if (tA < ntasks) store(tA, SA, compute(SA));
     } else {
     __builtin_amdgcn_s_waitcnt(0x0F70);
     __builtin_amdgcn_s_barrier();
@@ -414,19 +426,19 @@
     }
     if (tA >= ntasks) {
     } else if (PC == 1 && ntasks <= 2 * task_stride) {
-        issue_gather(tA, idA, SA);
-        if (tB < ntasks) issue_gather(tB, idB, SB);
-        store(tA, compute(SA));
-        if (tB < ntasks) store(tB, compute(SB));
+        issue_gather(tA, nA, idA, SA);
+        if (tB < ntasks) issue_gather(tB, nB, idB, SB);
+        store(tA, SA, compute(SA));
+        if (tB < ntasks) store(tB, SB, compute(SB));
     } else {
-        issue_gather(tA, idA, SA);
+        issue_gather(tA, nA, idA, SA);
         for (int tk = tA; tk < ntasks; tk += task_stride) {
             const Set cur = SA;
             if (tk + task_stride < ntasks) {
-                issue_gather(tk + task_stride, idB, SA);
-                if (tk + 2 * task_stride < ntasks) ld_ids(tk + 2 * task_stride, idB);
-            }
-            store(tk, compute(cur));
+                issue_gather(tk + task_stride, nB, idB, SA);
+                if (tk + 2 * task_stride < ntasks) nB = ld_ids(tk + 2 * task_stride, idB);
+            }
+            store(tk, cur, compute(cur));
         }
     }
     }
@@ -436,14 +448,18 @@
 template <int NF, int NV, int H0C, int H1C, int WAVES, bool DYN, bool SEP>
 __global__ __launch_bounds__(WAVES * 64, 2) void k_deepfm_pairs(const V1Run A, const int* __restrict__ ids, const float* __restrict__ dense,
                                                                 float* __restrict__ out, int B, int* __restrict__ err) {
-    v1_body<NF, NV, H0C, H1C, WAVES, DYN, false, SEP>(A, ids, dense, out, B, err, nullptr);
+    v1_body<NF, NV, H0C, H1C, WAVES, DYN, V1One, SEP>(A, ids, dense, out, B, err, nullptr);
 }
 template <int NF, int NV, int H0C, int H1C, int WAVES, bool DYN, bool SEP>
 __global__ __launch_bounds__(WAVES * 64, 2) void k_deepfm_pairs_many(const V1Run A, const V1Many M, int B, int* __restrict__ err) {
-    v1_body<NF, NV, H0C, H1C, WAVES, DYN, true, SEP>(A, nullptr, nullptr, nullptr, B, err, &M);
+    v1_body<NF, NV, H0C, H1C, WAVES, DYN, V1Many, SEP>(A, nullptr, nullptr, nullptr, B, err, &M);
+}
+template <int NF, int NV, int H0C, int H1C, int WAVES, bool DYN, bool SEP>
+__global__ __launch_bounds__(WAVES * 64, 2) void k_deepfm_pairs_many_tab(const V1Run A, const ManyTab M, int B, int* __restrict__ err) {
+    v1_body<NF, NV, H0C, H1C, WAVES, DYN, ManyTab, SEP>(A, nullptr, nullptr, nullptr, B, err, &M);
 }
 template <int NF, int NV, int H0C, int H1C, int WAVES, bool SEP>
 __global__ __launch_bounds__(WAVES * 64, 4) void k_deepfm_pairs1(const V1Run A, const int* __restrict__ ids, const float* __restrict__ dense,
                                                                  float* __restrict__ out, int B, int* __restrict__ err) {
-    v1_body<NF, NV, H0C, H1C, WAVES, true, false, SEP, true>(A, ids, dense, out, B, err, nullptr);
-}
+    v1_body<NF, NV, H0C, H1C, WAVES, true, V1One, SEP, true>(A, ids, dense, out, B, err, nullptr);
+}
diff --git a/sparrowrecsys_amd/csrc/k_chain_v2j.h b/sparrowrecsys_amd/csrc/k_chain_v2j.h
--- a/sparrowrecsys_amd/csrc/k_chain_v2j.h
+++ b/sparrowrecsys_amd/csrc/k_chain_v2j.h
@@ -29,25 +29,25 @@
     int n;
     int ntpb;
 };
-struct V2JBatch {
+struct ManyBatch {
     const int* ids;
     const float* dense;
     float* out;
     void* pad_;
 };
-struct V2JManyTab {
-    const V2JBatch* batch;
+struct ManyTab {
+    const ManyBatch* batch;
     int n;
     int ntpb;
 };
 struct V2JOne {};
-__device__ __forceinline__ const int* v2j_ids(const V2JMany& m, int b) { return m.ids[b]; }
-__device__ __forceinline__ const float* v2j_dense(const V2JMany& m, int b) { return m.dense[b]; }
-__device__ __forceinline__ float* v2j_out(const V2JMany& m, int b) { return m.out[b]; }
-typedef const __attribute__((address_space(4))) V2JBatch* V2JBatchCP;
-__device__ __forceinline__ const int* v2j_ids(const V2JManyTab& m, int b) { return ((V2JBatchCP)(uintptr_t)m.batch + b)->ids; }
-__device__ __forceinline__ const float* v2j_dense(const V2JManyTab& m, int b) { return ((V2JBatchCP)(uintptr_t)m.batch + b)->dense; }
-__device__ __forceinline__ float* v2j_out(const V2JManyTab& m, int b) { return ((V2JBatchCP)(uintptr_t)m.batch + b)->out; }
+__device__ __forceinline__ const int* many_ids(const V2JMany& m, int b) { return m.ids[b]; }
+__device__ __forceinline__ const float* many_dense(const V2JMany& m, int b) { return m.dense[b]; }
+__device__ __forceinline__ float* many_out(const V2JMany& m, int b) { return m.out[b]; }
+typedef const __attribute__((address_space(4))) ManyBatch* ManyBatchCP;
+__device__ __forceinline__ const int* many_ids(const ManyTab& m, int b) { return ((ManyBatchCP)(uintptr_t)m.batch + b)->ids; }
+__device__ __forceinline__ const float* many_dense(const ManyTab& m, int b) { return ((ManyBatchCP)(uintptr_t)m.batch + b)->dense; }
+__device__ __forceinline__ float* many_out(const ManyTab& m, int b) { return ((ManyBatchCP)(uintptr_t)m.batch + b)->out; }
 
 __device__ __forceinline__ void split_half4(f32x4 w, float scale, f16x4& hi, f16x4& lo) {
 #pragma unroll
@@ -206,7 +206,7 @@
         const int tk = in_batch(tkg, b);
         const int* ids_b = ids;
         const float* dense_b = dense;
-        if constexpr (MB) { ids_b = v2j_ids(*Mp, b); dense_b = v2j_dense(*Mp, b); }
+        if constexpr (MB) { ids_b = many_ids(*Mp, b); dense_b = many_dense(*Mp, b); }
         if (aligned && tk * 16 + 16 <= B) {
             const bool isid = lane < 32;
             const int j = isid ? lane : lane - 32;
@@ -227,7 +227,7 @@
         } else {
             const int* ids_b = ids;
             const float* dense_b = dense;
-            if constexpr (MB) { ids_b = v2j_ids(*Mp, b); dense_b = v2j_dense(*Mp, b); }
+            if constexpr (MB) { ids_b = many_ids(*Mp, b); dense_b = many_dense(*Mp, b); }
             stage_task_slow(stage, ids_b, dense_b, A.F, A.ND, tk, B, lane);
         }
         const int* sid_row = reinterpret_cast<const int*>(stage) + r * A.F;
@@ -271,7 +271,7 @@
         {
             float* out_b;
             if constexpr (MB) {
-                out_b = v2j_out(*Mp, b);
+                out_b = many_out(*Mp, b);
                 asm("" : "+s"(out_b));
             } else {
                 out_b = out;
@@ -502,7 +502,7 @@
     v2j_body<G_BIG, NJF, KPC, H0C, H1C, WAVES, HALF, V2JMany>(A, nullptr, nullptr, nullptr, B, err, image, &M);
 }
 template <int G_BIG, int NJF, int KPC, int H0C, int H1C, int WAVES, bool HALF>
-__global__ __launch_bounds__(WAVES * 64, 2) void k_deepfm_v2_joint_many_tab(const V2JRun A, const V2JManyTab M, int B, int* __restrict__ err,
+__global__ __launch_bounds__(WAVES * 64, 2) void k_deepfm_v2_joint_many_tab(const V2JRun A, const ManyTab M, int B, int* __restrict__ err,
                                                                             const float* __restrict__ image) {
-    v2j_body<G_BIG, NJF, KPC, H0C, H1C, WAVES, HALF, V2JManyTab>(A, nullptr, nullptr, nullptr, B, err, image, &M);
-}
+    v2j_body<G_BIG, NJF, KPC, H0C, H1C, WAVES, HALF, ManyTab>(A, nullptr, nullptr, nullptr, B, err, image, &M);
+}
diff --git a/sparrowrecsys_amd/csrc/k_rows_chain.h b/sparrowrecsys_amd/csrc/k_rows_chain.h
--- a/sparrowrecsys_amd/csrc/k_rows_chain.h
+++ b/sparrowrecsys_amd/csrc/k_rows_chain.h
@@ -26,6 +26,10 @@
     float* out[RC_MB];
     int n, ntpb;
 };
+struct RowsOne {};
+__device__ __forceinline__ const int* many_ids(const RowsMany& m, int b) { return m.ids[b]; }
+__device__ __forceinline__ const float* many_dense(const RowsMany& m, int b) { return m.dense[b]; }
+__device__ __forceinline__ float* many_out(const RowsMany& m, int b) { return m.out[b]; }
 
 template <int KPC, int H0C, int H1C, bool HASNUM, bool UNF = false>
 struct RowsLds {
@@ -113,6 +117,7 @@
     int so[RC_MAX_SMALL];
     float xa, xb;
     float sc;
+    float* dst;
 };
 
 template <int G_BIG, int KPC, int H0C>
@@ -122,6 +127,7 @@
     int so[RC_MAX_SMALL];
     float xa, xb;
     float sc;
+    float* dst;
 };
 
 __device__ __forceinline__ float dot4_fma(f32x4 a, f32x4 b, float acc) {
@@ -131,10 +137,11 @@
     return fmaf(a.w, b.w, acc);
 }
 
-template <int KPC, int H0C, int H1C, int G_BIG, int NJF, bool HASNUM, int WAVES, bool MB, bool ONE = false, bool UNF = false>
+template <int KPC, int H0C, int H1C, int G_BIG, int NJF, bool HASNUM, int WAVES, class Many, bool ONE = false, bool UNF = false>
 __device__ __forceinline__ void rows_chain_body(const RowsRun& A, const int* __restrict__ ids, const float* __restrict__ dense,
                                                 float* __restrict__ out, int B, int* __restrict__ err,
-                                                const float* __restrict__ image, const RowsMany* __restrict__ Mp) {
+                                                const float* __restrict__ image, const Many* __restrict__ Mp) {
+    constexpr bool MB = !std::is_same<Many, RowsOne>::value;
     using LD = RowsLds<KPC, H0C, H1C, HASNUM, UNF>;
     using Set = typename std::conditional<UNF, RowsSetUnf<G_BIG, KPC, H0C>, RowsSet<G_BIG, KPC, H0C>>::type;
     static_assert(!UNF || (G_BIG <= 2 && KPC > 0), "UNF: two big fields are one K = 32 block");
@@ -147,20 +154,15 @@
     const int wave = __builtin_amdgcn_readfirstlane(tid >> 6);
     const int r = lane & 15, q = lane >> 4;
     const f32x4 zero = f32x4{0.f, 0.f, 0.f, 0.f};
-    const int m_n = MB ? Mp->n : 1, m_ntpb = MB ? Mp->ntpb : 0;
-    const int ntasks = MB ? m_n * m_ntpb : (B + 15) >> 4;
+    int m_ntpb = 0, ntasks = (B + 15) >> 4;
+    if constexpr (MB) { m_ntpb = Mp->ntpb; ntasks = Mp->n * m_ntpb; }
     const int task_stride = gridDim.x * WAVES;
     const int wave_global = blockIdx.x * WAVES + wave;
-    auto batch_of = [&](int tk, int& tl) {
-        if constexpr (MB) {
-            const int b = __builtin_amdgcn_readfirstlane(tk / m_ntpb);
-            tl = tk - b * m_ntpb;
-            return b;
-        } else {
-            tl = tk;
-            return 0;
-        }
-    };
+    auto batch_of = [&](int tk) -> int {
+        if constexpr (MB) return __builtin_amdgcn_readfirstlane(tk / m_ntpb);
+        else return 0;
+    };
+    auto in_batch = [&](int tk, int b) -> int { return MB ? tk - b * m_ntpb : tk; };
     float* stage = smem + LD::total_pad + wave * LD::stage_floats;
     const float* small_s = smem + LD::total_pad + WAVES * LD::stage_floats;
     const float* wq = smem + 4 * q;
@@ -168,11 +170,12 @@
     const bool aligned = !(A.flags & 1);
     auto clampt = [&](int tk) { return tk < ntasks ? tk : ntasks - 1; };
 
-    auto ld_raw = [&](int tkg, f32x4& raw) {
-        int tk;
-        const int bi = batch_of(tkg, tk);
-        const int* ids_b = MB ? Mp->ids[bi] : ids;
-        const float* dense_b = MB ? Mp->dense[bi] : dense;
+    auto ld_raw = [&](int tkg, f32x4& raw) -> int {
+        const int bi = batch_of(tkg);
+        const int tk = in_batch(tkg, bi);
+        const int* ids_b = ids;
+        const float* dense_b = dense;
+        if constexpr (MB) { ids_b = many_ids(*Mp, bi); dense_b = many_dense(*Mp, bi); }
         if (aligned && tk * 16 + 16 <= B) {
             const bool isid = lane < 32 || !HASNUM;
             const int j = lane < 32 ? lane : lane - 32;
@@ -181,18 +184,19 @@
                                     : dense_b + (size_t)tk * 16 * A.ND;
             raw = ld4(src + 4 * (j < n4 ? j : 0));
         }
-    };
-    auto gather = [&](int tkg, const f32x4& raw, Set& S) {
-        int tk;
-        const int bi = batch_of(tkg, tk);
-        const int* ids_b = MB ? Mp->ids[bi] : ids;
-        const float* dense_b = MB ? Mp->dense[bi] : dense;
+        return bi;
+    };
+    auto gather = [&](int tkg, int bi, const f32x4& raw, Set& S) {
+        const int tk = in_batch(tkg, bi);
         if (aligned && tk * 16 + 16 <= B) {
             const bool isid = lane < 32;
             const int j = isid ? lane : lane - 32;
             const int n4 = 4 * (isid ? A.F : (HASNUM ? A.ND : 0));
             if (j < n4) st4(stage + (isid ? 0 : 128) + 4 * j, raw);
         } else {
+            const int* ids_b = ids;
+            const float* dense_b = dense;
+            if constexpr (MB) { ids_b = many_ids(*Mp, bi); dense_b = many_dense(*Mp, bi); }
             stage_task_slow(stage, ids_b, dense_b, A.F, HASNUM ? A.ND : 0, tk, B, lane);
         }
         const int* sid_row = reinterpret_cast<const int*>(stage) + r * A.F;
@@ -242,6 +246,14 @@
             if (G_BIG > 1) so = q == 1 ? s1 : so;
             if (G_BIG > 2) so = q == 2 ? s2 : so;
             S.sc = A.scal[so];
+        }
+        if constexpr (MB) {
+            float* out_b = many_out(*Mp, bi);
+            asm("" : "+s"(out_b));
+            const int m = tk * 16 + r;
+            S.dst = (q == 0 && m < B) ? out_b + m : nullptr;
+        } else {
+            S.dst = nullptr;
         }
     };
 
@@ -360,20 +372,22 @@
         z += __shfl_xor(z, 32);
         return sigmoidf_fast(z + A.bias);
     };
-    auto store = [&](int tkg, float score) {
-        int tk;
-        const int bi = batch_of(tkg, tk);
-        float* out_b = MB ? Mp->out[bi] : out;
-        const int m = tk * 16 + r;
-        if (q == 0 && m < B) out_b[m] = score;
+    auto store = [&](int tkg, const Set& S, float score) {
+        if constexpr (MB) {
+            if (S.dst) *(__attribute__((address_space(1))) float*)(uintptr_t)S.dst = score;
+        } else {
+            const int m = tkg * 16 + r;
+            if (q == 0 && m < B) out[m] = score;
+        }
     };
 
     Set SA, SB;
     f32x4 rawA = zero, rawB = zero;
     int tA = wave_global, tB = wave_global + task_stride;
+    int nA = 0, nB = 0;
     if (ntasks > 0) {
-        if (!ONE || tA < ntasks) ld_raw(clampt(tA), rawA);
-        if (!ONE) ld_raw(clampt(tB), rawB);
+        if (!ONE || tA < ntasks) nA = ld_raw(clampt(tA), rawA);
+        if (!ONE) nB = ld_raw(clampt(tB), rawB);
     }
 #pragma unroll 1
     for (int c = wave; c < LD::total_pad / 256; c += WAVES) lds_dma16(image + c * 256 + lane * 4, smem + c * 256);
@@ -386,19 +400,19 @@
     static_assert(NG < 64, "vmcnt field");
     if constexpr (ONE) {
         if (tA < ntasks) {
-            gather(tA, rawA, SA);
+            gather(tA, nA, rawA, SA);
             __builtin_amdgcn_s_waitcnt(WAIT_NG);
         } else {
             __builtin_amdgcn_s_waitcnt(0x0F70);
         }
         __builtin_amdgcn_s_barrier();
         load_weights();
-        if (tA < ntasks) store(tA, compute(SA));
+        if (tA < ntasks) store(tA, SA, compute(SA));
     } else {
     constexpr bool FAST2 = NG < 16;
     const bool two = FAST2 && tA < ntasks && ntasks <= 2 * task_stride;
     if (two) {
-        gather(tA, rawA, SA);
+        gather(tA, nA, rawA, SA);
         __builtin_amdgcn_s_waitcnt(0x0F70 | (FAST2 ? NG : 0));
     } else {
         __builtin_amdgcn_s_waitcnt(0x0F70);
@@ -407,24 +421,24 @@
     load_weights();
     if (tA >= ntasks) {
     } else if (two) {
-        gather(clampt(tB), rawB, SB);
-        store(tA, compute(SA));
-        if (tB < ntasks) store(tB, compute(SB));
+        gather(clampt(tB), nB, rawB, SB);
+        store(tA, SA, compute(SA));
+        if (tB < ntasks) store(tB, SB, compute(SB));
     } else {
-        gather(tA, rawA, SA);
-        ld_raw(clampt(tA + 2 * task_stride), rawA);
-        gather(clampt(tB), rawB, SB);
-        ld_raw(clampt(tB + 2 * task_stride), rawB);
+        gather(tA, nA, rawA, SA);
+        nA = ld_raw(clampt(tA + 2 * task_stride), rawA);
+        gather(clampt(tB), nB, rawB, SB);
+        nB = ld_raw(clampt(tB + 2 * task_stride), rawB);
         for (;;) {
-            store(tA, compute(SA));
+            store(tA, SA, compute(SA));
             tA += 2 * task_stride;
-            gather(clampt(tA), rawA, SA);
-            ld_raw(clampt(tA + 2 * task_stride), rawA);
+            gather(clampt(tA), nA, rawA, SA);
+            nA = ld_raw(clampt(tA + 2 * task_stride), rawA);
             if (tB >= ntasks) break;
-            store(tB, compute(SB));
+            store(tB, SB, compute(SB));
             tB += 2 * task_stride;
-            gather(clampt(tB), rawB, SB);
-            ld_raw(clampt(tB + 2 * task_stride), rawB);
+            gather(clampt(tB), nB, rawB, SB);
+            nB = ld_raw(clampt(tB + 2 * task_stride), rawB);
             if (tA >= ntasks) break;
         }
     }
@@ -436,16 +450,21 @@
 __global__ __launch_bounds__(WAVES * 64, 2) void k_rows_chain(const RowsRun A, const int* __restrict__ ids,
                                                               const float* __restrict__ dense, float* __restrict__ out, int B,
                                                               int* __restrict__ err, const float* __restrict__ image) {
-    rows_chain_body<KPC, H0C, H1C, G_BIG, NJF, HASNUM, WAVES, false, false, UNF>(A, ids, dense, out, B, err, image, nullptr);
+    rows_chain_body<KPC, H0C, H1C, G_BIG, NJF, HASNUM, WAVES, RowsOne, false, UNF>(A, ids, dense, out, B, err, image, nullptr);
 }
 template <int KPC, int H0C, int H1C, int G_BIG, int NJF, bool HASNUM, int WAVES, bool UNF = false>
 __global__ __launch_bounds__(WAVES * 64, UNF ? 4 : 3) void k_rows_chain1(const RowsRun A, const int* __restrict__ ids,
                                                                const float* __restrict__ dense, float* __restrict__ out, int B,
                                                                int* __restrict__ err, const float* __restrict__ image) {
-    rows_chain_body<KPC, H0C, H1C, G_BIG, NJF, HASNUM, WAVES, false, true, UNF>(A, ids, dense, out, B, err, image, nullptr);
+    rows_chain_body<KPC, H0C, H1C, G_BIG, NJF, HASNUM, WAVES, RowsOne, true, UNF>(A, ids, dense, out, B, err, image, nullptr);
 }
 template <int KPC, int H0C, int H1C, int G_BIG, int NJF, bool HASNUM, int WAVES, bool UNF = false>
 __global__ __launch_bounds__(WAVES * 64, 2) void k_rows_chain_many(const RowsRun A, const RowsMany M, int B,
                                                                    int* __restrict__ err, const float* __restrict__ image) {
-    rows_chain_body<KPC, H0C, H1C, G_BIG, NJF, HASNUM, WAVES, true, false, UNF>(A, nullptr, nullptr, nullptr, B, err, image, &M);
-}
+    rows_chain_body<KPC, H0C, H1C, G_BIG, NJF, HASNUM, WAVES, RowsMany, false, UNF>(A, nullptr, nullptr, nullptr, B, err, image, &M);
+}
+template <int KPC, int H0C, int H1C, int G_BIG, int NJF, bool HASNUM, int WAVES, bool UNF = false>
+__global__ __launch_bounds__(WAVES * 64, 2) void k_rows_chain_many_tab(const RowsRun A, const ManyTab M, int B,
+                                                                       int* __restrict__ err, const float* __restrict__ image) {
+    rows_chain_body<KPC, H0C, H1C, G_BIG, NJF, HASNUM, WAVES, ManyTab, false, UNF>(A, nullptr, nullptr, nullptr, B, err, image, &M);
+}
diff --git a/sparrowrecsys_amd/csrc/tu_instances.h b/sparrowrecsys_amd/csrc/tu_instances.h
--- a/sparrowrecsys_amd/csrc/tu_instances.h
+++ b/sparrowrecsys_amd/csrc/tu_instances.h
@@ -68,24 +68,24 @@
 SPRK_INST_1 __global__ void sprk_dev::k_deepfm_v2_joint_many<3, 2, 1, 2, 1, 8, true>(sprk_dev::V2JRun, sprk_dev::V2JMany, int, int*, float const*);
 SPRK_INST_1 __global__ void sprk_dev::k_deepfm_v2_joint_many<3, 3, 1, 2, 1, 8, false>(sprk_dev::V2JRun, sprk_dev::V2JMany, int, int*, float const*);
 SPRK_INST_1 __global__ void sprk_dev::k_deepfm_v2_joint_many<3, 3, 1, 2, 1, 8, true>(sprk_dev::V2JRun, sprk_dev::V2JMany, int, int*, float const*);
-SPRK_INST_1 __global__ void sprk_dev::k_deepfm_v2_joint_many_tab<1, 1, 1, 2, 1, 8, false>(sprk_dev::V2JRun, sprk_dev::V2JManyTab, int, int*, float const*);
-SPRK_INST_1 __global__ void sprk_dev::k_deepfm_v2_joint_many_tab<1, 1, 1, 2, 1, 8, true>(sprk_dev::V2JRun, sprk_dev::V2JManyTab, int, int*, float const*);
-SPRK_INST_1 __global__ void sprk_dev::k_deepfm_v2_joint_many_tab<1, 2, 1, 2, 1, 8, false>(sprk_dev::V2JRun, sprk_dev::V2JManyTab, int, int*, float const*);
-SPRK_INST_1 __global__ void sprk_dev::k_deepfm_v2_joint_many_tab<1, 2, 1, 2, 1, 8, true>(sprk_dev::V2JRun, sprk_dev::V2JManyTab, int, int*, float const*);
-SPRK_INST_1 __global__ void sprk_dev::k_deepfm_v2_joint_many_tab<1, 3, 1, 2, 1, 8, false>(sprk_dev::V2JRun, sprk_dev::V2JManyTab, int, int*, float const*);
-SPRK_INST_1 __global__ void sprk_dev::k_deepfm_v2_joint_many_tab<1, 3, 1, 2, 1, 8, true>(sprk_dev::V2JRun, sprk_dev::V2JManyTab, int, int*, float const*);
-SPRK_INST_1 __global__ void sprk_dev::k_deepfm_v2_joint_many_tab<2, 1, 1, 2, 1, 8, false>(sprk_dev::V2JRun, sprk_dev::V2JManyTab, int, int*, float const*);
-SPRK_INST_1 __global__ void sprk_dev::k_deepfm_v2_joint_many_tab<2, 1, 1, 2, 1, 8, true>(sprk_dev::V2JRun, sprk_dev::V2JManyTab, int, int*, float const*);
-SPRK_INST_1 __global__ void sprk_dev::k_deepfm_v2_joint_many_tab<2, 2, 1, 2, 1, 8, false>(sprk_dev::V2JRun, sprk_dev::V2JManyTab, int, int*, float const*);
-SPRK_INST_1 __global__ void sprk_dev::k_deepfm_v2_joint_many_tab<2, 2, 1, 2, 1, 8, true>(sprk_dev::V2JRun, sprk_dev::V2JManyTab, int, int*, float const*);
-SPRK_INST_1 __global__ void sprk_dev::k_deepfm_v2_joint_many_tab<2, 3, 1, 2, 1, 8, false>(sprk_dev::V2JRun, sprk_dev::V2JManyTab, int, int*, float const*);
-SPRK_INST_1 __global__ void sprk_dev::k_deepfm_v2_joint_many_tab<2, 3, 1, 2, 1, 8, true>(sprk_dev::V2JRun, sprk_dev::V2JManyTab, int, int*, float const*);
-SPRK_INST_1 __global__ void sprk_dev::k_deepfm_v2_joint_many_tab<3, 1, 1, 2, 1, 8, false>(sprk_dev::V2JRun, sprk_dev::V2JManyTab, int, int*, float const*);
-SPRK_INST_1 __global__ void sprk_dev::k_deepfm_v2_joint_many_tab<3, 1, 1, 2, 1, 8, true>(sprk_dev::V2JRun, sprk_dev::V2JManyTab, int, int*, float const*);
-SPRK_INST_1 __global__ void sprk_dev::k_deepfm_v2_joint_many_tab<3, 2, 1, 2, 1, 8, false>(sprk_dev::V2JRun, sprk_dev::V2JManyTab, int, int*, float const*);
-SPRK_INST_1 __global__ void sprk_dev::k_deepfm_v2_joint_many_tab<3, 2, 1, 2, 1, 8, true>(sprk_dev::V2JRun, sprk_dev::V2JManyTab, int, int*, float const*);
-SPRK_INST_1 __global__ void sprk_dev::k_deepfm_v2_joint_many_tab<3, 3, 1, 2, 1, 8, false>(sprk_dev::V2JRun, sprk_dev::V2JManyTab, int, int*, float const*);
-SPRK_INST_1 __global__ void sprk_dev::k_deepfm_v2_joint_many_tab<3, 3, 1, 2, 1, 8, true>(sprk_dev::V2JRun, sprk_dev::V2JManyTab, int, int*, float const*);
+SPRK_INST_1 __global__ void sprk_dev::k_deepfm_v2_joint_many_tab<1, 1, 1, 2, 1, 8, false>(sprk_dev::V2JRun, sprk_dev::ManyTab, int, int*, float const*);
+SPRK_INST_1 __global__ void sprk_dev::k_deepfm_v2_joint_many_tab<1, 1, 1, 2, 1, 8, true>(sprk_dev::V2JRun, sprk_dev::ManyTab, int, int*, float const*);
+SPRK_INST_1 __global__ void sprk_dev::k_deepfm_v2_joint_many_tab<1, 2, 1, 2, 1, 8, false>(sprk_dev::V2JRun, sprk_dev::ManyTab, int, int*, float const*);
+SPRK_INST_1 __global__ void sprk_dev::k_deepfm_v2_joint_many_tab<1, 2, 1, 2, 1, 8, true>(sprk_dev::V2JRun, sprk_dev::ManyTab, int, int*, float const*);
+SPRK_INST_1 __global__ void sprk_dev::k_deepfm_v2_joint_many_tab<1, 3, 1, 2, 1, 8, false>(sprk_dev::V2JRun, sprk_dev::ManyTab, int, int*, float const*);
+SPRK_INST_1 __global__ void sprk_dev::k_deepfm_v2_joint_many_tab<1, 3, 1, 2, 1, 8, true>(sprk_dev::V2JRun, sprk_dev::ManyTab, int, int*, float const*);
+SPRK_INST_1 __global__ void sprk_dev::k_deepfm_v2_joint_many_tab<2, 1, 1, 2, 1, 8, false>(sprk_dev::V2JRun, sprk_dev::ManyTab, int, int*, float const*);
+SPRK_INST_1 __global__ void sprk_dev::k_deepfm_v2_joint_many_tab<2, 1, 1, 2, 1, 8, true>(sprk_dev::V2JRun, sprk_dev::ManyTab, int, int*, float const*);
+SPRK_INST_1 __global__ void sprk_dev::k_deepfm_v2_joint_many_tab<2, 2, 1, 2, 1, 8, false>(sprk_dev::V2JRun, sprk_dev::ManyTab, int, int*, float const*);
+SPRK_INST_1 __global__ void sprk_dev::k_deepfm_v2_joint_many_tab<2, 2, 1, 2, 1, 8, true>(sprk_dev::V2JRun, sprk_dev::ManyTab, int, int*, float const*);
+SPRK_INST_1 __global__ void sprk_dev::k_deepfm_v2_joint_many_tab<2, 3, 1, 2, 1, 8, false>(sprk_dev::V2JRun, sprk_dev::ManyTab, int, int*, float const*);
+SPRK_INST_1 __global__ void sprk_dev::k_deepfm_v2_joint_many_tab<2, 3, 1, 2, 1, 8, true>(sprk_dev::V2JRun, sprk_dev::ManyTab, int, int*, float const*);
+SPRK_INST_1 __global__ void sprk_dev::k_deepfm_v2_joint_many_tab<3, 1, 1, 2, 1, 8, false>(sprk_dev::V2JRun, sprk_dev::ManyTab, int, int*, float const*);
+SPRK_INST_1 __global__ void sprk_dev::k_deepfm_v2_joint_many_tab<3, 1, 1, 2, 1, 8, true>(sprk_dev::V2JRun, sprk_dev::ManyTab, int, int*, float const*);
+SPRK_INST_1 __global__ void sprk_dev::k_deepfm_v2_joint_many_tab<3, 2, 1, 2, 1, 8, false>(sprk_dev::V2JRun, sprk_dev::ManyTab, int, int*, float const*);
+SPRK_INST_1 __global__ void sprk_dev::k_deepfm_v2_joint_many_tab<3, 2, 1, 2, 1, 8, true>(sprk_dev::V2JRun, sprk_dev::ManyTab, int, int*, float const*);
+SPRK_INST_1 __global__ void sprk_dev::k_deepfm_v2_joint_many_tab<3, 3, 1, 2, 1, 8, false>(sprk_dev::V2JRun, sprk_dev::ManyTab, int, int*, float const*);
+SPRK_INST_1 __global__ void sprk_dev::k_deepfm_v2_joint_many_tab<3, 3, 1, 2, 1, 8, true>(sprk_dev::V2JRun, sprk_dev::ManyTab, int, int*, float const*);
 SPRK_INST_2 __global__ void sprk_dev::k_deepfm_v2_joint1<1, 1, false>(sprk_dev::V2JRun, int const*, float const*, float*, int, int*, float const*);
 SPRK_INST_2 __global__ void sprk_dev::k_deepfm_v2_joint1<1, 1, true>(sprk_dev::V2JRun, int const*, float const*, float*, int, int*, float const*);
 SPRK_INST_2 __global__ void sprk_dev::k_deepfm_v2_joint1<1, 2, false>(sprk_dev::V2JRun, int const*, float const*, float*, int, int*, float const*);
@@ -143,6 +143,19 @@
 SPRK_INST_2 __global__ void sprk_dev::k_rows_chain_many<4, 2, 1, 2, 2, true, 8, true>(sprk_dev::RowsRun, sprk_dev::RowsMany, int, int*, float const*);
 SPRK_INST_2 __global__ void sprk_dev::k_rows_chain_many<4, 2, 1, 3, 1, true, 8, false>(sprk_dev::RowsRun, sprk_dev::RowsMany, int, int*, float const*);
 SPRK_INST_2 __global__ void sprk_dev::k_rows_chain_many<4, 2, 1, 3, 3, true, 8, false>(sprk_dev::RowsRun, sprk_dev::RowsMany, int, int*, float const*);
+SPRK_INST_2 __global__ void sprk_dev::k_rows_chain_many_tab<0, 1, 1, 2, 0, false, 8, false>(sprk_dev::RowsRun, sprk_dev::ManyTab, int, int*, float const*);
+SPRK_INST_2 __global__ void sprk_dev::k_rows_chain_many_tab<1, 2, 1, 3, 3, true, 8, false>(sprk_dev::RowsRun, sprk_dev::ManyTab, int, int*, float const*);
+SPRK_INST_2 __global__ void sprk_dev::k_rows_chain_many_tab<2, 2, 1, 2, 2, true, 8, false>(sprk_dev::RowsRun, sprk_dev::ManyTab, int, int*, float const*);
+SPRK_INST_2 __global__ void sprk_dev::k_rows_chain_many_tab<2, 2, 1, 2, 2, true, 8, true>(sprk_dev::RowsRun, sprk_dev::ManyTab, int, int*, float const*);
+SPRK_INST_2 __global__ void sprk_dev::k_rows_chain_many_tab<2, 2, 1, 3, 3, true, 8, false>(sprk_dev::RowsRun, sprk_dev::ManyTab, int, int*, float const*);
+SPRK_INST_2 __global__ void sprk_dev::k_rows_chain_many_tab<4, 2, 1, 1, 1, true, 8, false>(sprk_dev::RowsRun, sprk_dev::ManyTab, int, int*, float const*);
+SPRK_INST_2 __global__ void sprk_dev::k_rows_chain_many_tab<4, 2, 1, 1, 1, true, 8, true>(sprk_dev::RowsRun, sprk_dev::ManyTab, int, int*, float const*);
+SPRK_INST_2 __global__ void sprk_dev::k_rows_chain_many_tab<4, 2, 1, 2, 1, true, 8, false>(sprk_dev::RowsRun, sprk_dev::ManyTab, int, int*, float const*);
+SPRK_INST_2 __global__ void sprk_dev::k_rows_chain_many_tab<4, 2, 1, 2, 1, true, 8, true>(sprk_dev::RowsRun, sprk_dev::ManyTab, int, int*, float const*);
+SPRK_INST_2 __global__ void sprk_dev::k_rows_chain_many_tab<4, 2, 1, 2, 2, true, 8, false>(sprk_dev::RowsRun, sprk_dev::ManyTab, int, int*, float const*);
+SPRK_INST_2 __global__ void sprk_dev::k_rows_chain_many_tab<4, 2, 1, 2, 2, true, 8, true>(sprk_dev::RowsRun, sprk_dev::ManyTab, int, int*, float const*);
+SPRK_INST_2 __global__ void sprk_dev::k_rows_chain_many_tab<4, 2, 1, 3, 1, true, 8, false>(sprk_dev::RowsRun, sprk_dev::ManyTab, int, int*, float const*);
+SPRK_INST_2 __global__ void sprk_dev::k_rows_chain_many_tab<4, 2, 1, 3, 3, true, 8, false>(sprk_dev::RowsRun, sprk_dev::ManyTab, int, int*, float const*);
 SPRK_INST_2 __global__ void sprk_dev::k_v2_pack_image<2, 4, 1, 2, 1, true>(sprk_dev::V2Args, float*);
 SPRK_INST_2 __global__ void sprk_dev::k_v2_pack_image<3, 4, 1, 2, 1, true>(sprk_dev::V2Args, float*);
 SPRK_INST_2 __global__ void sprk_dev::k_v2_pack_image<4, 4, 1, 2, 1, true>(sprk_dev::V2Args, float*);
@@ -186,6 +199,22 @@
 SPRK_INST_3 __global__ void sprk_dev::k_deepfm_pairs_many<6, 4, 4, 4, 8, false, true>(sprk_dev::V1Run, sprk_dev::V1Many, int, int*);
 SPRK_INST_3 __global__ void sprk_dev::k_deepfm_pairs_many<6, 4, 4, 4, 8, true, false>(sprk_dev::V1Run, sprk_dev::V1Many, int, int*);
 SPRK_INST_3 __global__ void sprk_dev::k_deepfm_pairs_many<6, 4, 4, 4, 8, true, true>(sprk_dev::V1Run, sprk_dev::V1Many, int, int*);
+SPRK_INST_3 __global__ void sprk_dev::k_deepfm_pairs_many_tab<4, 16, 4, 4, 8, false, false>(sprk_dev::V1Run, sprk_dev::ManyTab, int, int*);
+SPRK_INST_3 __global__ void sprk_dev::k_deepfm_pairs_many_tab<4, 16, 4, 4, 8, false, true>(sprk_dev::V1Run, sprk_dev::ManyTab, int, int*);
+SPRK_INST_3 __global__ void sprk_dev::k_deepfm_pairs_many_tab<4, 16, 4, 4, 8, true, false>(sprk_dev::V1Run, sprk_dev::ManyTab, int, int*);
+SPRK_INST_3 __global__ void sprk_dev::k_deepfm_pairs_many_tab<4, 16, 4, 4, 8, true, true>(sprk_dev::V1Run, sprk_dev::ManyTab, int, int*);
+SPRK_INST_3 __global__ void sprk_dev::k_deepfm_pairs_many_tab<4, 3, 4, 4, 8, false, false>(sprk_dev::V1Run, sprk_dev::ManyTab, int, int*);
+SPRK_INST_3 __global__ void sprk_dev::k_deepfm_pairs_many_tab<4, 3, 4, 4, 8, false, true>(sprk_dev::V1Run, sprk_dev::ManyTab, int, int*);
+SPRK_INST_3 __global__ void sprk_dev::k_deepfm_pairs_many_tab<4, 3, 4, 4, 8, true, false>(sprk_dev::V1Run, sprk_dev::ManyTab, int, int*);
+SPRK_INST_3 __global__ void sprk_dev::k_deepfm_pairs_many_tab<4, 3, 4, 4, 8, true, true>(sprk_dev::V1Run, sprk_dev::ManyTab, int, int*);
+SPRK_INST_3 __global__ void sprk_dev::k_deepfm_pairs_many_tab<4, 4, 4, 4, 8, false, false>(sprk_dev::V1Run, sprk_dev::ManyTab, int, int*);
+SPRK_INST_3 __global__ void sprk_dev::k_deepfm_pairs_many_tab<4, 4, 4, 4, 8, false, true>(sprk_dev::V1Run, sprk_dev::ManyTab, int, int*);
+SPRK_INST_3 __global__ void sprk_dev::k_deepfm_pairs_many_tab<4, 4, 4, 4, 8, true, false>(sprk_dev::V1Run, sprk_dev::ManyTab, int, int*);
+SPRK_INST_3 __global__ void sprk_dev::k_deepfm_pairs_many_tab<4, 4, 4, 4, 8, true, true>(sprk_dev::V1Run, sprk_dev::ManyTab, int, int*);
+SPRK_INST_3 __global__ void sprk_dev::k_deepfm_pairs_many_tab<6, 4, 4, 4, 8, false, false>(sprk_dev::V1Run, sprk_dev::ManyTab, int, int*);
+SPRK_INST_3 __global__ void sprk_dev::k_deepfm_pairs_many_tab<6, 4, 4, 4, 8, false, true>(sprk_dev::V1Run, sprk_dev::ManyTab, int, int*);
+SPRK_INST_3 __global__ void sprk_dev::k_deepfm_pairs_many_tab<6, 4, 4, 4, 8, true, false>(sprk_dev::V1Run, sprk_dev::ManyTab, int, int*);
+SPRK_INST_3 __global__ void sprk_dev::k_deepfm_pairs_many_tab<6, 4, 4, 4, 8, true, true>(sprk_dev::V1Run, sprk_dev::ManyTab, int, int*);
 SPRK_INST_3 __global__ void sprk_dev::k_v1_pack_image<4, 4, 1>(sprk_dev::V1Run, float*);
 SPRK_INST_3 __global__ void sprk_dev::k_v1_pack_image<4, 4, 4>(sprk_dev::V1Run, float*);
 SPRK_INST_4 __global__ void sprk_dev::k_dien_fused<10, 32, 8, 4>(sprk_dev::DienRun, sprk_dev::DinTailRun, int const*, float const*, float*, int, int*, float const*, float*);
```

Result: slower. 16.76 billion (-2.4%).
